# noway/nzcb-circom

Measured on AMD Instinct MI355X. Metric: PLONK proofs/sec for nzcp_live (~2^21 constraints) at 1/2/4/8 MI355X, higher is better.
Workload: dtype u32 limbs: BN254 Fr/Fq Montgomery, 8x32-bit and 9x29-bit (MSM, NTT twiddles, quotient); 1 GPU; nzcp_live fullProve: NZCPPubIdentity(1,351,0,4,2,4) witness on the GPU (600560 signals) + PLONK proof, n=2^21, nPublic=3, 2970 inputs; domain_size=2097152, n_public=3, n_constraints=1785813, n_vars=1782570, n_additions=1182010, proofs_per_gpu=140, total_proofs=140, parallelism=batch-shard x1 (no collective), proofs_in_flight_per_gpu=5

## Files before the change

include/nzcb_internal.h:

```cpp
#ifndef NZCB_INTERNAL_H
#define NZCB_INTERNAL_H

#include "nzcb.h"

#ifdef __cplusplus
extern "C" {
#endif

int nzcb_ctx_kernel_stats(nzcb_ctx* ctx, int enable, double out[4]);

int nzcb_debug_guard_check(int device, size_t* checked, int* damaged, nzcb_err* err);
int nzcb_debug_guard_selftest(int device, nzcb_err* err);

#define NZCB_FAULT_QUOTIENT 1
#define NZCB_DEBUG_GENERIC_K 2
#define NZCB_FAULT_LANE_ALLOC 3
int nzcb_debug_inject_fault(nzcb_ctx* ctx, int kind);

int nzcb_debug_f29(int device, int op, const uint32_t* in, size_t count, uint32_t* out, nzcb_err* err);

int nzcb_synth_setup(int power, int n_public, int n_inputs, uint64_t seed, uint32_t n_constraints,
                     const uint8_t* tau, int device, uint8_t** zkey_out, size_t* zkey_len, uint8_t** wtns_out,
                     size_t* wtns_len, nzcb_err* err);
#define NZCB_SYNTH_FREE_PUBLIC 1u
int nzcb_synth_setup_ex(int power, int n_public, int n_inputs, uint64_t seed, uint32_t n_constraints, uint32_t flags,
                        const uint8_t* tau, int device, uint8_t** zkey_out, size_t* zkey_len, uint8_t** wtns_out,
                        size_t* wtns_len, nzcb_err* err);
typedef struct nzcb_engine nzcb_engine;
nzcb_engine* nzcb_engine_create(int device, int max_log_ntt, size_t max_msm_points, nzcb_err* err);
void nzcb_engine_destroy(nzcb_engine* e);
int nzcb_engine_ntt(nzcb_engine* e, const uint8_t* in_lem, uint8_t* out_lem, int log_n, int inverse, nzcb_err* err);
int nzcb_engine_msm(nzcb_engine* e, const uint8_t* bases_lem, const uint8_t* scalars, size_t n, int scalars_mont,
                    uint8_t* out_affine, nzcb_err* err);
int nzcb_debug_ntt_coset(nzcb_engine* e, const uint8_t* in_lem, uint8_t* out_lem, int log_n, const uint8_t* c_lem,
                         int fold_len, nzcb_err* err);
int nzcb_engine_ntt_dev(nzcb_engine* e, const void* in, void* out, int log_n, int inverse, nzcb_err* err);
int nzcb_engine_msm_dev(nzcb_engine* e, const void* bases, const void* scalars, size_t n, int scalars_mont,
                        uint8_t* out_affine, nzcb_err* err);
int nzcb_engine_time_ntt(nzcb_engine* e, const void* in, void* out, int log_n, int inverse, int reps, double* ms,
                         nzcb_err* err);
int nzcb_engine_random_fr(nzcb_engine* e, void* dev_out, size_t n, uint64_t seed, nzcb_err* err);
int nzcb_engine_fixed_base(nzcb_engine* e, const void* dev_scalars_mont, size_t n, void* dev_out, nzcb_err* err);
int nzcb_engine_lagrange_basis(nzcb_engine* e, const void* dev_ptau, size_t ptau_n, int log_n, void* dev_out,
                               nzcb_err* err);
int nzcb_engine_time_msm(nzcb_engine* e, const void* bases, const void* scalars, size_t n, int scalars_mont, int reps,
                         double* ms, double* acc_ms, nzcb_err* err);
int nzcb_engine_msm_fixed_dev(nzcb_engine* e, const void* bases, size_t n_table, const void* scalars, size_t n,
                              int scalars_mont, uint8_t* out_affine, nzcb_err* err);
int nzcb_engine_msm_table_dev(nzcb_engine* e, const void* bases, size_t n_table, const void* scalars, size_t n,
                              int scalars_mont, int window, int sparse, int fold, uint8_t* out_affine,
                              nzcb_err* err);
int nzcb_debug_msm_plan(nzcb_engine* e, const void* bases, size_t n_table, const void* scalars, size_t n,
                        int scalars_mont, int window, int fold, uint32_t* info, uint32_t* offsets, size_t offsets_cap,
                        uint32_t* seg, size_t seg_cap, uint8_t* out_affine, nzcb_err* err);
int nzcb_engine_msm_sets_dev(nzcb_engine* e, const void* bases, size_t n_table, const void* const* scalars, int sets,
                             size_t n, int scalars_mont, int sparse, uint8_t* out_affine, nzcb_err* err);
int nzcb_engine_time_msm2(nzcb_engine* e, const void* bases, const void* scalars, size_t n, int scalars_mont,
                          int fixed_base, int reps, double* out, nzcb_err* err);
int nzcb_engine_fr_mul(nzcb_engine* e, const uint8_t* a_lem, const uint8_t* b_lem, uint8_t* out_lem, size_t n,
                       int field_q, nzcb_err* err);

int nzcb_engine_g1_lincomb(int device, const uint8_t* points, const uint8_t* scalars, const uint32_t* group_end,
                           size_t groups, uint8_t* out, nzcb_err* err);
int nzcb_engine_verify_batch(const uint8_t* vk, const uint8_t* proofs, const uint8_t* pubs, size_t pub_stride,
                             int n_public, int count, int transcript_public, int device, const uint8_t* seed,
                             int* valid_out, uint8_t* points_out, int* pairing_checks, nzcb_err* err);
int nzcb_debug_verify_batch_timings(double* ms, int cap);

nzcb_r1cs* nzcb_engine_r1cs_create(const uint8_t* r1cs, size_t len, int device, uint32_t long_row_threshold,
                                   int witness_tile, nzcb_err* err);
int nzcb_debug_r1cs_check_timings(double* ms, int cap);

nzcb_p256_key* nzcb_engine_p256_key_create(const uint8_t pub_xy[64], int device, int window, nzcb_err* err);
#define NZCB_P256_OP_ADD 0
#define NZCB_P256_OP_SUB 1
#define NZCB_P256_OP_MUL 2
#define NZCB_P256_OP_SQR 3
#define NZCB_P256_OP_INV 4
int nzcb_debug_p256_field(int device, int op, int field, const uint8_t* a, const uint8_t* b, size_t count,
                          uint8_t* out, nzcb_err* err);
int nzcb_debug_p256_mul2(nzcb_p256_key* k, const uint8_t* u1, const uint8_t* u2, size_t count, uint8_t* out_xy,
                         nzcb_err* err);
int nzcb_debug_p256_timings(double* ms, int cap);

int nzcb_debug_nzcp_decode_timings(double* ms, int cap);

int nzcb_engine_srs_check(int device, const uint8_t* points, uint64_t m, const uint8_t* g2, const uint8_t* seed,
                          uint32_t chunk_points, nzcb_key_finding* finding, uint8_t* lr_out ,
                          nzcb_err* err);
int nzcb_debug_key_check_timings(double* ms, int cap);

int nzcb_debug_ptau_timings(double* ms, int cap);
int nzcb_debug_ptau_batch_top(int level);

int nzcb_engine_groth16_rows(int device, int g2, const void* points, uint64_t n_points, const uint64_t* row_off,
                             uint64_t n_rows, const uint32_t* idx, const uint8_t* coefs, uint8_t* out,
                             nzcb_err* err);
int nzcb_debug_groth16_schedule(int chunk, int fan_in, int* prev_chunk, int* prev_fan_in);
int nzcb_debug_groth16_timings(double* out, int cap);

// ... 5 lines not shown
```

nzcb-circom_amd/csrc/capi_prover.cpp:

```cpp
#include <algorithm>
#include <atomic>
#include <condition_variable>
#include <cstring>
#include <mutex>
#include <shared_mutex>
#include <string>
#include <thread>
#include <vector>

#include "../../include/nzcb_internal.h"
#include "prover.h"

namespace nzcb {

std::string dec_le32(const uint8_t* le32) {
  uint32_t v[8];
  std::memcpy(v, le32, 32);
  std::string s;
  bool nz = true;
  while (nz) {
    uint64_t rem = 0;
    nz = false;
    for (int i = 7; i >= 0; i--) {
      uint64_t cur = (rem << 32) | v[i];
      v[i] = (uint32_t)(cur / 10);
      rem = cur % 10;
      if (v[i]) nz = true;
    }
    s.push_back((char)('0' + rem));
  }
  return std::string(s.rbegin(), s.rend());
}

}
using namespace nzcb;

struct nzcb_ctx {
  std::unique_ptr<Prover> p;
  std::vector<std::unique_ptr<Prover>> extra;
  std::vector<std::unique_ptr<Prover>> dev_p;
  std::vector<std::vector<std::unique_ptr<Prover>>> dev_extra;
  nzcb_log_fn log_fn = nullptr;
  void* log_user = nullptr;
  std::shared_mutex cfg;
  std::mutex pool_mu;
  std::condition_variable pool_cv;
  std::vector<Prover*> idle;
  double last_tm[11] = {0};
  std::atomic<int> pending_fault{0};
  std::atomic<int> lane_alloc_fault{0};
  Prover* lane(size_t i) { return i == 0 ? p.get() : extra[i - 1].get(); }
  size_t lanes() const { return 1 + extra.size(); }
  std::vector<Prover*> all() {
    std::vector<Prover*> v;
    for (size_t l = 0; l < lanes(); l++) {
      v.push_back(lane(l));
      for (size_t d = 0; d < dev_p.size(); d++) v.push_back(l == 0 ? dev_p[d].get() : dev_extra[d][l - 1].get());
    }
    return v;
  }
  std::vector<Prover*> usable() {
    if (p->split_send || !p->shards.empty()) return {p.get()};
    return all();
  }
  void reset_pool() {
    std::lock_guard<std::mutex> lk(pool_mu);
    idle = usable();
    std::reverse(idle.begin(), idle.end());
  }
  Prover* acquire(nzcb_log_fn fn, void* user) {
    Prover* q;
    {
      std::unique_lock<std::mutex> lk(pool_mu);
      pool_cv.wait(lk, [&] { return !idle.empty(); });
      q = idle.back();
      idle.pop_back();
    }
    if (!fn) {
      fn = log_fn;
      user = log_user;
    }
    if (fn)
      q->log = [fn, user](const std::string& m) { fn(user, m.c_str()); };
    else
      q->log = nullptr;
    q->fault = pending_fault.exchange(0);
    return q;
  }
  void release(Prover* q) {
    {
      std::lock_guard<std::mutex> lk(pool_mu);
      std::memcpy(last_tm, q->tm, sizeof(last_tm));
      idle.push_back(q);
    }
// ... 263 lines not shown
      throw;
    }
    pr->log = nullptr;
    ctx->release(pr);
    NZ_HIP(hipSetDevice(caller_dev));
  });
}
}

int nzcb_prove_witness(nzcb_ctx* ctx, const uint8_t* witness, size_t n_witness, const uint8_t* blinding,
                       uint8_t* proof_out, uint8_t* pub_out, size_t pub_cap, nzcb_err* err) {
  return prove_one(ctx, witness, n_witness, NZCB_WITNESS_HOST, blinding, proof_out, pub_out, pub_cap, nullptr, nullptr,
                   err);
}

int nzcb_prove_device(nzcb_ctx* ctx, const void* dev_witness, size_t n_witness, const uint8_t* blinding,
                      uint8_t* proof_out, uint8_t* pub_out, size_t pub_cap, nzcb_err* err) {
  return prove_one(ctx, dev_witness, n_witness, NZCB_WITNESS_DEVICE, blinding, proof_out, pub_out, pub_cap, nullptr,
                   nullptr, err);
}

int nzcb_prove(nzcb_ctx* ctx, const uint8_t* wtns, size_t wtns_len, const uint8_t* blinding, uint8_t* proof_out,
               uint8_t* pub_out, size_t pub_cap, nzcb_err* err) {
  return prove_one(ctx, wtns, wtns_len, NZCB_WITNESS_WTNS, blinding, proof_out, pub_out, pub_cap, nullptr, nullptr,
                   err);
}

int nzcb_prove_logged(nzcb_ctx* ctx, const void* witness, size_t n, int kind, const uint8_t* blinding,
                      uint8_t* proof_out, uint8_t* pub_out, size_t pub_cap, nzcb_log_fn log, void* log_user,
                      nzcb_err* err) {
  return prove_one(ctx, witness, n, kind, blinding, proof_out, pub_out, pub_cap, log, log_user, err);
}

int nzcb_ctx_last_timings(const nzcb_ctx* ctx, double* ms, int cap) {
  if (!ctx || !ms) return 0;
  int k = cap < 11 ? cap : 11;
  std::lock_guard<std::mutex> lk(const_cast<nzcb_ctx*>(ctx)->pool_mu);
  for (int i = 0; i < k; i++) ms[i] = ctx->last_tm[i];
  return k;
}

int nzcb_ctx_kernel_stats(nzcb_ctx* ctx, int enable, double out[4]) {
  if (!ctx) return NZCB_ERR_ARG;
  std::unique_lock<std::shared_mutex> ex(ctx->cfg, std::defer_lock);
  std::shared_lock<std::shared_mutex> sh(ctx->cfg, std::defer_lock);
  if (enable >= 0) ex.lock(); else sh.lock();
  if (out) {
    for (int i = 0; i < 4; i++) out[i] = 0;
    for (Prover* q : ctx->all())
      for (auto& m : q->msc) {
        out[0] += m->prof_ms;
        out[1] += (double)m->prof_launches;
        out[2] += (double)m->prof_points;
        out[3] += (double)m->prof_entries;
      }
  }
  if (enable >= 0) {
    for (Prover* q : ctx->all()) {
      q->prof_gpu = enable != 0;
      for (auto& m : q->msc) {
        m->prof = enable != 0;
        m->prof_ms = 0;
        m->prof_launches = m->prof_points = m->prof_entries = 0;
      }
    }
  }
  return 0;
}

int nzcb_debug_inject_fault(nzcb_ctx* ctx, int kind) {
  if (!ctx || (kind != 0 && kind != NZCB_FAULT_QUOTIENT && kind != NZCB_DEBUG_GENERIC_K &&
               kind != NZCB_FAULT_LANE_ALLOC))
    return NZCB_ERR_ARG;
  std::unique_lock<std::shared_mutex> lk(ctx->cfg);
  if (kind == NZCB_FAULT_LANE_ALLOC) {
    ctx->lane_alloc_fault = 1;
    return 0;
  }
  ctx->pending_fault = kind;
  if (kind == 0) ctx->lane_alloc_fault = 0;
  return 0;
}

int nzcb_proof_to_json(const uint8_t* proof, char* out, size_t cap) {
  if (!proof) return -1;
  static const char* pts[7] = {"A", "B", "C", "Z", "T1", "T2", "T3"};
  static const char* evs[7] = {"eval_a", "eval_b", "eval_c", "eval_s1", "eval_s2", "eval_zw", "eval_r"};
  std::string s = "{";
  for (int i = 0; i < 7; i++) s += std::string("\"") + pts[i] + "\":" + g1_json(proof + 64 * i) + ",";
  for (int i = 0; i < 7; i++) s += std::string("\"") + evs[i] + "\":\"" + dec_le32(proof + 9 * 64 + 32 * i) + "\",";
  s += "\"Wxi\":" + g1_json(proof + 7 * 64) + ",";
  s += "\"Wxiw\":" + g1_json(proof + 8 * 64) + ",";
  s += "\"protocol\":\"plonk\",\"curve\":\"bn128\"}";
  return copy_out(s, out, cap);
}

int nzcb_public_to_json(const uint8_t* pub, int n_public, char* out, size_t cap) {
  std::string s = "[";
  for (int i = 0; i < n_public; i++) {
    if (i) s += ",";
    s += "\"" + dec_le32(pub + 32 * i) + "\"";
  }
  s += "]";
  return copy_out(s, out, cap);
}

}
```

nzcb-circom_amd/csrc/groth16.h:

```cpp
#pragma once
#include <chrono>

#include "ptau_ops.h"
#include "r1cs_reader.h"

namespace nzcb {

struct G16Term {
  uint32_t idx, k;
};
constexpr uint32_t kG16Neg = 1u << 31, kG16Big = 1u << 30, kG16Low = kG16Big - 1;
struct G16Chunk {
  uint32_t t0, slot;
  uint16_t len, bits;
};
struct G16Fold {
  uint32_t begin, count;
};
constexpr uint32_t kG16NoSlot = ~0u;
constexpr uint32_t kG16DefaultChunk = 32, kG16DefaultFanIn = 8, kG16MaxKnob = 1024;

NZ_HD bool g16_bit(uint32_t k, const Fr* big, int b) {
  if (k & kG16Big) return (big[k & kG16Low].v[b >> 5] >> (b & 31)) & 1u;
  return b < 30 && ((k >> b) & 1u);
// ... 74 lines not shown
    if (!small) {
      if (big.size() >= kG16Low) throw Error(NZCB_ERR_ARG, "groth16: too many long coefficients");
      code = kG16Big | (uint32_t)big.size();
      big.push_back(k);
    }
    if (raw.size() >= kG16NoSlot - 1) throw Error(NZCB_ERR_ARG, "groth16: too many terms");
    raw.push_back({(uint32_t)row, (uint32_t)idx, code | (negative ? kG16Neg : 0u)});
  }
  G16Rows finish() {
    G16Rows r;
    r.n_rows = n_rows;
    r.n_points = n_points;
    r.row_off.assign((size_t)n_rows + 1, 0);
    for (const Raw& t : raw) r.row_off[t.row + 1]++;
    for (uint64_t i = 0; i < n_rows; i++) r.row_off[i + 1] += r.row_off[i];
    r.terms.resize(raw.size());
    std::vector<uint32_t> at(r.row_off.begin(), r.row_off.end() - 1);
    for (const Raw& t : raw) r.terms[at[t.row]++] = G16Term{t.idx, t.k};
    r.big = std::move(big);
    raw.clear();
    raw.shrink_to_fit();
    return r;
  }
};

struct G16Plan {
  std::vector<G16Chunk> chunks;
  std::vector<std::vector<G16Fold>> levels;
  std::vector<uint32_t> final_slot;
};
inline G16Plan g16_plan(G16Rows& r, uint32_t chunk, uint32_t fan_in) {
  if (chunk < 1 || chunk > kG16MaxKnob || fan_in < 2 || fan_in > kG16MaxKnob)
    throw Error(NZCB_ERR_ARG, "groth16: chunk length in 1..1024 and fan-in in 2..1024");
  G16Plan p;
  std::vector<uint32_t> off((size_t)r.n_rows), cnt((size_t)r.n_rows);
  std::vector<G16Chunk> cs;
  std::vector<uint32_t> hist((size_t)255 * (chunk + 1) + 1, 0);
  auto key = [&](const G16Chunk& c) { return (size_t)(254 - c.bits) * (chunk + 1) + (chunk - c.len); };
  uint32_t max_cnt = 0;
  for (uint64_t row = 0; row < r.n_rows; row++) {
    off[row] = (uint32_t)cs.size();
    if (r.row_off[row + 1] - r.row_off[row] > 1)
      std::stable_sort(r.terms.begin() + r.row_off[row], r.terms.begin() + r.row_off[row + 1],
                       [&](const G16Term& x, const G16Term& y) {
                         return g16_k_bits(x.k, r.big.data()) > g16_k_bits(y.k, r.big.data());
                       });
    for (uint32_t t0 = r.row_off[row], len; t0 < r.row_off[row + 1]; t0 += len) {
      uint32_t work = 0;
      for (len = 0; len < chunk && t0 + len < r.row_off[row + 1]; len++) {
        const uint32_t adds = std::max(1, g16_k_bits(r.terms[t0 + len].k, r.big.data()) / 2);
        if (len && work + adds > 4 * chunk) break;
        work += adds;
      }
      G16Chunk c;
      c.t0 = t0;
      c.slot = (uint32_t)cs.size();
      c.len = (uint16_t)len;
      c.bits = (uint16_t)g16_k_bits(r.terms[t0].k, r.big.data());
      hist[key(c) + 1]++;
      cs.push_back(c);
    }
    cnt[row] = (uint32_t)cs.size() - off[row];
    max_cnt = std::max(max_cnt, cnt[row]);
  }
  for (size_t i = 1; i < hist.size(); i++) hist[i] += hist[i - 1];
  p.chunks.resize(cs.size());
  for (const G16Chunk& c : cs) p.chunks[hist[key(c)]++] = c;
  while (max_cnt > 1) {
    std::vector<G16Fold> lv;
    max_cnt = 0;
    for (uint64_t row = 0; row < r.n_rows; row++) {
      const uint32_t begin = off[row], have = cnt[row];
      off[row] = (uint32_t)lv.size();
      for (uint32_t g = 0; g < have; g += fan_in) lv.push_back({begin + g, std::min(fan_in, have - g)});
      cnt[row] = (uint32_t)lv.size() - off[row];
      max_cnt = std::max(max_cnt, cnt[row]);
    }
    p.levels.push_back(std::move(lv));
  }
  p.final_slot.resize((size_t)r.n_rows);
  for (uint64_t row = 0; row < r.n_rows; row++) p.final_slot[row] = cnt[row] ? off[row] : kG16NoSlot;
  return p;
}

struct G16Schedule {
  uint32_t chunk = kG16DefaultChunk, fan_in = kG16DefaultFanIn;
};
inline G16Schedule& g16_schedule() {
  static G16Schedule s;
  return s;
}
enum {
  kG16MsKernels,
  kG16MsCall,
  kG16MsRowsG1,
  kG16MsRowsG2,
  kG16MsTests,
  kG16MsScale,
  kG16MsPlan,
  kG16TermsA,
  kG16TermsB1,
  kG16TermsB2,
  kG16TermsK,
  kG16ChunksG1,
  kG16ChunksG2,
  kG16StatCount
};
inline double* g16_stats() {
  thread_local double s[kG16StatCount] = {0};
  return s;
}
using G16Clock = std::chrono::steady_clock;
inline double g16_ms_since(G16Clock::time_point t0) {
  return std::chrono::duration<double, std::milli>(G16Clock::now() - t0).count();
}
struct G16CallClock {
  G16Clock::time_point t0 = G16Clock::now();
  G16CallClock() {
    for (int i = 0; i < kG16StatCount; i++) g16_stats()[i] = 0;
  }
  ~G16CallClock() { g16_stats()[kG16MsCall] = g16_ms_since(t0); }
};

struct G16Span {
  const uint8_t* p;
  uint64_t count;
};

struct G16HostBackend {
  Fq2 b2 = g2_twist_b();

  template <class F>
  Tally test(const uint8_t* pts, uint64_t n, bool zero_ok) {
    Tally t;
    for (uint64_t i = 0; i < n; i++) {
      PtAffine<F> p;
      std::memcpy((void*)&p, pts + sizeof p * i, sizeof p);
      const int st = g16_pt_status<F>(&p, b2, zero_ok);
      if (st == NZCB_KEY_OK) continue;
      t.n_bad++;
      t.key = std::min(t.key, srs_bad_key(i, st));
    }
    return t;
  }
  template <class F>
  void rows(const std::vector<G16Span>& spans, const G16Rows& r, const G16Plan& plan, uint8_t* out) {
    std::vector<PtAffine<F>> pts((size_t)r.n_points);
    size_t at = 0;
    for (const G16Span& s : spans) {
      if (s.count) std::memcpy((void*)(pts.data() + at), s.p, sizeof(PtAffine<F>) * (size_t)s.count);
      at += (size_t)s.count;
    }
    std::vector<PtXyzz<F>> a(plan.chunks.size()), b;
    parallel_for(plan.chunks.size(), [&](uint64_t i) {
      const G16Chunk& c = plan.chunks[i];
      a[c.slot] = g16_chunk_sum<F>(pts.data(), r.terms.data(), r.big.data(), c);
    });
    for (const auto& lv : plan.levels) {
      b.resize(lv.size());
      parallel_for(lv.size(), [&](uint64_t i) { b[i] = g16_fold_sum<F>(a.data(), lv[i]); });
      a.swap(b);
    }
    parallel_for(r.n_rows, [&](uint64_t row) {
      const uint32_t s = plan.final_slot[row];
      const PtAffine<F> v = s == kG16NoSlot ? PtAffine<F>{F::zero(), F::zero()} : pt_to_affine(a[s]);
      std::memcpy(out + sizeof v * row, &v, sizeof v);
// ... 334 lines not shown
```

nzcb-circom_amd/csrc/groth16.hip:

```cpp
#include "devcall.h"
#include "groth16.h"

namespace nzcb {

namespace {

constexpr unsigned kGB = 64;

template <class F>
__global__ __launch_bounds__(kGB) void k_g16_test(const PtAffine<F>* __restrict__ pts, uint64_t n, Fq2 b2,
                                                  int zero_ok, unsigned long long* res) {
  const uint64_t i = (uint64_t)blockIdx.x * kGB + threadIdx.x;
  if (i >= n) return;
  const PtAffine<F> p = pts[i];
  const int st = g16_pt_status<F>(&p, b2, zero_ok != 0);
  if (st != NZCB_KEY_OK) {
    atomicAdd(&res[0], 1ull);
    atomicMin(&res[1], (unsigned long long)srs_bad_key(i, st));
  }
}

template <class F>
__global__ __launch_bounds__(kGB) void k_g16_chunks(const PtAffine<F>* __restrict__ pts,
                                                    const G16Term* __restrict__ terms, const Fr* __restrict__ big,
// ... 109 lines not shown
    }
    k_g16_store<F><<<grid_for(r.n_rows, kGB, 1u << 30), kGB, 0, cs.st>>>(in, d_final.p, (uint32_t)r.n_rows, d_out.p);
    NZ_HIP(hipGetLastError());
    cs.record(1);
    NZ_HIP(hipMemcpyAsync(out, d_out.p, sizeof(PtAffine<F>) * (size_t)r.n_rows, hipMemcpyDeviceToHost, cs.st));
    NZ_HIP(hipStreamSynchronize(cs.st));
    took(std::is_same<F, Fq>::value ? kG16MsRowsG1 : kG16MsRowsG2);
  }
  template <class F>
  void rows(const std::vector<G16Span>& spans, const G16Rows& r, const G16Plan& plan, uint8_t* out) {
    DevBuf<PtAffine<F>> d_pts(std::max<size_t>(1, (size_t)r.n_points));
    size_t at = 0;
    for (const G16Span& s : spans) {
      if (s.count)
        NZ_HIP(hipMemcpyAsync(d_pts.p + at, s.p, sizeof(PtAffine<F>) * (size_t)s.count, hipMemcpyHostToDevice, cs.st));
      at += (size_t)s.count;
    }
    if (at != r.n_points) throw Error(NZCB_ERR_INTERNAL, "groth16: point count mismatch");
    rows_on<F>(d_pts.p, r, plan, out);
  }
  template <class F>
  void scale(const uint8_t* src, uint64_t n, const Fr& k, uint8_t* dst) {
    if (!n) return;
    DevBuf<uint8_t> d(sizeof(PtAffine<F>) * n);
    NZ_HIP(hipMemcpyAsync(d_k, &k, sizeof k, hipMemcpyHostToDevice, cs.st));
    NZ_HIP(hipMemcpyAsync(d.p, src, d.n, hipMemcpyHostToDevice, cs.st));
    cs.record(0);
    k_g16_scale<F><<<grid_for(n, kGB, 1u << 30), kGB, 0, cs.st>>>(reinterpret_cast<PtAffine<F>*>(d.p), n, d_k);
    NZ_HIP(hipGetLastError());
    cs.record(1);
    NZ_HIP(hipMemsetAsync(d_k, 0, sizeof(Fr), cs.st));
    NZ_HIP(hipMemcpyAsync(dst, d.p, d.n, hipMemcpyDeviceToHost, cs.st));
    NZ_HIP(hipStreamSynchronize(cs.st));
    took(kG16MsScale);
  }
};

void setup_on(int device, const uint8_t* r1cs, size_t r1cs_len, const uint8_t* ptau, size_t ptau_len,
              const char* out_path, PtauOut& o) {
  G16CallClock clock;
  if (device == NZCB_GROTH16_HOST) {
    G16HostBackend be;
    g16_setup(be, r1cs, r1cs_len, ptau, ptau_len, out_path, o);
  } else {
    G16DeviceBackend be(device);
    g16_setup(be, r1cs, r1cs_len, ptau, ptau_len, out_path, o);
  }
}

struct Secret {
  Fr d;
  ~Secret() { wipe(&d, sizeof d); }
};

void contribute_on(int device, const uint8_t* zkey, size_t len, const uint8_t* secret, const uint8_t* entropy,
                   size_t entropy_len, const char* out_path, PtauOut& o) {
  if (!zkey) throw Error(NZCB_ERR_ARG, "null argument");
  G16CallClock clock;
  (void)g16_zkey_open(zkey, len);
  Secret sec;
  make_secrets(secret, entropy, entropy_len, &sec.d, 1, "zkey");
  if (device == NZCB_GROTH16_HOST) {
    G16HostBackend be;
    g16_contribute(be, zkey, len, sec.d, out_path, o);
  } else {
    G16DeviceBackend be(device);
    g16_contribute(be, zkey, len, sec.d, out_path, o);
  }
}

void require_distinct(const char* in_path, const char* out_path, const char* what) {
  struct stat a, b;
  if (stat(in_path, &a) == 0 && stat(out_path, &b) == 0 && a.st_dev == b.st_dev && a.st_ino == b.st_ino)
    throw Error(NZCB_ERR_ARG, std::string(what) + ": the output path is an input file");
}

void give(PtauOut& o, uint8_t** out, size_t* out_len) {
  *out_len = (size_t)o.len;
  *out = o.release();
}

}

}

using namespace nzcb;

extern "C" {

int nzcb_groth16_setup(const uint8_t* r1cs, size_t r1cs_len, const uint8_t* ptau, size_t ptau_len, int device,
                       uint8_t** zkey_out, size_t* zkey_len, nzcb_err* err) {
  return guarded(err, [&] {
    if (!zkey_out || !zkey_len) throw Error(NZCB_ERR_ARG, "null argument");
    PtauOut o;
    setup_on(device, r1cs, r1cs_len, ptau, ptau_len, nullptr, o);
    give(o, zkey_out, zkey_len);
  });
}

int nzcb_groth16_setup_file(const char* r1cs_path, const char* ptau_path, const char* zkey_path, int device,
                            nzcb_err* err) {
  return guarded(err, [&] {
    if (!r1cs_path || !ptau_path || !zkey_path) throw Error(NZCB_ERR_ARG, "null argument");
    require_distinct(r1cs_path, zkey_path, "groth16");
    require_distinct(ptau_path, zkey_path, "groth16");
    MappedFile rf(r1cs_path, "the r1cs", "r1cs: invalid file format");
    MappedFile pf(ptau_path, "the ptau", "ptau: invalid file format");
    PtauOut o;
    setup_on(device, rf.data, rf.size, pf.data, pf.size, zkey_path, o);
  });
}

int nzcb_groth16_contribute(const uint8_t* zkey, size_t len, const uint8_t* secret, const uint8_t* entropy,
                            size_t entropy_len, int device, uint8_t** zkey_out, size_t* zkey_len, nzcb_err* err) {
  return guarded(err, [&] {
    if (!zkey_out || !zkey_len) throw Error(NZCB_ERR_ARG, "null argument");
    PtauOut o;
    contribute_on(device, zkey, len, secret, entropy, entropy_len, nullptr, o);
    give(o, zkey_out, zkey_len);
  });
}

int nzcb_groth16_contribute_file(const char* in_path, const char* out_path, const uint8_t* secret,
                                 const uint8_t* entropy, size_t entropy_len, int device, nzcb_err* err) {
  return guarded(err, [&] {
    if (!in_path || !out_path) throw Error(NZCB_ERR_ARG, "null argument");
    require_distinct(in_path, out_path, "zkey");
    MappedFile mf(in_path, "the zkey", "zkey: invalid file format");
    PtauOut o;
    contribute_on(device, mf.data, mf.size, secret, entropy, entropy_len, out_path, o);
  });
}

int nzcb_groth16_vk_to_json(const uint8_t* zkey, size_t len, char* out, size_t cap) {
  nzcb_err err;
  std::string s;
  const int rc = guarded(&err, [&] { s = g16_vk_json(zkey, len); });
  if (rc != 0) {
    if (out && cap) std::snprintf(out, cap, "%s", err.msg);
    return rc;
  }
  if (!out || cap < s.size() + 1) return -(int)(s.size() + 1);
  std::memcpy(out, s.c_str(), s.size() + 1);
  return 0;
}

int nzcb_groth16_vk_to_json_file(const char* zkey_path, char* out, size_t cap) {
  nzcb_err err;
  std::string s;
  const int rc = guarded(&err, [&] {
    if (!zkey_path) throw Error(NZCB_ERR_ARG, "null argument");
    MappedFile mf(zkey_path, "the zkey", "zkey: invalid file format");
    s = g16_vk_json(mf.data, mf.size);
  });
  if (rc != 0) {
    if (out && cap) std::snprintf(out, cap, "%s", err.msg);
    return rc;
  }
  if (!out || cap < s.size() + 1) return -(int)(s.size() + 1);
  std::memcpy(out, s.c_str(), s.size() + 1);
  return 0;
}

int nzcb_engine_groth16_rows(int device, int g2, const void* points, uint64_t n_points, const uint64_t* row_off,
                             uint64_t n_rows, const uint32_t* idx, const uint8_t* coefs, uint8_t* out,
                             nzcb_err* err) {
// ... 42 lines not shown
```

nzcb-circom_amd/csrc/msm.h:

```cpp
#pragma once
#include <vector>

#include "common.h"
#include "ec.h"
#include "f29.h"
#include "msm_seg.h"

namespace nzcb {

struct MsmBaseTable {
  DevBuf<G1Affine> q;
  size_t n = 0, stride = 0;
  int c = 0, nw = 0;
  bool mont_folded = false;
  bool sparse = false;
  void build(const G1Affine* bases, size_t n, int c, hipStream_t st, bool fold_mont = false);
};

int fixed_base_window();
int lagrange_window();
bool lagrange_sparse();
bool acc_segments();

struct MsmScratch {
  size_t max_points = 0;
  int max_lsets = 1;
  DevBuf<uint32_t> offsets;
  DevBuf<uint32_t> sorted;
  DevBuf<uint32_t> keys_in, keys_out, vals_in;
  DevBuf<uint8_t> sort_tmp;
  size_t sort_tmp_bytes = 0;
  DevBuf<uint32_t> bin_counts, vals_mid;
  DevBuf<uint32_t> lo_seg;
  DevBuf<G1xyzz> buckets;
  DevBuf<G1xyzz> carry_own;
  DevBuf<G1xyzz> carry_cont;
  DevBuf<Xyzz29> buckets29, carry_own29, carry_cont29;
  DevBuf<uint32_t> large;
  DevBuf<uint32_t> large_off;
  DevBuf<Xyzz29> large_part;
  DevBuf<uint32_t> seg_start, seg_len, seg_bucket, seg_dst, seg_cnt, seg_meta, seg_mk, seg_mfs, seg_mnp;
  DevBuf<Xyzz29> rowp29, colp29, lines29;
  DevBuf<G1xyzz> seg_tot;
  DevBuf<G1xyzz> seg_run;
  DevBuf<G1xyzz> parts;
  DevBuf<G1xyzz> win;
  G1xyzz* host_win = nullptr;
  uint32_t* host_total = nullptr;
  size_t host_win_cap = 0;
  int cur_c = 0, cur_nsets = 0, cur_nbits = 0, cur_seglen = 0;
  bool cur_fixed = false, cur_sparse = false;
  bool cur_seg = false;
  int cur_a = 0, cur_hb = 0;
  int cur_msets = 1;
  size_t cur_n = 0;
  uint32_t cur_nkeys = 0;
  bool prof = false, prof_phases = false;
  double prof_ms = 0;
  double phase_ms[7] = {0, 0, 0, 0, 0, 0, 0};
  double host_ms = 0;
  double enqueue_ms = 0;
  double sort_host_ms = 0;
  uint64_t prof_launches = 0, prof_points = 0, prof_entries = 0;
  hipEvent_t ev[8] = {nullptr, nullptr, nullptr, nullptr, nullptr, nullptr, nullptr, nullptr};
  hipEvent_t done = nullptr;
  void init(size_t max_points, bool fixed_base = false, int lagrange_sets = 1, bool generic = true);
  ~MsmScratch();
};

int msm_window_bits(size_t n);

void msm_enqueue(MsmScratch& sc, const G1Affine* bases, const Fr* scalars, size_t n, bool scalars_mont,
                 hipStream_t st, const MsmBaseTable* table = nullptr);
G1xyzz msm_finish(MsmScratch& sc, hipStream_t st);
void msm_enqueue_sets(MsmScratch& sc, const Fr* const* scalars, int sets, size_t n, bool scalars_mont,
                      hipStream_t st, const MsmBaseTable* table);
void msm_finish_sets(MsmScratch& sc, hipStream_t st, G1xyzz* out);

inline G1xyzz msm(MsmScratch& sc, const G1Affine* bases, const Fr* scalars, size_t n, bool mont, hipStream_t st,
                  const MsmBaseTable* table = nullptr) {
  msm_enqueue(sc, bases, scalars, n, mont, st, table);
  return msm_finish(sc, st);
}

bool msm_debug_plan(MsmScratch& sc, hipStream_t st, std::vector<uint32_t>& offsets, std::vector<uint32_t>& start,
                    std::vector<uint32_t>& len, std::vector<uint32_t>& bucket);

G1Affine xyzz_to_affine(const G1xyzz& p);

}
```

nzcb-circom_amd/csrc/msm.hip:

```cpp
#include "msm.h"

#include "f29.h"

#include <chrono>
#include <cstdlib>
#include <type_traits>
#include <rocprim/rocprim.hpp>
#include <rocprofiler-sdk-roctx/roctx.h>

namespace nzcb {

static constexpr int kMsmThreads = 256;

#ifndef NZ_TAIL_PRIO
#define NZ_TAIL_PRIO 0
#endif
__device__ __forceinline__ void tail_prio() {
  if constexpr (NZ_TAIL_PRIO > 0) __builtin_amdgcn_s_setprio(NZ_TAIL_PRIO);
}

using SortConfig = rocprim::radix_sort_config<
    rocprim::default_config, rocprim::default_config,
    rocprim::radix_sort_onesweep_config<rocprim::kernel_config<1024, 16>, rocprim::kernel_config<1024, 16>, 10,
                                        rocprim::block_radix_rank_algorithm::match>>;
// ... 97 lines not shown
      if (d) f(w, d - 1u, 0u);
      carry = 0;
    }
  }
}

#ifdef NZCB_MSM_STATS
template <class F>
static void for_each_digit_host(const Fr& s, int C, F&& f) {
  const int NW = (255 + C - 1) / C;
  const uint32_t MASK = (1u << C) - 1u, HALF = 1u << (C - 1);
  uint32_t carry = 0;
  for (int w = 0; w < NW; w++) {
    const int bit = w * C, limb = bit >> 5, sh = bit & 31;
    uint64_t x = s.v[limb];
    if (limb + 1 < 8) x |= (uint64_t)s.v[limb + 1] << 32;
    uint32_t d = ((uint32_t)(x >> sh) & MASK) + carry;
    if (d > HALF) {
      uint32_t mag = (MASK + 1u) - d;
      if (mag) f(w, mag - 1u, 1u);
      carry = 1;
    } else {
      if (d) f(w, d - 1u, 0u);
      carry = 0;
    }
  }
}
#endif

template <int C>
__global__ void __launch_bounds__(kMsmThreads)
msm_keys_kernel(const Fr* __restrict__ scalars, size_t n, int mont, uint32_t* __restrict__ keys,
                uint32_t* __restrict__ vals) {
  constexpr int NW = (255 + C - 1) / C;
  constexpr uint32_t NB = 1u << (C - 1);
  constexpr uint32_t SENTINEL = NW * NB;
  for (size_t i = (size_t)blockIdx.x * blockDim.x + threadIdx.x; i < n; i += (size_t)gridDim.x * blockDim.x) {
    Fr s = scalars[i];
    if (mont) s = from_mont_fr29(s);
    uint32_t k[NW];
#pragma unroll
    for (int w = 0; w < NW; w++) k[w] = SENTINEL;
    uint32_t sg[NW];
#pragma unroll
    for (int w = 0; w < NW; w++) sg[w] = 0;
    for_each_digit<C>(s, [&](int w, uint32_t b, uint32_t sign) {
      k[w] = (uint32_t)w * NB + b;
      sg[w] = sign << 31;
    });
#pragma unroll
    for (int w = 0; w < NW; w++) {
      keys[(size_t)w * n + i] = k[w];
      vals[(size_t)w * n + i] = (uint32_t)i | sg[w];
    }
  }
}

static constexpr int kBinThreads = 256;
static constexpr int kBinPer = 2;
static constexpr uint32_t kTileScalars = kBinThreads * kBinPer;
static constexpr int kLoThreads = 512;

static constexpr int kDigMont = 1;
static constexpr int kDigMinForm = 2;

__device__ __forceinline__ uint32_t scalar_min_form(Fr& s) {
  constexpr uint32_t H[8] = {0xf8000000u, 0xa1f0fac9u, 0x3cdcb848u, 0x9419f424u,
                             0x40c0ac2eu, 0xdc2822dbu, 0x7098d014u, 0x18322739u};
  bool gt = false, eq = true, lt_r = false, eq_r = true;
#pragma unroll
  for (int l = 7; l >= 0; l--) {
    gt = gt || (eq && s.v[l] > H[l]);
    eq = eq && s.v[l] == H[l];
    lt_r = lt_r || (eq_r && s.v[l] < FrParams::P[l]);
    eq_r = eq_r && s.v[l] == FrParams::P[l];
  }
  if (!(gt && lt_r)) return 0u;
  s = neg(s);
  return 1u;
}

template <int C, int NW>
__device__ __forceinline__ uint32_t bin_entries(const Fr* __restrict__ scalars, size_t i, int mont, size_t stride,
                                                uint32_t (&kk)[NW], uint32_t (&vv)[NW]) {
  Fr s = scalars[i];
  if (mont & kDigMont) s = from_mont_fr29(s);
  const uint32_t flip = (mont & kDigMinForm) ? scalar_min_form(s) : 0u;
  uint32_t live = 0;
#pragma unroll
  for (int w = 0; w < NW; w++) {
    kk[w] = 0;
    vv[w] = 0;
  }
  for_each_digit<C>(s, [&](int w, uint32_t b, uint32_t sign) {
    kk[w] = b;
    vv[w] = (uint32_t)((size_t)w * stride + i) | ((sign ^ flip) << 31);
    live |= 1u << w;
  });
  return live;
}

template <int KB> struct BinKeys {
  static constexpr int LO = KB - 8 > 8 ? KB - 8 : 8;
  using Lo = typename std::conditional<LO <= 8, uint8_t, uint16_t>::type;
  using Full = typename std::conditional<KB <= 16, uint16_t, uint32_t>::type;
};

static constexpr int kMaxSets = 3;
struct BinSets {
  const Fr* p[kMaxSets];
  uint32_t tps;
  uint32_t nb;
};

template <int C, int KB>
__global__ void __launch_bounds__(kBinThreads)
msm_bin_hist_kernel(BinSets sets, size_t n, int mont, uint32_t* __restrict__ counts, uint32_t ntiles) {
  constexpr int NW = (255 + C - 1) / C;
  constexpr int LO = BinKeys<KB>::LO;
  __shared__ uint32_t h[256];
  h[threadIdx.x] = 0;
  __syncthreads();
  const uint32_t set = blockIdx.x / sets.tps, lt = blockIdx.x - set * sets.tps;
  const Fr* __restrict__ scalars = sets.p[set];
  const uint32_t kbase = set * sets.nb;
#pragma unroll
  for (int j = 0; j < kBinPer; j++) {
    const size_t i = (size_t)lt * kTileScalars + (size_t)j * kBinThreads + threadIdx.x;
    if (i < n) {
      uint32_t kk[NW], vv[NW];
      const uint32_t live = bin_entries<C, NW>(scalars, i, mont, 0, kk, vv);
#pragma unroll
      for (int w = 0; w < NW; w++)
        if ((live >> w) & 1u) atomicAdd(&h[(kk[w] + kbase) >> LO], 1u);
    }
  }
  __syncthreads();
  counts[(size_t)threadIdx.x * ntiles + blockIdx.x] = h[threadIdx.x];
}

__device__ __forceinline__ uint32_t wave_incl_scan(uint32_t v) {
  const int lane = threadIdx.x & 63;
#pragma unroll
  for (int off = 1; off < 64; off <<= 1) {
    const uint32_t u = __shfl_up(v, off, 64);
    if (lane >= off) v += u;
  }
  return v;
}

__device__ __forceinline__ uint32_t scan256_excl(uint32_t v, uint32_t* wsum4, uint32_t& total) {
  const uint32_t inc = wave_incl_scan(threadIdx.x < 256 ? v : 0u);
  if (threadIdx.x < 256 && (threadIdx.x & 63) == 63) wsum4[threadIdx.x >> 6] = inc;
  __syncthreads();
  uint32_t off = 0;
  for (int w = 0; w < (int)(threadIdx.x >> 6) && w < 4; w++) off += wsum4[w];
  total = wsum4[0] + wsum4[1] + wsum4[2] + wsum4[3];
  __syncthreads();
  return threadIdx.x < 256 ? off + inc - v : 0u;
}

__global__ void __launch_bounds__(256)
msm_bin_rowscan_kernel(uint32_t* __restrict__ counts, uint32_t ntiles, uint32_t* __restrict__ tail) {
  __shared__ uint32_t wsum[4];
  uint32_t* row = counts + (size_t)blockIdx.x * ntiles;
  uint32_t carry = 0;
  for (uint32_t c0 = 0; c0 < ntiles; c0 += 256) {
    const uint32_t t = c0 + threadIdx.x;
    const uint32_t v = t < ntiles ? row[t] : 0u;
    uint32_t tot;
    const uint32_t ex = scan256_excl(v, wsum, tot);
    if (t < ntiles) row[t] = carry + ex;
    carry += tot;
  }
  if (threadIdx.x == 0) tail[blockIdx.x] = carry;
}

template <int C, int KB>
__global__ void __launch_bounds__(kBinThreads)
msm_bin_scatter_kernel(BinSets sets, size_t n, int mont, size_t stride, const uint32_t* __restrict__ counts,
                       uint32_t ntiles, typename BinKeys<KB>::Lo* __restrict__ lo2, uint32_t* __restrict__ vals2) {
  constexpr int NW = (255 + C - 1) / C;
  constexpr int TE = kTileScalars * NW;
  constexpr int LO = BinKeys<KB>::LO;
  __shared__ uint32_t lcount[256], lstart[256], gbase[256];
  __shared__ uint32_t lval[TE];
  __shared__ typename BinKeys<KB>::Full lkey[TE];
  const uint32_t set = blockIdx.x / sets.tps, lt = blockIdx.x - set * sets.tps;
  const Fr* __restrict__ scalars = sets.p[set];
  const uint32_t kbase = set * sets.nb;
  __shared__ uint32_t wsum[4];
  const uint32_t* tail = counts + (size_t)256 * ntiles;
  {
    uint32_t tot;
    const uint32_t st = scan256_excl(tail[threadIdx.x], wsum, tot);
    gbase[threadIdx.x] = st + counts[(size_t)threadIdx.x * ntiles + blockIdx.x];
    lcount[threadIdx.x] = 0;
  }
  __syncthreads();
  uint32_t kk[kBinPer][NW], vv[kBinPer][NW], rk[kBinPer][NW], live[kBinPer];
#pragma unroll
  for (int j = 0; j < kBinPer; j++) {
    const size_t i = (size_t)lt * kTileScalars + (size_t)j * kBinThreads + threadIdx.x;
    live[j] = 0;
    if (i < n) {
      live[j] = bin_entries<C, NW>(scalars, i, mont, stride, kk[j], vv[j]);
#pragma unroll
      for (int w = 0; w < NW; w++) {
        kk[j][w] += kbase;
        if ((live[j] >> w) & 1u) rk[j][w] = atomicAdd(&lcount[kk[j][w] >> LO], 1u);
      }
    }
  }
  __syncthreads();
  uint32_t total;
  {
    lstart[threadIdx.x] = scan256_excl(lcount[threadIdx.x], wsum, total);
  }
  __syncthreads();
#pragma unroll
  for (int j = 0; j < kBinPer; j++) {
#pragma unroll
    for (int w = 0; w < NW; w++) {
      if ((live[j] >> w) & 1u) {
        const uint32_t q = lstart[kk[j][w] >> LO] + rk[j][w];
        lkey[q] = (typename BinKeys<KB>::Full)kk[j][w];
        lval[q] = vv[j][w];
      }
    }
  }
  __syncthreads();
  for (uint32_t q = threadIdx.x; q < total; q += kBinThreads) {
    const uint32_t key = lkey[q], hb = key >> LO;
    const uint32_t pos = gbase[hb] + (q - lstart[hb]);
    lo2[pos] = (typename BinKeys<KB>::Lo)(key & ((1u << LO) - 1u));
    vals2[pos] = lval[q];
  }
}

template <int NT>
__device__ __forceinline__ uint32_t block_scan_excl(uint32_t* a, uint32_t count, uint32_t* wsum) {
  const uint32_t per = (count + NT - 1) / NT;
  const uint32_t b = threadIdx.x * per;
  uint32_t loc = 0;
  for (uint32_t i = 0; i < per; i++)
    if (b + i < count) loc += a[b + i];
  const uint32_t inc = wave_incl_scan(loc);
  if ((threadIdx.x & 63) == 63) wsum[threadIdx.x >> 6] = inc;
  __syncthreads();
  uint32_t off = 0, tot = 0;
#pragma unroll
  for (int w = 0; w < NT / 64; w++) {
    if (w < (int)(threadIdx.x >> 6)) off += wsum[w];
    tot += wsum[w];
  }
  uint32_t run = off + inc - loc;
  for (uint32_t i = 0; i < per; i++)
    if (b + i < count) {
      const uint32_t v = a[b + i];
      a[b + i] = run;
      run += v;
    }
  __syncthreads();
  return tot;
}

static constexpr uint32_t kLoSeg = 32768;
static constexpr uint32_t kLoU = 8;

__device__ __forceinline__ void lo_regions(const uint32_t* __restrict__ tail, uint32_t* wsum, uint32_t* rs,
                                           uint32_t* rf) {
  const uint32_t t = threadIdx.x;
  const uint32_t cnt = t < 256 ? tail[t] : 0u;
  uint32_t tot, nitems;
  const uint32_t st = scan256_excl(cnt, wsum, tot);
  const uint32_t f = scan256_excl((cnt + kLoSeg - 1) / kLoSeg, wsum, nitems);
  if (t < 256) {
    rs[t] = st;
    rf[t] = f;
  }
  if (t == 0) rf[256] = nitems;
  __syncthreads();
}

__device__ __forceinline__ uint32_t lo_region_of(const uint32_t* rf, uint32_t item) {
  uint32_t lo = 0, hi = 256;
  while (hi - lo > 1) {
    const uint32_t mid = (lo + hi) >> 1;
    if (rf[mid] <= item) lo = mid; else hi = mid;
// ... 206 lines not shown
    inf = false;
  } else {
    F29 U2, S2, PP, RR;
    mul29x2<Fq29>(x, acc.ZZ, y, acc.ZZZ, U2, S2);
    const F29 Pd = sub29(U2, acc.X, Fq29::K8);
    const F29 R = sub29(S2, acc.Y, Fq29::K4);
    sqr29x2(Pd, R, PP, RR);
    if (is0p29_fast(PP)) {
      if (is0p29(RR)) {
        norm29(y);
        mdbl29_rare(x, y, &acc);
      } else {
        inf = true;
      }
    } else {
      F29 PPP, Q, ZZ3, ZZZ3;
      mul29x2<Fq29>(Pd, PP, acc.X, PP, PPP, Q);
      const F29 X3 = sub2x29(RR, PPP, Q);
      mul29x2<Fq29>(acc.ZZ, PP, acc.ZZZ, PPP, ZZ3, ZZZ3);
      acc.Y = mul2sum29(R, sub29_nn(Q, X3, Fq29W::K10), neg4p29_nn(acc.Y), PPP);
      acc.ZZ = ZZ3;
      acc.ZZZ = ZZZ3;
      acc.X = X3;
    }
  }
}

static constexpr uint32_t kLdsStride = kMsmThreads + 1;
template <bool kLdsIdx>
__global__ void __launch_bounds__(kMsmThreads) __attribute__((amdgpu_waves_per_eu(3, 8)))
msm_accumulate29_kernel(uint32_t chunk, const G1Affine* __restrict__ bases, const uint32_t* __restrict__ sorted,
                        const uint32_t* __restrict__ offsets, uint32_t nkeys, size_t nthreads,
                        Xyzz29* __restrict__ buckets, Xyzz29* __restrict__ carry_own,
                        Xyzz29* __restrict__ carry_cont) {
  __shared__ uint32_t sidx[kLdsIdx ? kChunk * kLdsStride : 1];
  const uint32_t t = blockIdx.x * blockDim.x + threadIdx.x;
  const uint32_t M = offsets[nkeys];
  if (!chunk) {
    chunk = dyn_chunk(M);
    tail_prio();
  }
  if (kLdsIdx) {
    const uint32_t wg0 = (uint32_t)blockIdx.x * kMsmThreads * chunk;
    if (wg0 >= M) return;
    const uint32_t inv = (uint32_t)((0x100000000ull + chunk - 1) / chunk);
    for (uint32_t j = threadIdx.x; j < kMsmThreads * chunk; j += kMsmThreads) {
      const uint32_t thr = __umulhi(j, inv), slot = j - thr * chunk;
      sidx[slot * kLdsStride + thr] = wg0 + j < M ? sorted[wg0 + j] : 0u;
    }
    __syncthreads();
  }
  if (t >= nthreads) return;
  const uint32_t s = (uint32_t)t * chunk;
  if (s >= M) return;
  const uint32_t e = (s + chunk < M) ? s + chunk : M;
  auto index_at = [&](uint32_t q) -> uint32_t {
    return kLdsIdx ? sidx[(q - s) * kLdsStride + threadIdx.x] : sorted[q];
  };
  uint32_t k = find_key(offsets, nkeys, s);
  uint32_t kstart = offsets[k], kend = offsets[k + 1];
  Xyzz29 acc;
  bool inf = true;
  uint32_t ent = index_at(s);
  G1Affine P = bases[ent & 0x7fffffffu];
  uint32_t ent_n = s + 1 < e ? index_at(s + 1) : 0u;
  for (uint32_t pos = s; pos < e;) {
    G1Affine Pn;
    uint32_t ent_nn = 0;
    if (pos + 1 < e) Pn = bases[ent_n & 0x7fffffffu];
    if (pos + 2 < e) ent_nn = index_at(pos + 2);
    acc_entry29(acc, inf, P, ent);
    pos++;
    if (pos == kend || pos == e) {
      const bool starts = kstart >= s;
      const bool ends = kend <= e;
      Xyzz29 out = acc;
      if (inf)
#pragma unroll
        for (int i = 0; i < 9; i++) out.ZZ.v[i] = 0;
      if (starts && ends) buckets[k] = out;
      else if (!starts) carry_cont[t] = out;
      else carry_own[t] = out;
      inf = true;
      while (pos < e && kend <= pos) {
        k++;
        kstart = kend;
        kend = offsets[k + 1];
      }
    }
    ent = ent_n;
    ent_n = ent_nn;
    P = Pn;
  }
}

struct SegPlan {
  uint32_t *start, *len, *bucket, *dst;
  uint32_t *mk, *mfs, *mnp;
  uint32_t* meta;
};

static constexpr int kSegThreads = 256;
static constexpr uint32_t kSegWaves = kSegThreads / 64;

__global__ void __launch_bounds__(kSegThreads)
msm_seg_hist_kernel(const uint32_t* __restrict__ offsets, uint32_t nkeys, uint32_t ntiles,
                    uint32_t* __restrict__ cnt, uint32_t* __restrict__ meta) {
  __shared__ uint32_t h[kSegWaves][kSegMax + 1];
  const uint32_t wave = threadIdx.x >> 6, lane = threadIdx.x & 63;
  const uint32_t tile = blockIdx.x * kSegWaves + wave;
  for (uint32_t i = threadIdx.x; i < kSegWaves * (kSegMax + 1); i += kSegThreads) (&h[0][0])[i] = 0;
  if (blockIdx.x == 0 && threadIdx.x == 0) meta[1] = 0;
  __syncthreads();
  if (tile < ntiles) {
    for (uint32_t it = 0; it < kSegTile / 64; it++) {
      const uint32_t k = tile * kSegTile + it * 64 + lane;
      if (k >= nkeys) break;
      const uint32_t len = offsets[k + 1] - offsets[k];
      const uint32_t whole = len / kSegMax, rest = len % kSegMax;
      if (whole) atomicAdd(&h[wave][kSegMax], whole);
      if (rest) atomicAdd(&h[wave][rest], 1u);
    }
  }
  __syncthreads();
  if (tile < ntiles)
    for (uint32_t L = 1 + lane; L <= kSegMax; L += 64) cnt[(size_t)(kSegMax - L) * ntiles + tile] = h[wave][L];
}

__global__ void __launch_bounds__(kSegThreads)
msm_seg_scatter_kernel(const uint32_t* __restrict__ offsets, uint32_t nkeys, uint32_t ntiles,
                       const uint32_t* __restrict__ cnt, SegPlan pl) {
  __shared__ uint32_t cb[256], wsum[4];
  __shared__ uint32_t base_s[kSegWaves][kSegMax + 1];
  const uint32_t wave = threadIdx.x >> 6, lane = threadIdx.x & 63;
  const uint32_t tile = blockIdx.x * kSegWaves + wave;
  uint32_t total;
  const uint32_t* tail = cnt + (size_t)kSegMax * ntiles;
  cb[threadIdx.x] = scan256_excl(threadIdx.x < kSegMax ? tail[threadIdx.x] : 0u, wsum, total);
  if (blockIdx.x == 0 && threadIdx.x == 0) pl.meta[0] = total;
  __syncthreads();
  volatile uint32_t* base = base_s[wave];
  if (tile < ntiles)
    for (uint32_t L = 1 + lane; L <= kSegMax; L += 64)
      base[L] = cb[kSegMax - L] + cnt[(size_t)(kSegMax - L) * ntiles + tile];
  __syncthreads();
  if (tile >= ntiles) return;
  for (uint32_t it = 0; it < kSegTile / 64; it++) {
    const uint32_t k0 = tile * kSegTile + it * 64;
    if (k0 >= nkeys) break;
    const uint32_t k = k0 + lane;
    const uint32_t s = k < nkeys ? offsets[k] : 0u;
    const uint32_t len = k < nkeys ? offsets[k + 1] - s : 0u;
    const uint32_t whole = len / kSegMax, rest = len % kSegMax;
    const bool cut = whole + (rest ? 1u : 0u) > 1;
    const uint32_t incl = wave_incl_scan(whole);
    const uint32_t wtot = __shfl(incl, 63, 64);
    const uint32_t fs = base[kSegMax] + incl - whole;
    if (lane == 0 && wtot) base[kSegMax] = fs + wtot;
    const uint32_t dst = cut ? 0x80000000u | fs : k;
    for (uint32_t j = 0; j < whole; j++) {
      pl.start[fs + j] = s + j * kSegMax;
      pl.len[fs + j] = kSegMax;
      pl.bucket[fs + j] = k;
      pl.dst[fs + j] = dst;
    }
    uint64_t same = __ballot(rest != 0);
#pragma unroll
// ... 733 lines not shown
  };
  switch (c) {
#define NZ_CASE(K) case K: launch(std::integral_constant<int, K>()); break;
    NZ_CASE(4) NZ_CASE(5) NZ_CASE(6) NZ_CASE(7) NZ_CASE(8) NZ_CASE(9) NZ_CASE(10) NZ_CASE(11) NZ_CASE(12)
    NZ_CASE(13) NZ_CASE(14) NZ_CASE(15) NZ_CASE(16)
#undef NZ_CASE
    default: throw Error(NZCB_ERR_INTERNAL, "bad msm window");
  }
  NZ_HIP(hipGetLastError());
}

G1Affine xyzz_to_affine(const G1xyzz& p) {
  G1Affine r;
  if (p.is_inf()) {
    r.x = Fq::zero();
    r.y = Fq::zero();
    return r;
  }
  r.x = p.X * inverse(p.ZZ);
  r.y = p.Y * inverse(p.ZZZ);
  return r;
}

template <class Mark>
static void fixed_bucketing(MsmScratch& sc, const MsmPlan& p, const BinSets& sets, size_t n, int mdig,
                            const MsmBaseTable* table, hipStream_t st, const Mark& mark) {
  const uint32_t tps = (uint32_t)((n + kTileScalars - 1) / kTileScalars);
  const uint32_t ntiles = tps * (uint32_t)p.msets;
  BinSets bs = sets;
  bs.tps = tps;
  bs.nb = p.nb;
  uint32_t* tail = sc.bin_counts.p + (size_t)256 * ntiles;
  auto run_bins = [&](auto cc, auto kb) {
    constexpr int C = decltype(cc)::value;
    constexpr int KB = decltype(kb)::value;
    using Lo = typename BinKeys<KB>::Lo;
    constexpr int LO = BinKeys<KB>::LO;
    Lo* lo2 = (Lo*)sc.keys_out.p;
    hipLaunchKernelGGL((msm_bin_hist_kernel<C, KB>), dim3(ntiles), dim3(kBinThreads), 0, st, bs, n, mdig,
                       sc.bin_counts.p, ntiles);
    NZ_HIP(hipGetLastError());
    lmark("mark: L hist");
    mark(1);
    hipLaunchKernelGGL(msm_bin_rowscan_kernel, dim3(256), dim3(256), 0, st, sc.bin_counts.p, ntiles, tail);
    lmark("mark: L rowscan");
    hipLaunchKernelGGL((msm_bin_scatter_kernel<C, KB>), dim3(ntiles), dim3(kBinThreads), 0, st, bs, n, mdig,
                       table->stride, sc.bin_counts.p, ntiles, lo2, sc.vals_mid.p);
    NZ_HIP(hipGetLastError());
    lmark("mark: L scatter");
    mark(2);
    const dim3 igrid((unsigned)lo_items_bound(p.entries));
    hipLaunchKernelGGL(msm_lo_count_kernel<LO>, igrid, dim3(kLoThreads), 0, st, (const Lo*)lo2, sc.bin_counts.p,
                       ntiles, sc.lo_seg.p);
    NZ_HIP(hipGetLastError());
    lmark("mark: L lo_count");
    hipLaunchKernelGGL(msm_lo_scan_kernel<LO>, dim3(256), dim3(kLoThreads), 0, st, sc.bin_counts.p, ntiles,
                       sc.lo_seg.p, p.nkeys, sc.offsets.p, sc.large.p);
    NZ_HIP(hipGetLastError());
    lmark("mark: L lo_scan");
    constexpr int sNT = LO > 8 ? 1024 : kLoThreads;
    constexpr uint32_t sU = LO > 8 ? 16 : kLoU;
    hipLaunchKernelGGL((msm_lo_scatter_kernel<LO, sNT, sU>), igrid, dim3(sNT), 0, st, (const Lo*)lo2, sc.vals_mid.p,
                       sc.bin_counts.p, ntiles, (const uint32_t*)sc.lo_seg.p, sc.sorted.p);
    NZ_HIP(hipGetLastError());
    lmark("mark: L lo_scatter");
  };
  using std::integral_constant;
  if (p.msets > 1) {
    if (p.c != 17) throw Error(NZCB_ERR_INTERNAL, "msm sets: the Lagrange window (17) only");
    run_bins(integral_constant<int, 17>(), integral_constant<int, 18>());
    return;
  }
  switch (p.c) {
    case 16: run_bins(integral_constant<int, 16>(), integral_constant<int, 15>()); break;
    case 17: run_bins(integral_constant<int, 17>(), integral_constant<int, 16>()); break;
    case 18: run_bins(integral_constant<int, 18>(), integral_constant<int, 17>()); break;
    case 19: run_bins(integral_constant<int, 19>(), integral_constant<int, 18>()); break;
    case 20: run_bins(integral_constant<int, 20>(), integral_constant<int, 19>()); break;
    default: throw Error(NZCB_ERR_INTERNAL, "bad fixed-base msm window");
  }
}

static void msm_enqueue_impl(MsmScratch& sc, const G1Affine* bases, const Fr* const* scalars, int msets, size_t n,
                             bool mont, hipStream_t st, const MsmBaseTable* table) {
  const auto t_enq = std::chrono::steady_clock::now();
  struct EnqueueClock {
    MsmScratch& sc;
    std::chrono::steady_clock::time_point t0;
    ~EnqueueClock() {
      if (sc.prof && sc.prof_phases)
        sc.enqueue_ms += std::chrono::duration<double, std::milli>(std::chrono::steady_clock::now() - t0).count();
    }
  } enqueue_clock{sc, t_enq};
  if (msets < 1 || msets > kMaxSets || (msets > 1 && (!table || msets > sc.max_lsets)))
    throw Error(NZCB_ERR_ARG, "msm sets: 1..3 over a table, within the scratch's sizing");
  sc.cur_n = n;
  sc.cur_msets = table ? msets : 1;
  if (n == 0) return;
  if (!sc.done) NZ_HIP(hipEventCreateWithFlags(&sc.done, hipEventDisableTiming));
  if (n > sc.max_points) throw Error(NZCB_ERR_ARG, "msm larger than scratch");
  if (table && n > table->n) throw Error(NZCB_ERR_ARG, "msm larger than its base table");
  if (table && table->mont_folded && !mont) throw Error(NZCB_ERR_ARG, "2^-256-folded table needs Montgomery scalars");
  if (table && (!sc.buckets29.p || !sc.bin_counts.p))
    throw Error(NZCB_ERR_ARG, "msm scratch was not sized for the fixed-base schedule");
  const int mdig = (mont && !(table && table->mont_folded)) ? 1 : 0;
  const MsmPlan p = make_plan(n, table, msets);
#ifdef NZCB_MSM_STATS
  if (table && !table->mont_folded) {
    NZ_HIP(hipStreamSynchronize(st));
    for (int k = 0; k < msets; k++) {
      std::vector<Fr> h(n);
      NZ_HIP(hipMemcpy(h.data(), scalars[k], n * sizeof(Fr), hipMemcpyDeviceToHost));
      size_t e_pos = 0, e_min = 0, nneg = 0, zero = 0, hist[17] = {0};
      for (size_t i = 0; i < n; i++) {
        Fr v = mdig ? from_mont(h[i]) : h[i];
        if (v.is_zero()) { zero++; continue; }
        const Fr w = neg(v);
        auto digits = [&](const Fr& x) {
          size_t d = 0;
          for_each_digit_host(x, p.c, [&](int, uint32_t, uint32_t) { d++; });
          return d;
        };
        const size_t dp = digits(v), dn = digits(w);
        e_pos += dp;
        e_min += dp <= dn ? dp : dn;
        if (dn < dp) nneg++;
        const size_t dm = dp <= dn ? dp : dn;
        hist[dm < 16 ? dm : 16]++;
      }
      fprintf(stderr, "MSMSCALARS set=%d n=%zu c=%d zero=%zu entries=%zu entries_minform=%zu flipped=%zu hist_minform=",
              k, n, p.c, zero, e_pos, e_min, nneg);
      for (int b = 0; b < 17; b++) fprintf(stderr, "%zu%c", hist[b], b == 16 ? '\n' : ',');
    }
  }
#endif
  if (p.entries + 4 > sc.sorted.n || p.nkeys + 1 > sc.offsets.n)
    throw Error(NZCB_ERR_ARG, "msm scratch was not sized for this schedule");
  const bool seg = table && !table->sparse && msets == 1 && acc_segments();
  if (seg && (seg_bound(p.entries, p.nkeys) > sc.seg_start.n || seg_counters(p.nkeys) > sc.seg_cnt.n ||
              seg_multi_bound(p.entries, p.nkeys) + 1 > sc.seg_mk.n ||
              seg_whole_bound(p.entries) + 1 > sc.carry_cont29.n ||
              seg_carry_bound(p.entries, p.nkeys) / kPieceCarries + seg_multi_bound(p.entries, p.nkeys) + 1 >
                  sc.large_part.n))
    throw Error(NZCB_ERR_ARG, "msm scratch was not sized for the segment plan");
  if (table && ((size_t)p.nb / kTileSide * msets > sc.rowp29.n ||
                (((size_t)1 << p.hb) + ((size_t)1 << p.a)) * msets > sc.lines29.n ||
                (size_t)(p.lb + 1) * msets > sc.host_win_cap || (msets > 1 && p.c >= kStripMinC)))
    throw Error(NZCB_ERR_ARG, "msm scratch was not sized for this window");
  sc.cur_c = p.c;
  sc.cur_nsets = p.nsets;
  sc.cur_nbits = p.nbits;
  sc.cur_seglen = p.seglen;
  sc.cur_nkeys = p.nkeys;
  sc.cur_fixed = table != nullptr;
  sc.cur_seg = seg;
  sc.cur_a = p.a;
  sc.cur_hb = p.hb;
  sc.cur_msets = p.msets;
  const bool phases = sc.prof && sc.prof_phases;
  if (sc.prof && !sc.ev[0])
    for (auto& e : sc.ev) NZ_HIP(hipEventCreate(&e));
  auto mark = [&](int i) {
    if (phases) NZ_HIP(hipEventRecord(sc.ev[i], st));
  };
  mark(0);
  if (table) {
    BinSets bs{};
    for (int k = 0; k < msets; k++) bs.p[k] = scalars[k];
    fixed_bucketing(sc, p, bs, n, mdig | (table->mont_folded ? 0 : kDigMinForm), table, st, mark);
  } else {
    keys_dispatch(p.c, scalars[0], n, mdig, sc, st);
    mark(1);
    size_t tmp = sc.sort_tmp_bytes;
    int end_bit = 1;
    while ((1u << end_bit) <= p.nkeys) end_bit++;
    const auto t_sort = std::chrono::steady_clock::now();
    radix_sort(sc.sort_tmp.p, tmp, sc.keys_in.p, sc.keys_out.p, sc.vals_in.p, sc.sorted.p, p.entries, end_bit, st);
    if (phases)
      sc.sort_host_ms += std::chrono::duration<double, std::milli>(std::chrono::steady_clock::now() - t_sort).count();
    mark(2);
    hipLaunchKernelGGL(msm_offsets_kernel, dim3(grid_for((size_t)p.nkeys + 1, kMsmThreads, 1u << 30)),
                       dim3(kMsmThreads), 0, st, sc.keys_out.p, p.entries, p.nkeys, sc.offsets.p);
    NZ_HIP(hipGetLastError());
  }
  const SegPlan pl{sc.seg_start.p, sc.seg_len.p, sc.seg_bucket.p, sc.seg_dst.p,
                   sc.seg_mk.p,    sc.seg_mfs.p, sc.seg_mnp.p,   sc.seg_meta.p};
  if (seg) {
    const uint32_t ntiles = (uint32_t)seg_tiles(p.nkeys);
    const dim3 tgrid((ntiles + kSegWaves - 1) / kSegWaves);
    hipLaunchKernelGGL(msm_seg_hist_kernel, tgrid, dim3(kSegThreads), 0, st, (const uint32_t*)sc.offsets.p, p.nkeys,
                       ntiles, sc.seg_cnt.p, sc.seg_meta.p);
    NZ_HIP(hipGetLastError());
    hipLaunchKernelGGL(msm_bin_rowscan_kernel, dim3(kSegMax), dim3(256), 0, st, sc.seg_cnt.p, ntiles,
                       sc.seg_cnt.p + (size_t)kSegMax * ntiles);
    NZ_HIP(hipGetLastError());
    hipLaunchKernelGGL(msm_seg_scatter_kernel, tgrid, dim3(kSegThreads), 0, st, (const uint32_t*)sc.offsets.p, p.nkeys,
                       ntiles, (const uint32_t*)sc.seg_cnt.p, pl);
    NZ_HIP(hipGetLastError());
    lmark("mark: L seg_plan");
  }
  if (sc.prof) NZ_HIP(hipEventRecord(sc.ev[3], st));
  const bool sparse = table && table->sparse;
  sc.cur_sparse = sparse;
  const uint32_t chunk = sparse ? 0u : chunk_for(p.entries);
  const size_t nthreads = sparse ? dyn_threads_bound(p.entries) : (p.entries + chunk - 1) / chunk;
  const dim3 agrid(grid_for(nthreads, kMsmThreads, 1u << 30));
  const G1Affine* gather = table ? table->q.p : bases;
  if (seg) {
    const dim3 sgrid(grid_for(seg_bound(p.entries, p.nkeys), kMsmThreads, 1u << 30));
    hipLaunchKernelGGL(msm_accumulate29_seg_kernel, sgrid, dim3(kMsmThreads), 0, st, gather, (const uint32_t*)sc.sorted.p,
                       (const uint32_t*)pl.start, (const uint32_t*)pl.len, (const uint32_t*)pl.dst,
                       (const uint32_t*)pl.meta, sc.buckets29.p, sc.carry_own29.p, sc.carry_cont29.p);
  } else if (table) {
    if (chunk == kChunk || sparse)
      hipLaunchKernelGGL(msm_accumulate29_kernel<true>, agrid, dim3(kMsmThreads), 0, st, chunk, gather, sc.sorted.p,
                         sc.offsets.p, p.nkeys, nthreads, sc.buckets29.p, sc.carry_own29.p, sc.carry_cont29.p);
    else
      hipLaunchKernelGGL(msm_accumulate29_kernel<false>, agrid, dim3(kMsmThreads), 0, st, chunk, gather, sc.sorted.p,
                         sc.offsets.p, p.nkeys, nthreads, sc.buckets29.p, sc.carry_own29.p, sc.carry_cont29.p);
  } else {
    hipLaunchKernelGGL(msm_accumulate_kernel, agrid, dim3(kMsmThreads), 0, st, chunk, gather, sc.sorted.p, sc.offsets.p,
                       p.nkeys, nthreads, sc.buckets.p, sc.carry_own.p, sc.carry_cont.p);
  }
  NZ_HIP(hipGetLastError());
  lmark("mark: L accumulate");
  if (sc.prof) NZ_HIP(hipEventRecord(sc.ev[4], st));
  const dim3 fgrid(grid_for(p.nkeys, kMsmThreads, 1u << 30));
  if (table) {
    auto finalize = [&](auto kseg) {
      constexpr bool kSeg = decltype(kseg)::value;
      const dim3 grid = kSeg ? dim3(grid_for(seg_multi_bound(p.entries, p.nkeys) + 1, kMsmThreads, 1u << 30)) : fgrid;
      hipLaunchKernelGGL(msm_finalize29_kernel<kSeg>, grid, dim3(kMsmThreads), 0, st, chunk, sc.offsets.p, p.nkeys,
                         sparse ? kSeqSpanSparse : kSeqSpan29, (const Xyzz29*)sc.carry_own29.p,
                         (const Xyzz29*)sc.carry_cont29.p, sc.large.p, sc.buckets29.p, pl);
      NZ_HIP(hipGetLastError());
      lmark("mark: L finalize");
      hipLaunchKernelGGL(msm_large_scan_kernel<kSeg>, dim3(1), dim3(1024), 0, st, chunk, sc.offsets.p, p.nkeys,
                         sc.large.p, sc.large_off.p, pl);
      NZ_HIP(hipGetLastError());
      lmark("mark: L large_scan");
      hipLaunchKernelGGL(msm_large_piece29_kernel<kSeg>, dim3(sparse ? kSparsePieceBlocks : kLargePieceBlocks),
                         dim3(kSumThreads), 0, st, chunk, sc.offsets.p, p.nkeys, sc.large.p, sc.large_off.p,
                         (const Xyzz29*)sc.carry_own29.p, (const Xyzz29*)sc.carry_cont29.p, sc.large_part.p, pl);
      NZ_HIP(hipGetLastError());
      lmark("mark: L piece");
      if (sparse)
        hipLaunchKernelGGL((msm_large_final29_kernel<kSumThreads, kSeg>), dim3(kSparseFinalBlocks), dim3(kSumThreads),
                           0, st, sc.large.p, sc.large_off.p, sc.large_part.p, sc.buckets29.p,
                           (const uint32_t*)pl.mk);
      else
        hipLaunchKernelGGL((msm_large_final29_kernel<64, kSeg>), dim3(kLargeFinalBlocks), dim3(64), 0, st, sc.large.p,
// ... 5 lines not shown
    mark(5);
    int lparts = p.ltiles, hparts = p.htiles;
    if (p.c >= kStripMinC) {
      lparts = (1 << p.a) / kStrip;
      hparts = (1 << p.hb) / kStrip;
      const size_t nthr = ((size_t)lparts << p.hb) + ((size_t)hparts << p.a);
      hipLaunchKernelGGL(msm_strips29_kernel, dim3(grid_for(nthr, 256, 1u << 30)), dim3(256), 0, st,
                         (const Xyzz29*)sc.buckets29.p, sc.offsets.p, p.a, p.hb, sc.rowp29.p, sc.colp29.p);
    } else {
      hipLaunchKernelGGL(msm_tile29_kernel, dim3((unsigned)(p.ltiles * p.htiles), (unsigned)p.msets), dim3(256), 0, st,
                         (const Xyzz29*)sc.buckets29.p, sc.offsets.p, p.a, p.ltiles, p.htiles, sc.rowp29.p, sc.colp29.p);
    }
    NZ_HIP(hipGetLastError());
    mark(6);
    const int nrows = 1 << p.hb, ncols = 1 << p.a;
    hipLaunchKernelGGL(msm_lines29_kernel, dim3(grid_for((size_t)(nrows + ncols) * kLineThreads, 256), (unsigned)p.msets),
                       dim3(256), 0,
                       st, (const Xyzz29*)sc.rowp29.p, lparts, (const Xyzz29*)sc.colp29.p, hparts, nrows, ncols,
                       sc.lines29.p);
    NZ_HIP(hipGetLastError());
    lmark("mark: L lines");
    hipLaunchKernelGGL(msm_slots29_kernel, dim3(p.hb + p.a + 1, (unsigned)p.msets), dim3(kSumThreads), 0, st,
                       (const Xyzz29*)sc.lines29.p, p.hb, p.a, sc.host_win, (const uint32_t*)sc.offsets.p + p.nkeys,
                       sc.prof ? sc.host_total : nullptr);
    NZ_HIP(hipGetLastError());
    lmark("mark: L slots");
    mark(7);
    NZ_HIP(hipEventRecord(sc.done, st));
    return;
  }
  NZ_HIP(hipMemsetAsync(sc.large.p, 0, sizeof(uint32_t), st));
  hipLaunchKernelGGL(msm_bucket_finalize_kernel, fgrid, dim3(kMsmThreads), 0, st, chunk, sc.offsets.p, p.nkeys,
                     kSeqSpan, (const G1xyzz*)sc.carry_own.p, (const G1xyzz*)sc.carry_cont.p, sc.buckets.p, sc.large.p);
  NZ_HIP(hipGetLastError());
  hipLaunchKernelGGL(msm_bucket_large_kernel, dim3(kLargeBlocks), dim3(kSumThreads), 0, st, chunk, sc.offsets.p,
                     sc.large.p, (const G1xyzz*)sc.carry_own.p, (const G1xyzz*)sc.carry_cont.p, sc.buckets.p);
  NZ_HIP(hipGetLastError());
  mark(5);
  hipLaunchKernelGGL(msm_bucket_reduce_kernel, dim3(grid_for((size_t)p.nsets * p.nseg, kMsmThreads, 1u << 30)),
                     dim3(kMsmThreads), 0, st, sc.buckets.p, sc.offsets.p, (int)p.nb, p.seglen, p.nseg, p.nsets,
                     sc.seg_tot.p, sc.seg_run.p);
  NZ_HIP(hipGetLastError());
  mark(6);
  hipLaunchKernelGGL(msm_sums_kernel, dim3(p.nsets * p.nslots * p.nparts), dim3(kSumThreads), 0, st, sc.seg_tot.p,
                     sc.seg_run.p, p.nseg, p.nslots, p.nparts, sc.parts.p);
  NZ_HIP(hipGetLastError());
  hipLaunchKernelGGL(msm_parts_kernel, dim3(p.nsets * p.nslots), dim3(kPartThreads), 0, st, sc.parts.p, p.nparts,
                     sc.win.p);
  NZ_HIP(hipGetLastError());
  mark(7);
  if (sc.prof) NZ_HIP(hipMemcpyAsync(sc.host_total, sc.offsets.p + p.nkeys, 4, hipMemcpyDeviceToHost, st));
  NZ_HIP(hipMemcpyAsync(sc.host_win, sc.win.p, (size_t)p.nsets * p.nslots * sizeof(G1xyzz), hipMemcpyDeviceToHost,
                        st));
  NZ_HIP(hipEventRecord(sc.done, st));
}

bool msm_debug_plan(MsmScratch& sc, hipStream_t st, std::vector<uint32_t>& offsets, std::vector<uint32_t>& start,
                    std::vector<uint32_t>& len, std::vector<uint32_t>& bucket) {
  if (!sc.cur_fixed || !sc.cur_seg || sc.cur_n == 0) return false;
  NZ_HIP(hipStreamSynchronize(st));
  uint32_t meta[2] = {0, 0};
  NZ_HIP(hipMemcpy(meta, sc.seg_meta.p, sizeof(meta), hipMemcpyDeviceToHost));
  if (meta[0] > sc.seg_start.n) throw Error(NZCB_ERR_INTERNAL, "segment plan larger than its bound");
  offsets.resize((size_t)sc.cur_nkeys + 1);
  start.resize(meta[0]);
  len.resize(meta[0]);
  bucket.resize(meta[0]);
  NZ_HIP(hipMemcpy(offsets.data(), sc.offsets.p, offsets.size() * 4, hipMemcpyDeviceToHost));
  if (meta[0]) {
    NZ_HIP(hipMemcpy(start.data(), sc.seg_start.p, (size_t)meta[0] * 4, hipMemcpyDeviceToHost));
    NZ_HIP(hipMemcpy(len.data(), sc.seg_len.p, (size_t)meta[0] * 4, hipMemcpyDeviceToHost));
    NZ_HIP(hipMemcpy(bucket.data(), sc.seg_bucket.p, (size_t)meta[0] * 4, hipMemcpyDeviceToHost));
  }
  return true;
}

void msm_enqueue(MsmScratch& sc, const G1Affine* bases, const Fr* scalars, size_t n, bool mont, hipStream_t st,
                 const MsmBaseTable* table) {
  const Fr* one[1] = {scalars};
  msm_enqueue_impl(sc, bases, one, 1, n, mont, st, table);
}

void msm_enqueue_sets(MsmScratch& sc, const Fr* const* scalars, int sets, size_t n, bool mont, hipStream_t st,
                      const MsmBaseTable* table) {
  if (!table) throw Error(NZCB_ERR_ARG, "msm sets: a table schedule");
  msm_enqueue_impl(sc, nullptr, scalars, sets, n, mont, st, table);
}

static G1xyzz fixed_window_result(const G1xyzz* s, int hb, int a) {
  G1xyzz acc = G1xyzz::inf();
  for (int b = hb - 1; b >= 0; b--) acc = xyzz_add(xyzz_dbl(acc), s[b]);
  for (int i = 0; i < a; i++) acc = xyzz_dbl(acc);
  G1xyzz col = G1xyzz::inf();
  for (int b = a - 1; b >= 0; b--) col = xyzz_add(xyzz_dbl(col), s[hb + b]);
  return xyzz_add(xyzz_add(acc, col), s[hb + a]);
}

void msm_finish_sets(MsmScratch& sc, hipStream_t st, G1xyzz* out) {
  const int msets = sc.cur_msets;
  if (sc.cur_n == 0) {
    for (int k = 0; k < msets; k++) out[k] = G1xyzz::inf();
    return;
  }
  out[0] = msm_finish(sc, st);
  for (int k = 1; k < msets; k++) out[k] = fixed_window_result(sc.host_win + (size_t)k * (sc.cur_hb + sc.cur_a + 1),
                                                               sc.cur_hb, sc.cur_a);
}

G1xyzz msm_finish(MsmScratch& sc, hipStream_t st) {
  if (sc.cur_n == 0) return G1xyzz::inf();
  NZ_HIP(hipEventSynchronize(sc.done));
#ifdef NZCB_MSM_STATS
  if (sc.cur_fixed) {
    std::vector<uint32_t> off(sc.cur_nkeys + 1);
    NZ_HIP(hipMemcpy(off.data(), sc.offsets.p, off.size() * 4, hipMemcpyDeviceToHost));
    uint32_t cnt = 0;
    NZ_HIP(hipMemcpy(&cnt, sc.large.p, 4, hipMemcpyDeviceToHost));
    uint32_t pieces = 0;
    NZ_HIP(hipMemcpy(&pieces, sc.large_off.p + cnt, 4, hipMemcpyDeviceToHost));
    const uint32_t M = off.back();
    const uint32_t chunk = sc.cur_sparse ? dyn_chunk(M) : chunk_for(sc.cur_n * (size_t)num_windows(sc.cur_c));
    size_t h[12] = {0};
    uint32_t mx = 0;
    uint64_t carries_large = 0, carries_mid = 0;
    for (uint32_t k = 0; k < sc.cur_nkeys; k++) {
      if (off[k + 1] == off[k]) { h[0]++; continue; }
      const uint32_t sp = (off[k + 1] - 1) / chunk - off[k] / chunk + 1;
      mx = sp > mx ? sp : mx;
      int b = 1;
      while (b < 11 && sp > (1u << (b - 1))) b++;
      h[b]++;
      if (sp > (sc.cur_sparse ? kSeqSpanSparse : kSeqSpan29) + 1) carries_large += sp; else if (sp > 1) carries_mid += sp;
    }
    fprintf(stderr, "MSMSTATS n=%zu c=%d entries=%u chunk=%u large=%u pieces=%u maxspan=%u carries_mid=%llu "
            "carries_large=%llu spans[empty,1,2,<=4,<=8,..,<=512,>512]=", sc.cur_n, sc.cur_c, M, chunk, cnt, pieces, mx,
            (unsigned long long)carries_mid, (unsigned long long)carries_large);
    for (int b = 0; b < 12; b++) fprintf(stderr, "%zu%c", h[b], b == 11 ? '\n' : ',');
  }
#endif
  const int c = sc.cur_c, nsets = sc.cur_nsets, nslots = sc.cur_nbits + 1;
  if (sc.prof) {
    float t = 0;
    NZ_HIP(hipEventElapsedTime(&t, sc.ev[3], sc.ev[4]));
    const uint32_t total = *sc.host_total;
    sc.prof_ms += t;
    sc.prof_launches++;
    sc.prof_points += sc.cur_n;
    sc.prof_entries += total;
    if (sc.prof_phases) {
      for (int i = 0; i < 7; i++) {
        float ms = 0;
        NZ_HIP(hipEventElapsedTime(&ms, sc.ev[i], sc.ev[i + 1]));
        sc.phase_ms[i] += ms;
      }
    }
  }
  const auto t_host = std::chrono::steady_clock::now();
  struct HostClock {
    MsmScratch& sc;
    std::chrono::steady_clock::time_point t0;
    ~HostClock() {
      if (sc.prof && sc.prof_phases)
        sc.host_ms += std::chrono::duration<double, std::milli>(std::chrono::steady_clock::now() - t0).count();
    }
  } host_clock{sc, t_host};
  if (sc.cur_fixed) return fixed_window_result(sc.host_win, sc.cur_hb, sc.cur_a);
  int lg_seg = 0;
  while ((1 << lg_seg) < sc.cur_seglen) lg_seg++;
  G1xyzz res = G1xyzz::inf();
// ... 18 lines not shown
```

nzcb-circom_amd/csrc/prover.h:

```cpp
#pragma once
#include <chrono>
#include <functional>
#include <memory>
#include <string>
#include <vector>

#include "engine.h"
#include "zkey.h"

namespace nzcb {

struct AddRec {
  uint32_t ai, bi, dst, pad;
  Fr ac, bc;
};

struct MsmShard {
  static constexpr int kSlots = 3;
  int device = 0;
  size_t lo = 0, hi = 0;
  size_t llo = 0, lhi = 0;
  MsmBaseTable table, ltable;
  std::unique_ptr<MsmScratch> sc[kSlots];
  DevBuf<Fr> scal[kSlots];
  hipStream_t st[kSlots] = {nullptr, nullptr, nullptr};
  ~MsmShard();
};

struct Prover {
  uint32_t n = 0, n4 = 0, nVars = 0, nPublic = 0, nAdditions = 0, nConstraints = 0, nWit = 0;
  int power = 0;
  Fr k1, k2, wn, w2;
  std::vector<uint32_t> add_level_start;
  bool transcript_public = true;
  std::function<void(const std::string&)> log;

  std::unique_ptr<Engine> eng;
  static constexpr int kSlots = 3;
  std::unique_ptr<MsmScratch> msc[kSlots];
  hipStream_t aux[kSlots] = {nullptr, nullptr, nullptr};
  hipEvent_t ready[kSlots] = {nullptr, nullptr, nullptr};
  bool slot_split[kSlots] = {false, false, false};
  bool slot_lag[kSlots] = {false, false, false};
  hipEvent_t side_ready = nullptr, side_done = nullptr, pows_done = nullptr;
  ~Prover();
  DevBuf<G1Affine> ptau;
  MsmBaseTable ptab;
  DevBuf<G1Affine> ltau;
  MsmBaseTable ltab;
  bool lcommit = false;
  DevBuf<Fr> qm, ql, qr, qo, qc;
  DevBuf<Fr> sigma;
  DevBuf<Fr> sig_h;
  DevBuf<Fr> q_h;
  DevBuf<Fr> w_h;
  DevBuf<Fr> lagrange;
  DevBuf<uint32_t> amap, bmap, cmap;
  DevBuf<AddRec> adds;
  DevBuf<Fr> root_lo, root_hi;
  DevBuf<Fr> x_lo;
  DevBuf<Fr> g_lo, g_hi, gi_lo, gi_hi;
  DevBuf<F29> g29, gi29;
  Fr zh_inv[4];
  DevBuf<Fr> cq, cs, cl;
  bool quot3 = false;
  DevBuf<Fr> cq3, cs3, cl3;
  DevBuf<NttTables::Tw> ctw3;
  DevBuf<F29> itw3;
  Fr d3[3];
  Fr sig_top[3][4];
  DevBuf<Fr> wit;
  DevBuf<Fr> wtns_in;
  DevBuf<Fr> A, B, C, Z;
  DevBuf<Fr> pol_a, pol_b, pol_c, pol_z;
  DevBuf<Fr> A4, B4, C4, Z4, T, Tz, t;
  DevBuf<Fr> bx_lo;
  DevBuf<Fr> pol_r, pol_wxi, pol_wxiw;
  DevBuf<Fr> blind;
  DevBuf<Fr> scan_tmp;
  DevBuf<Fr> lin_tab;
  size_t lin_qn = 0;
  Fr* lin_tile_pows(int k);
  std::vector<Fr> lin_host;
  DevBuf<Fr> eval_part;
  DevBuf<F29> eval_pw;
  DevBuf<uint32_t> flags;
  std::vector<Fr> host_part;
  DevBuf<uint32_t> ntt_scr2;
  Fr* top_host = nullptr;
  static constexpr int kMbFlags = 24, kMbTotals = 25, kMbEvals = 27, kMbEvalMax = 8;
  size_t mb_apub = 0, mb_pubw = 0, mb_words = 0;

  int lane_id = 0;
  int fault = 0;
  double tm[11] = {0};
  bool prof_gpu = false;
  std::vector<std::pair<hipEvent_t, hipEvent_t>> span_ev;
  std::vector<int> span_kind;
  size_t spans_used = 0;
  size_t span_begin(int kind, hipStream_t s);
  void span_end(size_t i, hipStream_t s);
  void span_totals(double* msm_ms, double* ntt_ms);

  Prover(const uint8_t* zkey, size_t len, int device);
  Prover(const Prover& primary, int lane);
  void set_msm_devices(const std::vector<int>& devices);
  std::vector<std::unique_ptr<MsmShard>> shards;
  size_t own_hi = 0, own_lhi = 0;
  nzcb_msm_send_fn split_send = nullptr;
  nzcb_msm_gather_fn split_gather = nullptr;
  void* split_user = nullptr;
  int split_world = 1;
  size_t split_own = 0, split_own_l = 0;
  void set_msm_split(int world, size_t own_points, size_t own_lagrange, nzcb_msm_send_fn send,
                     nzcb_msm_gather_fn gather, void* user);
  void prove(const uint8_t* witness, size_t n_witness, const uint8_t* blinding, uint8_t* proof_out,
             uint8_t* pub_out, bool witness_on_device = false);

 private:
  hipStream_t st() const { return eng->stream; }
  void init_slots();
  void alloc_workspace();
  void to4t(const Fr* evals, Fr* coefs, Fr* evals4, const int* bidx, int nb, hipStream_t s = nullptr);
  void to4t_coefs(const Fr* evals, Fr* coefs, const int* bidx, int nb, hipStream_t s, uint32_t* scr = nullptr);
  void to4t_evals4(const Fr* coefs, Fr* evals4, int nb, hipStream_t s, uint32_t* scr = nullptr);
  void round3_quot3(const Fr& beta, const Fr& gamma, const Fr& alpha, hipStream_t s);
  void launch_gate_check(hipStream_t s);
  void copy_tops(hipStream_t s);
  void commit_start(int slot, const Fr* scalars, size_t len, const MsmBaseTable* tab = nullptr,
                    const G1Affine* bases = nullptr, bool on_main = false);
  G1Affine commit_finish(int slot);
  void commit_start_abc(size_t len);
  void commit_finish_abc(G1Affine& a, G1Affine& b, G1Affine& c);
  void eval_many(int np, const Fr* const* polys, const size_t* lens, const Fr* xs, Fr* out,
                 const std::function<void()>& overlap = nullptr);
  void div_pol1(const Fr* src, size_t m, int tab, const Fr& p0_adjust, Fr* dst, uint32_t flag_bit);
  void lin_tables(int k, const Fr& d, hipStream_t s);
  double ms_since(std::chrono::steady_clock::time_point t0);
  double msm_ms = 0, ntt_ms = 0;
};

}
```

nzcb-circom_amd/csrc/prover.hip:

```cpp
#include <rocprofiler-sdk-roctx/roctx.h>
#include "lagrange.h"
#include "prover.h"
#include "transcript.h"

#include <cstring>
#include <cerrno>
#include <string>
#include <sys/random.h>

#include "keccak.h"

namespace nzcb {

static constexpr int kT = 256;
static constexpr uint32_t kZeroRef = 0xffffffffu;

__global__ void k_wit_to_mont(const Fr* __restrict__ in, Fr* __restrict__ out, size_t n) {
  size_t i = (size_t)blockIdx.x * blockDim.x + threadIdx.x;
  if (i >= n) return;
  out[i] = (i == 0) ? Fr::zero() : to_mont(in[i]);
}

__global__ void k_additions(const AddRec* __restrict__ recs, uint32_t count, Fr* __restrict__ wit) {
  uint32_t i = blockIdx.x * blockDim.x + threadIdx.x;
  if (i >= count) return;
  const AddRec r = recs[i];
  Fr a = r.ai == kZeroRef ? Fr::zero() : wit[r.ai];
  Fr b = r.bi == kZeroRef ? Fr::zero() : wit[r.bi];
  wit[r.dst] = r.ac * a + r.bc * b;
}


__global__ void k_build_abc(const uint32_t* __restrict__ am, const uint32_t* __restrict__ bm,
                            const uint32_t* __restrict__ cm, uint32_t nc, uint32_t n, const Fr* __restrict__ wit,
                            uint32_t nvars, Fr* __restrict__ A, Fr* __restrict__ B, Fr* __restrict__ C,
                            uint32_t npub, Fr* __restrict__ mb_apub, Fr* __restrict__ mb_pubw) {
  uint32_t i = blockIdx.x * blockDim.x + threadIdx.x;
  if (i < npub) {
    host_put(mb_pubw + i, 1 + i < nvars ? wit[1 + i] : Fr::zero());
  }
  if (i >= n) {
    if (i < npub) host_put_done();
    return;
  }
  Fr a = Fr::zero(), b = Fr::zero(), c = Fr::zero();
  if (i < nc) {
    uint32_t ia = am[i], ib = bm[i], ic = cm[i];
    if (ia < nvars) a = wit[ia];
    if (ib < nvars) b = wit[ib];
    if (ic < nvars) c = wit[ic];
  }
  A[i] = a;
  B[i] = b;
  C[i] = c;
  if (i < npub) {
    host_put(mb_apub + i, a);
    host_put_done();
  }
}

__global__ void k_tops(const Fr* __restrict__ pa, const Fr* __restrict__ pb, const Fr* __restrict__ pc,
                       const Fr* __restrict__ pz, size_t n, const uint32_t* __restrict__ flags, Fr* __restrict__ mb) {
  const int t = threadIdx.x;
  if (t < 24) {
    const int k = t / 6, j = t % 6;
    const Fr* src = k == 0 ? pa + (n - 4) : k == 1 ? pb + (n - 4) : k == 2 ? pc + (n - 4) : pz + (n - 3);
    host_put(mb + t, src[j]);
  } else if (t == 24) {
    Fr f = Fr::zero();
    f.v[0] = *flags;
    host_put(mb + 24, f);
  }
  host_put_done();
}

struct BlindIdx {
  int idx[3];
  int count;
};

__global__ void k_blind(Fr* pol, size_t n, const Fr* __restrict__ bl, BlindIdx bi) {
  if (threadIdx.x != 0 || blockIdx.x != 0) return;
  for (int k = 0; k < bi.count; k++) {
    Fr b = bl[bi.idx[k]];
    pol[n + k] = b;
    pol[k] = pol[k] - b;
  }
}

__global__ void k_abc_tail(Fr* A, Fr* B, Fr* C, size_t n, const Fr* __restrict__ bl) {
  if (threadIdx.x != 0 || blockIdx.x != 0) return;
  A[n] = bl[2];
  A[n + 1] = bl[1];
  B[n] = bl[4];
  B[n + 1] = bl[3];
  C[n] = bl[6];
  C[n + 1] = bl[5];
}

static bool abc_sets_enabled() {
  static const bool v = [] {
    const char* e = std::getenv("NZCB_ABC_SETS");
    return !e || std::atoi(e) != 0;
  }();
  return v;
}

static bool lagrange_commit_enabled() {
  static const bool v = [] {
    const char* e = std::getenv("NZCB_LAGRANGE_COMMIT");
    return !e || std::atoi(e) != 0;
  }();
  return v;
}

__device__ __forceinline__ Fr root4(const Fr* __restrict__ lo, const Fr* __restrict__ hi, size_t i) {
  return lo[i & 4095] * hi[i >> 12];
}

struct PermArgs {
  F29 beta, beta_s;
  F29 k1beta, k1beta_s, k2beta, k2beta_s;
  F29 gamma256;
  int k23;
};
static void shoup_pair(const Fr& c, F29& w, F29& ws) {
  Fr m = c;
  for (int k = 0; k < 5; k++) m = m + m;
  w = split29(from_mont(c));
  ws = mul_lo261(split29(m), f29_const(Fr29::NINV));
}

static F29 fr29_operand(Fr c) {
  for (int k = 0; k < 5; k++) c = c + c;
  return split29(c);
}

#ifndef NZ_KPER
#define NZ_KPER 4
#endif
static constexpr int kPer = NZ_KPER;
static constexpr int kTileN = kT * kPer;
static constexpr int kStageWords = kTileN * 8 + kTileN / 4;

__device__ __forceinline__ int stage_word(int e) { return e * 8 + e / 4; }

template <class F, class U>
__device__ __forceinline__ void stage_use(F&& f, size_t base, size_t len, uint32_t* lds, U&& use) {
#pragma unroll
  for (int k = 0; k < kPer; k++) {
    const int e = k * kT + (int)threadIdx.x;
    const size_t g = base + (size_t)e;
    const Fr v = g < len ? f(g) : Fr::zero();
#pragma unroll
    for (int w = 0; w < 8; w++) lds[stage_word(e) + w] = v.v[w];
  }
  __syncthreads();
#pragma unroll
  for (int j = 0; j < kPer; j++) {
    const int e = kPer * (int)threadIdx.x + j;
    Fr x;
#pragma unroll
    for (int w = 0; w < 8; w++) x.v[w] = lds[stage_word(e) + w];
    use(j, x);
  }
  __syncthreads();
}
template <class F>
__device__ __forceinline__ void stage_in(F&& f, size_t base, size_t len, uint32_t* lds, Fr (&out)[kPer]) {
  stage_use(f, base, len, lds, [&](int j, const Fr& x) { out[j] = x; });
}

__device__ __forceinline__ void stage_out(const Fr (&v)[kPer], size_t base, size_t len, uint32_t* lds, Fr* dst) {
#pragma unroll
  for (int j = 0; j < kPer; j++) {
    const int e = kPer * (int)threadIdx.x + j;
#pragma unroll
    for (int w = 0; w < 8; w++) lds[stage_word(e) + w] = v[j].v[w];
  }
  __syncthreads();
// ... 768 lines not shown
  n4 = 4 * n;
  power = z.power;
  nVars = z.nVars;
  nPublic = z.nPublic;
  nAdditions = z.nAdditions;
  nConstraints = z.nConstraints;
  if (nAdditions > nVars) throw Error(NZCB_ERR_FORMAT, "nAdditions > nVars");
  nWit = nVars - nAdditions;
  k1 = z.k1;
  k2 = z.k2;
  wn = fr_root_of_unity(power);
  w2 = fr_root_of_unity(2);
  eng.reset(new Engine(device, power + 2, 0));
  init_slots();
  hipStream_t s = st();
  auto up = [&](auto& buf, const Section& sec) {
    using T = typename std::remove_reference<decltype(*buf.p)>::type;
    buf.alloc(sec.len / sizeof(T) ? sec.len / sizeof(T) : 1);
    if (sec.len) NZ_HIP(hipMemcpyAsync(buf.p, sec.p, sec.len, hipMemcpyHostToDevice, s));
  };
  up(ptau, z.ptau);
  ptab.build(ptau.p, ptau.n, fixed_base_window(), s, true);
  lcommit = lagrange_commit_enabled() && ptau.n >= (size_t)n + 2;
  if (lcommit) {
    ltau.alloc((size_t)n + 2);
    lagrange_basis(ptau.p, ptau.n, power, ltau.p, s);
    ltab.build(ltau.p, ltau.n, lagrange_window(), s);
    ltab.sparse = lagrange_sparse();
  }
  up(qm, z.qm);
  up(ql, z.ql);
  up(qr, z.qr);
  up(qo, z.qo);
  up(qc, z.qc);
  up(sigma, z.sigma);
  sig_h.alloc((size_t)3 * n);
  w_h.alloc(n);
  for (int k = 0; k < 3; k++)
    hipLaunchKernelGGL(k_stride4, dim3(grid_for(n, kT, 1u << 30)), dim3(kT), 0, s, sigma.p + (size_t)k * 5 * n + n,
                       (size_t)n, sig_h.p + (size_t)k * n);
  NZ_HIP(hipGetLastError());
  up(lagrange, z.lagrange);
  up(amap, z.amap);
  up(bmap, z.bmap);
  up(cmap, z.cmap);
  {
    std::vector<uint32_t> level(nAdditions, 0);
    std::vector<AddRec> recs(nAdditions);
    uint32_t maxlev = 0;
    for (uint32_t k = 0; k < nAdditions; k++) {
      const uint8_t* p = z.additions.p + (size_t)k * 72;
      AddRec r;
      std::memcpy(&r.ai, p, 4);
      std::memcpy(&r.bi, p + 4, 4);
      std::memcpy(r.ac.v, p + 8, 32);
      std::memcpy(r.bc.v, p + 40, 32);
      r.dst = nWit + k;
      r.pad = 0;
      uint32_t lv = 0;
      for (uint32_t* ref : {&r.ai, &r.bi}) {
        if (*ref >= nVars) *ref = kZeroRef;
        else if (*ref >= nWit) {
          uint32_t kk = *ref - nWit;
          if (kk >= k) *ref = kZeroRef;
          else lv = std::max(lv, level[kk] + 1);
        }
      }
      level[k] = lv;
      maxlev = std::max(maxlev, lv);
      recs[k] = r;
    }
    std::vector<uint32_t> cnt(maxlev + 2, 0);
    for (uint32_t k = 0; k < nAdditions; k++) cnt[level[k] + 1]++;
    for (uint32_t l = 1; l < cnt.size(); l++) cnt[l] += cnt[l - 1];
    add_level_start.assign(cnt.begin(), cnt.end());
    std::vector<AddRec> sorted(nAdditions);
    std::vector<uint32_t> cur(cnt.begin(), cnt.end());
    for (uint32_t k = 0; k < nAdditions; k++) sorted[cur[level[k]]++] = recs[k];
    adds.alloc(nAdditions ? nAdditions : 1);
    if (nAdditions)
      NZ_HIP(hipMemcpyAsync(adds.p, sorted.data(), nAdditions * sizeof(AddRec), hipMemcpyHostToDevice, s));
    NZ_HIP(hipStreamSynchronize(s));
  }
  Fr w4 = fr_root_of_unity(power + 2);
  size_t nlo = 4096, nhi = (n4 + 4095) / 4096;
  const Fr one = Fr::one();
  auto table = [&](DevBuf<Fr>& out, size_t cnt, const Fr& base, const Fr& scale) {
    out.alloc(cnt);
    hipLaunchKernelGGL(k_root_table, dim3(grid_for(cnt, kT)), dim3(kT), 0, s, out.p, base, scale, cnt);
    NZ_HIP(hipGetLastError());
  };
  table(root_lo, nlo, w4, one);
  table(root_hi, nhi, pow_u64(w4, 4096), one);
  hipLaunchKernelGGL(k_root_n, dim3(grid_for(n, kT, 1u << 30)), dim3(kT), 0, s, w_h.p, root_lo.p, root_hi.p,
                     (size_t)n);
  NZ_HIP(hipGetLastError());
  const Fr g = fr_small(5), gi = inverse(g);
  table(x_lo, nlo, w4, g);
  table(g_lo, nlo, g, one);
  table(g_hi, nhi, pow_u64(g, 4096), one);
  table(gi_lo, nlo, gi, one);
  table(gi_hi, nhi, pow_u64(gi, 4096), one);
  quot3 = quot3_enabled() && nPublic <= kQ29MaxPub && power >= 6;
  {
    const Fr two = one + one;
    g29.alloc((size_t)n + 8);
    hipLaunchKernelGGL(k_factor29_table, dim3(grid_for((size_t)n + 8, kT, 1u << 30)), dim3(kT), 0, s, g29.p, g_lo.p,
                       g_hi.p, one, (size_t)n + 8);
    if (!quot3) {
      gi29.alloc(n4);
      hipLaunchKernelGGL(k_factor29_table, dim3(grid_for(n4, kT, 1u << 30)), dim3(kT), 0, s, gi29.p, gi_lo.p,
                         gi_hi.p, inverse(pow_u64(two, (uint64_t)power + 2)), (size_t)n4);
    }
    NZ_HIP(hipGetLastError());
  }
  {
    Fr gn = pow_u64(g, n), w4n = pow_u64(w4, n), p = gn;
    for (int k = 0; k < 4; k++) {
      zh_inv[k] = inverse(p - one);
      p = p * w4n;
    }
  }
  alloc_workspace();
  if (quot3) {
    q_h.alloc((size_t)5 * n);
    const DevBuf<Fr>* qs[5] = {&qm, &ql, &qr, &qo, &qc};
    for (int k = 0; k < 5; k++)
      hipLaunchKernelGGL(k_stride4, dim3(grid_for(n, kT, 1u << 30)), dim3(kT), 0, s, qs[k]->p + n, (size_t)n,
                         q_h.p + (size_t)k * n);
    NZ_HIP(hipGetLastError());
  }
  if (quot3) {
    const size_t nhi3 = (n + 4095) / 4096;
    ctw3.alloc((size_t)3 * (n - 1));
    itw3.alloc((size_t)3 * n);
    const Fr inv4n = inverse(fr_small(n4));
    DevBuf<Fr> lo, hi;
    for (int j = 0; j < 3; j++) {
      const Fr cj = g * pow_u64(w4, (uint64_t)j), cji = inverse(cj);
      d3[j] = pow_u64(cj, n);
      ntt_coset_twiddles(eng->ntt_tables, cj, power, ctw3.p + (size_t)j * (n - 1), s);
      table(lo, nlo, cji, one);
      table(hi, nhi3, pow_u64(cji, 4096), one);
      hipLaunchKernelGGL(k_factor29_table, dim3(grid_for(n, kT, 1u << 30)), dim3(kT), 0, s, itw3.p + (size_t)j * n,
                         lo.p, hi.p, inv4n * zh_inv[j], (size_t)n);
      NZ_HIP(hipGetLastError());
      NZ_HIP(hipStreamSynchronize(s));
    }
    for (int k = 0; k < 3; k++)
      NZ_HIP(hipMemcpy(sig_top[k], sigma.p + (size_t)k * 5 * n + (n - 4), 4 * sizeof(Fr), hipMemcpyDeviceToHost));
  }
  if (quot3) {
    const uint32_t nl = nPublic > 0 ? nPublic : 1;
    const size_t n3 = (size_t)3 * n;
    cq3.alloc(5 * n3);
    cs3.alloc(3 * n3);
    cl3.alloc(nl * n3);
    auto coset3 = [&](const Fr* coefs, Fr* out) {
      for (int j = 0; j < 3; j++) {
        NttIo io;
        io.in_len = n;
        io.tw = ctw3.p + (size_t)j * (n - 1);
        ntt(eng->ntt_tables, coefs, out + (size_t)j * n, power, false, s, nullptr, &io);
      }
    };
    const DevBuf<Fr>* qs[5] = {&qm, &ql, &qr, &qo, &qc};
    for (int k = 0; k < 5; k++) coset3(qs[k]->p, cq3.p + (size_t)k * n3);
    for (int k = 0; k < 3; k++) coset3(sigma.p + (size_t)k * 5 * n, cs3.p + (size_t)k * n3);
    for (uint32_t j = 0; j < nl; j++) coset3(lagrange.p + (size_t)j * 5 * n, cl3.p + (size_t)j * n3);
    NZ_HIP(hipGetLastError());
    auto scale = [&](Fr* p, size_t m, int e) {
      hipLaunchKernelGGL(k_dbl_pow, dim3(grid_for(m, kT, 1u << 30)), dim3(kT), 0, s, p, m, e);
    };
    scale(cq3.p, n3, 10);
    scale(cq3.p + n3, 3 * n3, 5);
    scale(cl3.p, (size_t)nl * n3, 5);
    scale(x_lo.p, nlo, 5);
    NZ_HIP(hipGetLastError());
  } else {
    const uint32_t nl = nPublic > 0 ? nPublic : 1;
    cq.alloc((size_t)5 * n4);
    cs.alloc((size_t)3 * n4);
    cl.alloc((size_t)nl * n4);
    auto coset_eval = [&](const Fr* coefs, Fr* out) {
      NttIo io;
      io.in_len = n;
      io.in_f = g29.p;
      ntt(eng->ntt_tables, coefs, out, power + 2, false, s, nullptr, &io);
    };
    const DevBuf<Fr>* qs[5] = {&qm, &ql, &qr, &qo, &qc};
    for (int k = 0; k < 5; k++) coset_eval(qs[k]->p, cq.p + (size_t)k * n4);
    for (int k = 0; k < 3; k++) coset_eval(sigma.p + (size_t)k * 5 * n, cs.p + (size_t)k * n4);
    for (uint32_t j = 0; j < nl; j++) coset_eval(lagrange.p + (size_t)j * 5 * n, cl.p + (size_t)j * n4);
    NZ_HIP(hipGetLastError());
    if (nPublic <= kQ29MaxPub) {
      auto scale = [&](Fr* p, size_t m, int e) {
        hipLaunchKernelGGL(k_dbl_pow, dim3(grid_for(m, kT, 1u << 30)), dim3(kT), 0, s, p, m, e);
      };
      scale(cq.p, n4, 10);
      scale(cq.p + n4, 3 * n4, 5);
      scale(cl.p, (size_t)nl * n4, 5);
      scale(x_lo.p, nlo, 5);
      NZ_HIP(hipGetLastError());
    }
  }
  NZ_HIP(hipStreamSynchronize(s));
}

void Prover::init_slots() {
  for (int i = 0; i < kSlots; i++) {
    msc[i].reset(new MsmScratch());
#ifdef NZCB_AB_GENERIC
    msc[i]->init((size_t)n + 6, true, i == 0 ? 3 : 1, true);
#else
    msc[i]->init((size_t)n + 6, true, i == 0 ? 3 : 1, false);
#endif
    NZ_HIP(hipStreamCreateWithFlags(&aux[i], hipStreamNonBlocking));
    NZ_HIP(hipEventCreateWithFlags(&ready[i], hipEventDisableTiming));
  }
  NZ_HIP(hipEventCreateWithFlags(&side_ready, hipEventDisableTiming));
  NZ_HIP(hipEventCreateWithFlags(&side_done, hipEventDisableTiming));
  NZ_HIP(hipEventCreateWithFlags(&pows_done, hipEventDisableTiming));
  mb_apub = kMbEvals + kMbEvalMax;
  mb_pubw = mb_apub + nPublic;
  mb_words = mb_pubw + nPublic;
  NZ_HIP(hipHostMalloc((void**)&top_host, mb_words * sizeof(Fr), hipHostMallocCoherent));
  std::memset((void*)top_host, 0, mb_words * sizeof(Fr));
}

void Prover::alloc_workspace() {
  wit.alloc(nVars ? nVars : 1);
  wtns_in.alloc(nWit ? nWit : 1);
  A.alloc(n + 2); B.alloc(n + 2); C.alloc(n + 2); Z.alloc(n);
  pol_a.alloc(n + 2); pol_b.alloc(n + 2); pol_c.alloc(n + 2); pol_z.alloc(n + 3);
  const size_t ne = quot3 ? (size_t)3 * n : n4;
  A4.alloc(ne); B4.alloc(ne); C4.alloc(ne); Z4.alloc(ne);
  T.alloc(ne); Tz.alloc(ne); t.alloc(quot3 ? ne + 6 : n4);
  if (quot3) bx_lo.alloc(4096);
  pol_r.alloc(n + 3); pol_wxi.alloc(n + 6); pol_wxiw.alloc(n + 3);
  blind.alloc(13);
  scan_tmp.alloc(3 * ((size_t)n / kTileN + 2) + 64);
  lin_qn = (size_t)n / kTileN + 3;
  lin_tab.alloc(2 * sizeof(LinTab) / sizeof(Fr) + 4 * lin_qn);
  lin_host.resize(2 * sizeof(LinTab) / sizeof(Fr));
  size_t nblocks = ((size_t)3 * n + 6 + (size_t)kT * kEvalChunk2 - 1) / ((size_t)kT * kEvalChunk2) + 1;
  eval_part.alloc((size_t)kEvalMax * nblocks + kEvalMax);
  eval_pw.alloc((size_t)kEvalMax * kT + (kEvalMax * kEvalBits * sizeof(Fr) + sizeof(F29) - 1) / sizeof(F29));
  host_part.resize(std::max<size_t>(nblocks, kEvalMax));
  flags.p = (uint32_t*)(blind.p + 12);
  flags.n = 1;
  flags.owned = false;
  const int zlog = quot3 ? power : power + 2;
  if (zlog > 8) ntt_scr2.alloc((size_t)9 << zlog);
}

Prover::Prover(const Prover& pk, int lane) {
  GuardScope guards;
  lane_id = lane;
  n = pk.n; n4 = pk.n4; nVars = pk.nVars; nPublic = pk.nPublic; nAdditions = pk.nAdditions;
  nConstraints = pk.nConstraints; nWit = pk.nWit; power = pk.power;
  k1 = pk.k1; k2 = pk.k2; wn = pk.wn; w2 = pk.w2;
  add_level_start = pk.add_level_start;
  transcript_public = pk.transcript_public;
  for (int k = 0; k < 4; k++) zh_inv[k] = pk.zh_inv[k];
  NZ_HIP(hipSetDevice(pk.eng->device));
  eng.reset(new Engine(pk.eng->device, power + 2, 0));
  init_slots();
  ptau.alias(pk.ptau);
  ptab.q.alias(pk.ptab.q);
  ptab.n = pk.ptab.n; ptab.stride = pk.ptab.stride; ptab.c = pk.ptab.c; ptab.nw = pk.ptab.nw;
  ptab.mont_folded = pk.ptab.mont_folded;
  lcommit = pk.lcommit;
  ltau.alias(pk.ltau);
  ltab.q.alias(pk.ltab.q);
  ltab.n = pk.ltab.n; ltab.stride = pk.ltab.stride; ltab.c = pk.ltab.c; ltab.nw = pk.ltab.nw;
  ltab.sparse = pk.ltab.sparse;
  qm.alias(pk.qm); ql.alias(pk.ql); qr.alias(pk.qr); qo.alias(pk.qo); qc.alias(pk.qc);
  sigma.alias(pk.sigma); sig_h.alias(pk.sig_h); q_h.alias(pk.q_h); w_h.alias(pk.w_h); lagrange.alias(pk.lagrange);
  amap.alias(pk.amap); bmap.alias(pk.bmap); cmap.alias(pk.cmap); adds.alias(pk.adds);
  root_lo.alias(pk.root_lo); root_hi.alias(pk.root_hi); x_lo.alias(pk.x_lo);
  g_lo.alias(pk.g_lo); g_hi.alias(pk.g_hi); gi_lo.alias(pk.gi_lo); gi_hi.alias(pk.gi_hi);
  g29.alias(pk.g29); gi29.alias(pk.gi29);
  cq.alias(pk.cq); cs.alias(pk.cs); cl.alias(pk.cl);
  quot3 = pk.quot3;
  cq3.alias(pk.cq3); cs3.alias(pk.cs3); cl3.alias(pk.cl3);
  ctw3.alias(pk.ctw3); itw3.alias(pk.itw3);
  for (int j = 0; j < 3; j++) d3[j] = pk.d3[j];
  std::memcpy(sig_top, pk.sig_top, sizeof(sig_top));
  alloc_workspace();
}

void Prover::launch_gate_check(hipStream_t s) {
  hipLaunchKernelGGL(k_gate_h, dim3(grid_for(n, kT, 1u << 30)), dim3(kT), 0, s, A.p, B.p, C.p, q_h.p, (size_t)n,
                     nPublic, flags.p);
  NZ_HIP(hipGetLastError());
}

void Prover::copy_tops(hipStream_t s) {
  hipLaunchKernelGGL(k_tops, dim3(1), dim3(32), 0, s, pol_a.p, pol_b.p, pol_c.p, pol_z.p, (size_t)n,
                     (const uint32_t*)flags.p, top_host);
  NZ_HIP(hipGetLastError());
  NZ_HIP(hipStreamSynchronize(s));
  if (top_host[kMbFlags].v[0] & 1u) throw Error(NZCB_ERR_T_DIV, "T Polynomial is not divisible");
}

void Prover::round3_quot3(const Fr& beta, const Fr& gamma, const Fr& alpha, hipStream_t s) {
  const size_t n3 = (size_t)3 * n;
  const bool side = lcommit;
  if (side) copy_tops(s);
  QArgs29 q29;
  q29.beta = f29_exp(beta, 5);
  q29.k23 = k1 == fr_small(2) && k2 == fr_small(3) ? 1 : 0;
  q29.bk1 = f29_exp(beta * k1, 5);
  q29.bk2 = f29_exp(beta * k2, 5);
  q29.alpha2 = f29_exp(alpha * alpha, 5);
  for (int k = 0; k < 4; k++) q29.zhinv[k] = f29_exp(zh_inv[k], 5);
  q29.gamma = f29_exp(gamma, 0);
  q29.negone = f29_exp(neg(Fr::one()), 0);
  q29.alpha = f29_exp(alpha, 20);
  if (q29.k23)
    hipLaunchKernelGGL(k_beta_xlo, dim3(grid_for(4096, kT)), dim3(kT), 0, s, x_lo.p, q29.beta, (size_t)4096, bx_lo.p);
  hipLaunchKernelGGL((k_quotient_coset29<true>), dim3(grid_for(n3, kT, 1u << 30)), dim3(kT), 0, s, A4.p, B4.p, C4.p,
                     Z4.p, cq3.p, cs3.p, cl3.p, nPublic, A.p, (size_t)n, x_lo.p, root_hi.p, bx_lo.p, q29, T.p);
  if (!side) launch_gate_check(s);
  for (int j = 0; j < 3; j++) {
    NttIo io;
    io.out_f = itw3.p + (size_t)j * n;
    io.out_f_has_scale = true;
    {
      const size_t sp = prof_gpu ? span_begin(1, s) : 0;
      ntt(eng->ntt_tables, T.p + (size_t)j * n, Tz.p + (size_t)j * n, power, true, s, nullptr, &io);
      if (prof_gpu) span_end(sp, s);
    }
  }
  NZ_HIP(hipGetLastError());
  if (!side) copy_tops(s);
  Fr top[4][6];
  std::memcpy(top, top_host, sizeof(top));
  Fr p1[4][6], p2[4][6];
  const Fr w = wn, wi = inverse(wn);
  const Fr wpow[6] = {w * w, w, Fr::one(), wi, wi * wi, wi * wi * wi};
  for (int u = 0; u < 6; u++) {
    for (int f3 = 0; f3 < 3; f3++) {
      p1[f3][u] = top[f3][5 - u];
      p2[f3][u] = top[f3][5 - u];
      if (u >= 2) p2[f3][u] = p2[f3][u] + beta * sig_top[f3][5 - u];
    }
    p1[3][u] = top[3][5 - u];
    p2[3][u] = top[3][5 - u] * wpow[u];
  }
  auto conv = [](const Fr (&x)[6], const Fr (&y)[6], Fr (&out)[6]) {
    for (int s2 = 0; s2 < 6; s2++) {
      Fr acc = Fr::zero();
      for (int u = 0; u <= s2; u++) acc = acc + x[u] * y[s2 - u];
      out[s2] = acc;
    }
  };
  Fr e1[6], e2[6], e3[6], h1[6], h2[6], h3[6];
  conv(p1[0], p1[1], e1);
// ... 84 lines not shown
  slot_split[slot] = false;
  if (!shards.empty() && (!lag || own_lhi)) {
    for (auto& sh : shards) {
      const size_t lo = lag ? sh->llo : sh->lo, hi = lag ? sh->lhi : sh->hi;
      const size_t cnt = len > lo ? std::min(len, hi) - lo : 0;
      NZ_HIP(hipSetDevice(sh->device));
      if (cnt) {
        NZ_HIP(hipStreamWaitEvent(sh->st[slot], ready[slot], 0));
        NZ_HIP(hipMemcpyPeerAsync(sh->scal[slot].p, sh->device, coefs + lo, eng->device, cnt * sizeof(Fr),
                                  sh->st[slot]));
      }
      msm_enqueue(*sh->sc[slot], nullptr, sh->scal[slot].p, cnt, true, sh->st[slot],
                  lag ? &sh->ltable : &sh->table);
    }
    NZ_HIP(hipSetDevice(eng->device));
    len = std::min(len, lag ? own_lhi : own_hi);
    slot_split[slot] = true;
  }
  if (split_send && (!lag || split_own_l)) {
    NZ_HIP(hipEventSynchronize(ready[slot]));
    if (split_send(split_user, slot | (lag ? NZCB_MSM_LAGRANGE : 0), coefs, len) != 0)
      throw Error(NZCB_ERR_INTERNAL, "msm split: sending the scalars to the other ranks failed");
    len = std::min(len, lag ? split_own_l : split_own);
    slot_split[slot] = true;
  }
  const size_t sp = prof_gpu ? span_begin(0, ms) : 0;
  msm_enqueue(*msc[slot], bases ? bases : ptau.p, coefs, len, true, ms, tab ? tab : &ptab);
  if (prof_gpu) span_end(sp, ms);
  static const bool serial = std::getenv("NZCB_SERIAL") != nullptr;
  if (serial) NZ_HIP(hipStreamSynchronize(ms));
  static const char* const kDone[kSlots] = {"mark: commit enqueued slot 0", "mark: commit enqueued slot 1",
                                            "mark: commit enqueued slot 2"};
  roctxMarkA(kDone[slot]);
}

namespace {
void affine_to_le(const G1Affine& a, uint8_t* out) {
  const Fq x = a.is_inf() ? Fq::zero() : from_mont(a.x);
  const Fq y = a.is_inf() ? Fq::zero() : from_mont(a.y);
  std::memcpy(out, x.v, 32);
  std::memcpy(out + 32, y.v, 32);
}

G1xyzz xyzz_from_le(const uint8_t* in) {
  G1Affine a;
  Fq x, y;
  std::memcpy(x.v, in, 32);
  std::memcpy(y.v, in + 32, 32);
  if (x.is_zero() && y.is_zero()) return G1xyzz::inf();
  if (reduce_once(x) != x || reduce_once(y) != y) throw Error(NZCB_ERR_ARG, "msm split: partial not reduced");
  a.x = to_mont(x);
  a.y = to_mont(y);
  return xyzz_from_affine(a);
}
}

G1Affine Prover::commit_finish(int slot) {
  auto t0 = std::chrono::steady_clock::now();
  G1xyzz r = msm_finish(*msc[slot], aux[slot]);
  static const char* const kRes[kSlots] = {"mark: commit result slot 0", "mark: commit result slot 1",
                                           "mark: commit result slot 2"};
  roctxMarkA(kRes[slot]);
  const bool split = slot_split[slot];
  for (auto& sh : shards) {
    if (!split) break;
    NZ_HIP(hipSetDevice(sh->device));
    r = xyzz_add(r, msm_finish(*sh->sc[slot], sh->st[slot]));
  }
  if (!shards.empty()) NZ_HIP(hipSetDevice(eng->device));
  if (split && split_gather) {
    const G1Affine own = xyzz_to_affine(r);
    uint8_t own_le[64];
    affine_to_le(own, own_le);
    std::vector<uint8_t> parts((size_t)split_world * 64);
    if (split_gather(split_user, slot | (slot_lag[slot] ? NZCB_MSM_LAGRANGE : 0), own_le, parts.data()) != 0)
      throw Error(NZCB_ERR_INTERNAL, "msm split: gathering the partial sums failed");
    r = G1xyzz::inf();
    for (int k = 0; k < split_world; k++) r = xyzz_add(r, xyzz_from_le(parts.data() + 64 * (size_t)k));
  }
  msm_ms += ms_since(t0);
  return xyzz_to_affine(r);
}

void Prover::commit_start_abc(size_t len) {
  roctxMarkA("mark: commit enqueue A, B, C");
  const Fr* sc[3] = {A.p, B.p, C.p};
  const size_t sp = prof_gpu ? span_begin(0, st()) : 0;
  msm_enqueue_sets(*msc[0], sc, 3, len, true, st(), &ltab);
  if (prof_gpu) span_end(sp, st());
  roctxMarkA("mark: commit enqueued A, B, C");
}

void Prover::commit_finish_abc(G1Affine& a, G1Affine& b, G1Affine& c) {
  auto t0 = std::chrono::steady_clock::now();
  G1xyzz r[3];
  msm_finish_sets(*msc[0], st(), r);
  roctxMarkA("mark: commit result A, B, C");
  a = xyzz_to_affine(r[0]);
  b = xyzz_to_affine(r[1]);
  c = xyzz_to_affine(r[2]);
  msm_ms += ms_since(t0);
}

void Prover::set_msm_split(int world, size_t own_points, size_t own_lagrange, nzcb_msm_send_fn send,
                           nzcb_msm_gather_fn gather, void* user) {
  if (world <= 1 || !send || !gather) {
    split_send = nullptr;
    split_gather = nullptr;
    split_world = 1;
    split_own = split_own_l = 0;
    return;
  }
  if (!shards.empty()) throw Error(NZCB_ERR_ARG, "msm split: a context splits over devices or over ranks, not both");
  if (own_points == 0 || own_points > ptau.n) throw Error(NZCB_ERR_ARG, "msm split: bad own point count");
  if (own_lagrange > (lcommit ? ltau.n : 0))
    throw Error(NZCB_ERR_ARG, "msm split: bad own Lagrange point count (A, B, C are committed from coefficients "
                              "when the context has no Lagrange basis)");
  split_send = send;
  split_gather = gather;
  split_user = user;
  split_world = world;
  split_own = own_points;
  split_own_l = own_lagrange;
}

void Prover::eval_many(int np, const Fr* const* polys, const size_t* lens, const Fr* xs, Fr* out,
                       const std::function<void()>& overlap) {
  if (np < 1 || np > kEvalMax) throw Error(NZCB_ERR_INTERNAL, "eval_many: bad count");
  hipStream_t s = st();
  EvalSet es{};
  size_t maxlen = 0;
  for (int j = 0; j < np; j++) {
    es.p[j] = polys[j];
    es.len[j] = lens[j];
    es.x[j] = xs[j];
    es.x29[j] = fr29_operand(xs[j]);
    es.y29[j] = fr29_operand(pow_u64(xs[j], kT));
    es.x4096[j] = pow_u64(xs[j], (uint64_t)kT * kEvalChunk2);
    maxlen = std::max(maxlen, lens[j]);
  }
  es.np = np;
  const size_t nblocks = (maxlen + (size_t)kT * kEvalChunk2 - 1) / ((size_t)kT * kEvalChunk2);
  if (nblocks > ((size_t)1 << kEvalBits)) throw Error(NZCB_ERR_INTERNAL, "eval_many: polynomial too long");
  es.nbits = 1;
  while (((size_t)1 << es.nbits) < nblocks) es.nbits++;
  if ((size_t)np * nblocks + kEvalMax > eval_part.n) throw Error(NZCB_ERR_INTERNAL, "eval partial buffer too small");
  Fr* res = eval_part.p + (size_t)np * nblocks;
  F29* pw = eval_pw.p;
  Fr* pw2 = (Fr*)(eval_pw.p + (size_t)kEvalMax * kT);
  hipLaunchKernelGGL(k_eval_pows, dim3((unsigned)np), dim3(kT), 0, s, es, pw, pw2);
  if (np == 7)
    hipLaunchKernelGGL(k_eval_multi<7>, dim3((unsigned)nblocks), dim3(kT), 0, s, es, (const F29*)pw, (const Fr*)pw2,
                       eval_part.p, (int)nblocks);
  else if (np == 1)
    hipLaunchKernelGGL(k_eval_multi<1>, dim3((unsigned)nblocks), dim3(kT), 0, s, es, (const F29*)pw, (const Fr*)pw2,
                       eval_part.p, (int)nblocks);
  else
    throw Error(NZCB_ERR_INTERNAL, "eval_many: 1 or 7 evaluations");
  NZ_HIP(hipGetLastError());
  (void)res;
  hipLaunchKernelGGL(k_eval_sum, dim3(np), dim3(kT), 0, s, (const Fr*)eval_part.p, (int)nblocks,
                     top_host + kMbEvals);
  NZ_HIP(hipGetLastError());
  if (overlap) overlap();
  NZ_HIP(hipStreamSynchronize(s));
  for (int j = 0; j < np; j++) out[j] = top_host[kMbEvals + j];
}

void Prover::lin_tables(int k, const Fr& d, hipStream_t s) {
  LinTab& t = ((LinTab*)lin_host.data())[k];
  t.dp[0] = Fr::one();
  for (int j = 1; j <= kPer; j++) t.dp[j] = t.dp[j - 1] * d;
  const Fr dk = t.dp[kPer], dki = inverse(dk);
  t.P[0] = t.Pinv[0] = Fr::one();
  for (int i = 1; i <= kT; i++) {
    t.P[i] = t.P[i - 1] * dk;
    t.Pinv[i] = t.Pinv[i - 1] * dki;
  }
  NZ_HIP(hipMemcpyAsync((LinTab*)lin_tab.p + k, &t, sizeof(LinTab), hipMemcpyHostToDevice, s));
  Fr* q = lin_tile_pows(k);
  const int qn = (int)lin_qn;
  hipLaunchKernelGGL(k_pow_tiles, dim3((qn + 255) / 256), dim3(256), 0, s, t.P[kT], t.Pinv[kT], qn, q, q + qn);
  NZ_HIP(hipGetLastError());
}

Fr* Prover::lin_tile_pows(int k) { return lin_tab.p + 2 * sizeof(LinTab) / sizeof(Fr) + (size_t)k * 2 * lin_qn; }

void Prover::div_pol1(const Fr* src, size_t m, int tab, const Fr& p0_adjust, Fr* dst, uint32_t flag_bit) {
  hipStream_t s = st();
  const size_t ntiles = (m + kTileN - 1) / kTileN;
  const LinTab* lt = (const LinTab*)lin_tab.p + tab;
  const LinTab& ht = ((const LinTab*)lin_host.data())[tab];
  if (ntiles + 1 > lin_qn) throw Error(NZCB_ERR_INTERNAL, "divPol1: more tiles than its power tables");
  Fr* heads = scan_tmp.p;
  hipLaunchKernelGGL(k_lin_tile<false>, dim3((unsigned)ntiles), dim3(kT), 0, s, src, m, lt, (const Fr*)nullptr, heads);
  const Fr* q = lin_tile_pows(tab);
  hipLaunchKernelGGL(k_tile_heads, dim3(1), dim3(1024), 0, s, heads, (int)ntiles, q, q + lin_qn);
  NZ_HIP(hipGetLastError());
  hipLaunchKernelGGL(k_lin_tile<true>, dim3((unsigned)ntiles), dim3(kT), 0, s, src, m, lt, (const Fr*)heads, dst);
  hipLaunchKernelGGL(k_div_check, dim3(1), dim3(64), 0, s, src, p0_adjust, dst, ht.dp[1], flags.p, flag_bit,
                     (uint32_t*)(top_host + kMbFlags));
  NZ_HIP(hipGetLastError());
}

namespace {
struct RoctxPhases {
  bool open = false;
  explicit RoctxPhases(const char* proof) { roctxRangePush(proof); }
  void next(const char* phase) {
    if (open) roctxRangePop();
    roctxRangePush(phase);
    open = true;
  }
  ~RoctxPhases() {
    if (open) roctxRangePop();
    roctxRangePop();
  }
};
}

namespace {
Fr random_fr() {
  for (;;) {
    uint8_t b[32];
    size_t got = 0;
    while (got < sizeof(b)) {
      ssize_t k = getrandom(b + got, sizeof(b) - got, 0);
      if (k < 0) {
        if (errno == EINTR || errno == EAGAIN) continue;
        throw Error(NZCB_ERR_INTERNAL, std::string("getrandom failed: ") + std::strerror(errno) +
                                           " (no entropy for the blinding scalars)");
      }
      got += (size_t)k;
    }
    b[31] &= 0x3f;
    Fr x;
    std::memcpy(x.v, b, 32);
    if (reduce_once(x) == x) return to_mont(x);
  }
}
}

void Prover::prove(const uint8_t* witness, size_t n_witness, const uint8_t* blinding, uint8_t* proof_out,
                   uint8_t* pub_out, bool witness_on_device) {
  if (n_witness != nWit) {
    throw Error(NZCB_ERR_WITNESS_LEN, "Invalid witness length. Circuit: " + std::to_string(nVars) +
                                          ", witness: " + std::to_string(n_witness) + ", " +
                                          std::to_string(nAdditions));
  }
  NZ_HIP(hipSetDevice(eng->device));
  hipStream_t s = st();
  msm_ms = ntt_ms = 0;
  spans_used = 0;
  if (side_done) NZ_HIP(hipEventSynchronize(side_done));
  static const char* kLaneMark[17] = {"lane 0", "lane 1", "lane 2", "lane 3", "lane 4", "lane 5", "lane 6", "lane 7",
                                      "lane 8", "lane 9", "lane 10", "lane 11", "lane 12", "lane 13", "lane 14",
                                      "lane 15", "lane 16"};
  roctxMarkA(kLaneMark[lane_id < 16 ? lane_id : 16]);
  RoctxPhases ranges("plonk_prove");
  ranges.next("witness: calculateAdditions + buildABC");
  auto T0 = std::chrono::steady_clock::now();
  auto lg = [&](const std::string& m) { if (log) log(m); };
  Fr bl[13];
  bl[0] = Fr::zero();
  bl[12] = Fr::zero();
  for (int i = 1; i <= 11; i++) bl[i] = blinding ? fr_from_le_normal(blinding + 32 * (i - 1)) : random_fr();
  NZ_HIP(hipMemcpyAsync(blind.p, bl, sizeof(bl), hipMemcpyHostToDevice, s));

  lg("Reading Wtns");
  const Fr* wsrc = (const Fr*)witness;
  if (!witness_on_device) {
    NZ_HIP(hipMemcpyAsync(wtns_in.p, witness, (size_t)nWit * 32, hipMemcpyHostToDevice, s));
    wsrc = wtns_in.p;
  } else {
    hipPointerAttribute_t at;
    if (hipPointerGetAttributes(&at, witness) == hipSuccess && at.device != eng->device) {
      NZ_HIP(hipMemcpyPeerAsync(wtns_in.p, eng->device, witness, at.device, (size_t)nWit * 32, s));
      wsrc = wtns_in.p;
    }
  }
  hipLaunchKernelGGL(k_wit_to_mont, dim3(grid_for(nWit, kT, 1u << 30)), dim3(kT), 0, s, wsrc, wit.p,
                     (size_t)nWit);
  for (size_t l = 0; l + 1 < add_level_start.size(); l++) {
    uint32_t a0 = add_level_start[l], a1 = add_level_start[l + 1];
    if (a1 > a0)
      hipLaunchKernelGGL(k_additions, dim3(grid_for(a1 - a0, kT, 1u << 30)), dim3(kT), 0, s, adds.p + a0, a1 - a0,
                         wit.p);
  }
  hipLaunchKernelGGL(k_build_abc, dim3(grid_for(std::max<size_t>(n, nPublic), kT, 1u << 30)), dim3(kT), 0, s,
                     amap.p, bmap.p, cmap.p, nConstraints, n, wit.p, nVars, A.p, B.p, C.p, nPublic,
                     top_host + mb_apub, top_host + mb_pubw);
  NZ_HIP(hipGetLastError());
  NZ_HIP(hipStreamSynchronize(s));
  tm[1] = ms_since(T0);

  ranges.next("round1: to4T + commit A, B, C");
  auto t1 = std::chrono::steady_clock::now();
  G1Affine pA, pB, pC, pZ, pT1, pT2, pT3, pWxi, pWxiw;
  {
    const int ba[2] = {2, 1}, bb[2] = {4, 3}, bc[2] = {6, 5};
    const bool abc_sets = lcommit && shards.empty() && !split_send && msc[0]->max_lsets >= 3 && abc_sets_enabled();
    if (lcommit) {
      hipLaunchKernelGGL(k_abc_tail, dim3(1), dim3(64), 0, s, A.p, B.p, C.p, (size_t)n, blind.p);
      NZ_HIP(hipGetLastError());
      NZ_HIP(hipEventRecord(side_ready, s));
      if (abc_sets) {
        lg("multiexp A");
        lg("multiexp B");
        lg("multiexp C");
        commit_start_abc(n + 2);
      } else {
      lg("multiexp A");
      commit_start(0, A.p, n + 2, &ltab, ltau.p);
      lg("multiexp B");
      commit_start(1, B.p, n + 2, &ltab, ltau.p);
      lg("multiexp C");
      }
      hipStream_t ss = aux[2];
      if (!abc_sets) commit_start(2, C.p, n + 2, &ltab, ltau.p, true);
      NZ_HIP(hipStreamWaitEvent(ss, side_ready, 0));
      to4t(A.p, pol_a.p, A4.p, ba, 2, ss);
      to4t(B.p, pol_b.p, B4.p, bb, 2, ss);
      to4t(C.p, pol_c.p, C4.p, bc, 2, ss);
      if (quot3) launch_gate_check(ss);
      NZ_HIP(hipEventRecord(side_done, ss));
    } else {
      to4t(A.p, pol_a.p, A4.p, ba, 2);
      lg("multiexp A");
      commit_start(0, pol_a.p, n + 2);
      to4t(B.p, pol_b.p, B4.p, bb, 2);
      lg("multiexp B");
      commit_start(1, pol_b.p, n + 2);
      to4t(C.p, pol_c.p, C4.p, bc, 2);
      lg("multiexp C");
      commit_start(2, pol_c.p, n + 2);
    }
    if (lcommit && abc_sets) {
      commit_finish_abc(pA, pB, pC);
    } else {
      pA = commit_finish(0);
      pB = commit_finish(1);
      pC = commit_finish(2);
    }
  }
  tm[2] = ms_since(t1);

  ranges.next("round2: grand product Z + commit");
  auto t2 = std::chrono::steady_clock::now();
  Fr beta, gamma;
  const Fr* Apub = top_host + mb_apub;
  {
    std::vector<uint8_t> tr;
    if (transcript_public) {
      for (uint32_t i = 0; i < nPublic; i++) {
        uint8_t be[32];
        fr_to_be(Apub[i], be);
        tr.insert(tr.end(), be, be + 32);
      }
    }
    for (const G1Affine* p : {&pA, &pB, &pC}) {
      uint8_t u[64];
      g1_uncompressed(*p, u);
      tr.insert(tr.end(), u, u + 64);
    }
    beta = hash_to_fr(tr);
    lg("beta: " + fr_dec(beta));
    std::vector<uint8_t> tr2(32);
    fr_to_be(beta, tr2.data());
    gamma = hash_to_fr(tr2);
    lg("gamma: " + fr_dec(gamma));
  }
  {
    PermArgs pa;
    shoup_pair(beta, pa.beta, pa.beta_s);
    shoup_pair(k1 * beta, pa.k1beta, pa.k1beta_s);
    shoup_pair(k2 * beta, pa.k2beta, pa.k2beta_s);
    pa.gamma256 = f29_exp(gamma, 0);
    pa.k23 = k1 == fr_small(2) && k2 == fr_small(3) ? 1 : 0;
    if (fault == NZCB_DEBUG_GENERIC_K) {
      fault = 0;
      pa.k23 = 0;
    }
    const size_t ntiles = (n + kTileN - 1) / kTileN;
    if (ntiles > 1024 * 64) throw Error(NZCB_ERR_INTERNAL, "round 2: domain too large for the tile factors");
    Fr* ntot = scan_tmp.p;
    Fr* dtot = ntot + ntiles;
    Fr* fac = dtot + ntiles;
    Fr* totals = fac + ntiles;
    hipLaunchKernelGGL(k_perm_tile, dim3((unsigned)ntiles), dim3(kT), 0, s, A.p, B.p, C.p, sig_h.p, (size_t)n,
                       w_h.p, pa, Z.p, ntot, dtot);
    hipLaunchKernelGGL(k_perm_factors, dim3(1), dim3(1024), 0, s, (const Fr*)ntot, (const Fr*)dtot, (int)ntiles,
                       fac, top_host + kMbTotals);
    NZ_HIP(hipGetLastError());
// ... 209 lines not shown
```

nzcb-circom_amd/nzcb/__init__.py:

```python
from __future__ import annotations

import ctypes
import json
import os
from ctypes import POINTER, c_char, c_double, c_int, c_size_t, c_uint8, c_uint32, c_uint64, c_void_p

_HERE = os.path.dirname(os.path.abspath(__file__))
LIB_PATH = os.environ.get("NZCB_LIB", os.path.join(os.path.dirname(_HERE), "lib", "libnzcb.so"))

PROOF_BYTES = 9 * 64 + 7 * 32
BLINDING_BYTES = 11 * 32
VK_BYTES = 8 + 2 * 32 + 8 * 64 + 4 * 32 + 32
PROOF_POINTS = ("A", "B", "C", "Z", "T1", "T2", "T3", "Wxi", "Wxiw")
PROOF_EVALS = ("eval_a", "eval_b", "eval_c", "eval_s1", "eval_s2", "eval_zw", "eval_r")
VK_POINTS = ("Qm", "Ql", "Qr", "Qo", "Qc", "S1", "S2", "S3")

ERROR_NAMES = {
    0: "OK", 1: "ARG", 2: "FORMAT", 3: "NOT_PLONK", 4: "CURVE", 5: "WITNESS_LEN", 6: "COPY",
    7: "T_DIV", 8: "TZ", 9: "DIVPOL", 10: "HIP", 11: "INTERNAL",
}

EXPORTED_SYMBOLS = [
    "nzcb_version", "nzcb_device_count", "nzcb_ctx_create", "nzcb_ctx_destroy", "nzcb_ctx_set_logger",
    "nzcb_ctx_set_transcript_public", "nzcb_ctx_info", "nzcb_prove", "nzcb_prove_witness", "nzcb_prove_device",
    "nzcb_ctx_kernel_stats",
    "nzcb_ctx_last_timings", "nzcb_proof_to_json", "nzcb_public_to_json", "nzcb_synth_setup", "nzcb_free",
    "nzcb_engine_create", "nzcb_engine_destroy", "nzcb_engine_ntt", "nzcb_engine_msm", "nzcb_dev_alloc",
    "nzcb_dev_free", "nzcb_memcpy_h2d", "nzcb_memcpy_d2h", "nzcb_engine_ntt_dev", "nzcb_engine_msm_dev",
    "nzcb_engine_time_ntt", "nzcb_engine_fr_mul", "nzcb_engine_random_fr", "nzcb_engine_fixed_base",
    "nzcb_engine_time_msm", "nzcb_engine_msm_fixed_dev", "nzcb_engine_msm_table_dev", "nzcb_engine_msm_sets_dev", "nzcb_engine_time_msm2", "nzcb_ctx_set_lanes",
    "nzcb_ctx_lanes", "nzcb_prove_batch", "nzcb_vk_from_zkey", "nzcb_vk_from_zkey_file", "nzcb_vk_to_json", "nzcb_verify",
    "nzcb_proof_to_calldata", "nzcb_vk_to_solidity", "nzcb_engine_lagrange_basis", "nzcb_ctx_set_msm_devices", "nzcb_nzcp_input_signals", "nzcb_nzcp_witness",
    "nzcb_nzcp_witness_dev", "nzcb_synth_setup_ex", "nzcb_memcpy_d2d",
    "nzcb_plonk_setup", "nzcb_prove_batch_status", "nzcb_wprog_remap", "nzcb_prove_logged", "nzcb_memcpy_d2d_async",
    "nzcb_debug_guard_check", "nzcb_debug_guard_selftest", "nzcb_debug_inject_fault", "nzcb_debug_f29",
    "nzcb_debug_ntt_coset", "nzcb_debug_msm_plan",
    "nzcb_msm_table_create_lagrange",
    "nzcb_verify_batch", "nzcb_engine_g1_lincomb", "nzcb_engine_verify_batch", "nzcb_debug_verify_batch_timings",
    "nzcb_r1cs_create", "nzcb_r1cs_create_file", "nzcb_r1cs_info", "nzcb_r1cs_check", "nzcb_r1cs_destroy",
    "nzcb_engine_r1cs_create", "nzcb_debug_r1cs_check_timings",
    "nzcb_p256_key_create", "nzcb_p256_verify", "nzcb_p256_key_destroy", "nzcb_engine_p256_key_create",
    "nzcb_debug_p256_field", "nzcb_debug_p256_mul2", "nzcb_debug_p256_timings",
    "nzcb_nzcp_pass_layout", "nzcb_nzcp_decode", "nzcb_nzcp_decode_dev", "nzcb_debug_nzcp_decode_timings",
    "nzcb_ptau_check", "nzcb_ptau_check_file", "nzcb_zkey_check", "nzcb_zkey_check_file", "nzcb_engine_srs_check",
    "nzcb_debug_key_check_timings",
    "nzcb_ptau_new", "nzcb_ptau_new_file", "nzcb_ptau_contribute", "nzcb_ptau_contribute_file",
    "nzcb_ptau_prepare_phase2", "nzcb_ptau_prepare_phase2_file", "nzcb_debug_ptau_timings",
    "nzcb_debug_ptau_batch_top",
    "nzcb_groth16_setup", "nzcb_groth16_setup_file", "nzcb_groth16_contribute", "nzcb_groth16_contribute_file",
    "nzcb_groth16_vk_to_json", "nzcb_groth16_vk_to_json_file", "nzcb_engine_groth16_rows",
    "nzcb_debug_groth16_schedule", "nzcb_debug_groth16_timings",
]

NZCB_FAULT_QUOTIENT = 1
NZCB_DEBUG_GENERIC_K = 2
NZCB_FAULT_LANE_ALLOC = 3
VERIFY_HOST = -1
R1CS_HOST = -1
WITNESS_WTNS, WITNESS_HOST, WITNESS_DEVICE = 0, 1, 2
P256_HOST = -1
SIG_OK, SIG_INVALID, SIG_RANGE = 0, 1, 2
NZCP_HOST = -1
PASS_MAX_URI = 2048
PASS_STATUS_NAMES = ("OK", "LENGTH", "PREFIX", "BASE32", "TRUNCATED", "CBOR", "NOT_COSE", "HEADER",
                     "CLAIMS")
PASS_HAS_ALG, PASS_HAS_KID, PASS_HAS_ISS, PASS_HAS_NBF, PASS_HAS_EXP, PASS_HAS_CTI, PASS_HAS_SIG = (
    1, 2, 4, 8, 16, 32, 64)
KEY_HOST = -1
PTAU_HOST = -1
GROTH16_HOST = -1
KEY_STATUS_NAMES = ("OK", "G2", "RANGE", "CURVE", "GENERATOR", "SEQUENCE", "COSETS", "NONCANONICAL", "LAGRANGE",
                    "EVALS", "COMMIT")
KEY_PARTS = ("Qm", "Ql", "Qr", "Qo", "Qc", "S1", "S2", "S3")
P256_OPS = {"add": 0, "sub": 1, "mul": 2, "sqr": 3, "inv": 4}


def lagrange_commit_enabled() -> bool:
    import re
    e = os.environ.get("NZCB_LAGRANGE_COMMIT")
    if e is None:
        return True
    m = re.match(r"\s*[+-]?\d+", e)
    return bool(m) and int(m.group()) != 0


def guard_check(device: int = -1) -> int:
    err, checked, bad = _Err(), c_size_t(0), c_int(0)
    _check(load().nzcb_debug_guard_check(device, ctypes.byref(checked), ctypes.byref(bad), ctypes.byref(err)), err)
    return checked.value


F29_WORDS = {1: (27, 9), 2: (54, 18), 3: (18, 9), 4: (36, 18), 5: (18, 18), 6: (36, 9), 7: (10, 9)}


def f29_check(op: int, words, device: int = 0):
    win, wout = F29_WORDS[op]
    count = len(words) // win
    assert count * win == len(words)
    arr = (c_uint32 * max(1, len(words)))(*words)
    out = (c_uint32 * max(1, count * wout))()
    err = _Err()
    _check(load().nzcb_debug_f29(device, op, arr, count, out, ctypes.byref(err)), err)
    return list(out)[:count * wout]


def guard_selftest(device: int = 0) -> None:
    err = _Err()
    _check(load().nzcb_debug_guard_selftest(device, ctypes.byref(err)), err)


class NzcbError(RuntimeError):
    def __init__(self, code: int, msg: str):
        super().__init__(msg)
        self.code = code
        self.name = ERROR_NAMES.get(code, str(code))


class _Err(ctypes.Structure):
    _fields_ = [("code", c_int), ("msg", c_char * 256)]


class NzcpParams(ctypes.Structure):
    _fields_ = [("is_live", ctypes.c_int32), ("max_tbs_bytes", ctypes.c_int32),
                ("max_array_len_vc", ctypes.c_int32), ("max_map_len_vc", ctypes.c_int32)]


class NzcpRecord(ctypes.Structure):
    _fields_ = [("status", ctypes.c_int32), ("detail", ctypes.c_int32), ("exp", ctypes.c_uint32),
                ("vc_pos", ctypes.c_int32), ("given_len", ctypes.c_int32), ("family_len", ctypes.c_int32),
                ("dob_len", ctypes.c_int32), ("nullifier_len", ctypes.c_int32),
                ("tbs_sha256", c_uint8 * 32), ("nullifier_sha512", c_uint8 * 64), ("nullifier", c_uint8 * 64),
                ("pub", (c_uint8 * 32) * 3)]


class NzcpPass(ctypes.Structure):
    _fields_ = [("status", ctypes.c_int32), ("detail", c_uint32), ("version", c_uint32), ("present", c_uint32),
                ("alg", ctypes.c_int32), ("kid_len", c_uint32), ("iss_len", c_uint32), ("cti_len", c_uint32),
                ("sig_len", c_uint32), ("cose_len", c_uint32), ("protected_off", c_uint32),
                ("protected_len", c_uint32), ("payload_off", c_uint32), ("payload_len", c_uint32),
                ("tbs_len", c_uint32), ("fits", c_uint32), ("nbf", c_uint64), ("exp", c_uint64),
                ("kid", c_uint8 * 32), ("cti", c_uint8 * 32), ("iss", c_uint8 * 64), ("sig", c_uint8 * 64),
                ("tbs_sha256", c_uint8 * 32)]


NZCP_LIVE = dict(is_live=1, max_tbs_bytes=351, max_array_len_vc=0, max_map_len_vc=4)
NZCP_EXAMPLE = dict(is_live=0, max_tbs_bytes=314, max_array_len_vc=0, max_map_len_vc=4)

LOG_FN = ctypes.CFUNCTYPE(None, c_void_p, ctypes.c_char_p)
MSM_SEND_FN = ctypes.CFUNCTYPE(c_int, c_void_p, c_int, c_void_p, c_size_t)
MSM_GATHER_FN = ctypes.CFUNCTYPE(c_int, c_void_p, c_int, POINTER(c_uint8), POINTER(c_uint8))
MSM_LAGRANGE = 0x100

class KeyFinding(ctypes.Structure):
    _fields_ = [("status", ctypes.c_int32), ("pairing_checks", c_uint32), ("index", ctypes.c_uint64),
                ("n_bad", ctypes.c_uint64), ("checked", ctypes.c_uint64)]


_lib = None


def load(path: str | None = None):
    global _lib
    if _lib is not None and path is None:
        return _lib
    if os.environ.get("GPU_MAX_HW_QUEUES", "4") == "4":
        os.environ["GPU_MAX_HW_QUEUES"] = "24"
# ... 81 lines not shown
                                           c_void_p, POINTER(_Err)]),
        "nzcb_msm_table_create": (c_void_p, [c_int, c_void_p, c_size_t, POINTER(_Err)]),
        "nzcb_msm_table_create_lagrange": (c_void_p, [c_int, c_void_p, c_size_t, c_int, c_size_t, c_size_t,
                                                      POINTER(_Err)]),
        "nzcb_msm_table_run": (c_int, [c_void_p, c_void_p, c_size_t, c_int, u8p, POINTER(_Err)]),
        "nzcb_msm_table_destroy": (None, [c_void_p]),
        "nzcb_ptau_synth": (c_int, [c_int, u8p, c_int, POINTER(POINTER(c_uint8)), POINTER(c_size_t), POINTER(_Err)]),
        "nzcb_wprog_create": (c_void_p, [ctypes.c_char_p, c_size_t, c_int, POINTER(_Err)]),
        "nzcb_wprog_destroy": (None, [c_void_p]),
        "nzcb_wprog_info": (c_int, [c_void_p, POINTER(c_uint32)]),
        "nzcb_wprog_run_dev": (c_int, [c_void_p, c_void_p, c_int, c_void_p, c_size_t, POINTER(ctypes.c_int32),
                                       c_void_p, POINTER(_Err)]),
        "nzcb_wprog_run": (c_int, [c_void_p, ctypes.c_char_p, c_int, u8p, POINTER(ctypes.c_int32), POINTER(_Err)]),
        "nzcb_wprog_remap": (c_int, [ctypes.c_char_p, c_size_t, ctypes.c_char_p, c_size_t, ctypes.c_char_p, c_size_t,
                                     POINTER(POINTER(c_uint8)), POINTER(c_size_t), POINTER(c_uint32), POINTER(_Err)]),
        "nzcb_debug_guard_check": (c_int, [c_int, POINTER(c_size_t), POINTER(c_int), POINTER(_Err)]),
        "nzcb_debug_guard_selftest": (c_int, [c_int, POINTER(_Err)]),
        "nzcb_debug_inject_fault": (c_int, [c_void_p, c_int]),
        "nzcb_debug_f29": (c_int, [c_int, c_int, POINTER(c_uint32), c_size_t, POINTER(c_uint32), POINTER(_Err)]),
        "nzcb_verify_batch": (c_int, [u8p, u8p, u8p, c_size_t, c_int, c_int, c_int, c_int, u8p, POINTER(c_int),
                                      POINTER(_Err)]),
        "nzcb_engine_g1_lincomb": (c_int, [c_int, u8p, u8p, POINTER(c_uint32), c_size_t, u8p, POINTER(_Err)]),
        "nzcb_engine_verify_batch": (c_int, [u8p, u8p, u8p, c_size_t, c_int, c_int, c_int, c_int, u8p, POINTER(c_int),
                                             u8p, POINTER(c_int), POINTER(_Err)]),
        "nzcb_debug_verify_batch_timings": (c_int, [POINTER(c_double), c_int]),
        "nzcb_r1cs_create": (c_void_p, [ctypes.c_char_p, c_size_t, c_int, POINTER(_Err)]),
        "nzcb_r1cs_create_file": (c_void_p, [ctypes.c_char_p, c_int, POINTER(_Err)]),
        "nzcb_engine_r1cs_create": (c_void_p, [ctypes.c_char_p, c_size_t, c_int, c_uint32, c_int, POINTER(_Err)]),
        "nzcb_r1cs_info": (c_int, [c_void_p, POINTER(c_uint32)]),
        "nzcb_r1cs_check": (c_int, [c_void_p, c_void_p, c_size_t, c_int, c_int, c_size_t, POINTER(c_uint32),
                                    POINTER(c_uint32), c_uint32, c_void_p, POINTER(_Err)]),
        "nzcb_r1cs_destroy": (None, [c_void_p]),
        "nzcb_debug_r1cs_check_timings": (c_int, [POINTER(c_double), c_int]),
        "nzcb_p256_key_create": (c_void_p, [ctypes.c_char_p, c_int, POINTER(_Err)]),
        "nzcb_engine_p256_key_create": (c_void_p, [ctypes.c_char_p, c_int, c_int, POINTER(_Err)]),
        "nzcb_p256_verify": (c_int, [c_void_p, c_void_p, c_size_t, c_void_p, c_size_t, c_int, c_int,
                                     POINTER(ctypes.c_int32), c_void_p, POINTER(_Err)]),
        "nzcb_p256_key_destroy": (None, [c_void_p]),
        "nzcb_debug_p256_field": (c_int, [c_int, c_int, c_int, ctypes.c_char_p, ctypes.c_char_p, c_size_t, u8p,
                                          POINTER(_Err)]),
        "nzcb_debug_p256_mul2": (c_int, [c_void_p, ctypes.c_char_p, ctypes.c_char_p, c_size_t, u8p, POINTER(_Err)]),
        "nzcb_debug_p256_timings": (c_int, [POINTER(c_double), c_int]),
        "nzcb_nzcp_pass_layout": (None, [POINTER(c_uint32)]),
        "nzcb_nzcp_decode": (c_int, [c_int, ctypes.c_char_p, POINTER(c_uint32), c_int, POINTER(NzcpParams),
                                     ctypes.c_char_p, POINTER(NzcpPass), u8p, u8p, c_size_t, POINTER(_Err)]),
        "nzcb_nzcp_decode_dev": (c_int, [c_int, c_void_p, c_void_p, c_int, POINTER(NzcpParams), c_void_p, c_void_p,
                                         c_void_p, c_void_p, c_size_t, c_void_p, POINTER(_Err)]),
        "nzcb_debug_nzcp_decode_timings": (c_int, [POINTER(c_double), c_int]),
        "nzcb_ptau_check": (c_int, [c_void_p, c_size_t, ctypes.c_uint64, c_int, u8p, POINTER(KeyFinding),
                                    POINTER(_Err)]),
        "nzcb_ptau_check_file": (c_int, [ctypes.c_char_p, ctypes.c_uint64, c_int, u8p, POINTER(KeyFinding),
                                         POINTER(_Err)]),
        "nzcb_zkey_check": (c_int, [c_void_p, c_size_t, c_int, u8p, POINTER(c_int), POINTER(KeyFinding),
                                    POINTER(KeyFinding), c_uint32, POINTER(c_uint32), POINTER(_Err)]),
        "nzcb_zkey_check_file": (c_int, [ctypes.c_char_p, c_int, u8p, POINTER(c_int), POINTER(KeyFinding),
                                         POINTER(KeyFinding), c_uint32, POINTER(c_uint32), POINTER(_Err)]),
        "nzcb_engine_srs_check": (c_int, [c_int, c_void_p, ctypes.c_uint64, u8p, u8p, c_uint32, POINTER(KeyFinding),
                                          u8p, POINTER(_Err)]),
        "nzcb_debug_key_check_timings": (c_int, [POINTER(c_double), c_int]),
        "nzcb_ptau_new": (c_int, [c_int, POINTER(POINTER(c_uint8)), POINTER(c_size_t), POINTER(_Err)]),
        "nzcb_ptau_new_file": (c_int, [c_int, ctypes.c_char_p, POINTER(_Err)]),
        "nzcb_ptau_contribute": (c_int, [c_void_p, c_size_t, u8p, ctypes.c_char_p, c_size_t, c_int,
                                         POINTER(POINTER(c_uint8)), POINTER(c_size_t), POINTER(_Err)]),
        "nzcb_ptau_contribute_file": (c_int, [ctypes.c_char_p, ctypes.c_char_p, u8p, ctypes.c_char_p, c_size_t,
                                              c_int, POINTER(_Err)]),
        "nzcb_ptau_prepare_phase2": (c_int, [c_void_p, c_size_t, c_int, POINTER(POINTER(c_uint8)),
                                             POINTER(c_size_t), POINTER(_Err)]),
        "nzcb_ptau_prepare_phase2_file": (c_int, [ctypes.c_char_p, ctypes.c_char_p, c_int, POINTER(_Err)]),
        "nzcb_debug_ptau_timings": (c_int, [POINTER(c_double), c_int]),
        "nzcb_debug_ptau_batch_top": (c_int, [c_int]),
        "nzcb_groth16_setup": (c_int, [c_void_p, c_size_t, c_void_p, c_size_t, c_int, POINTER(POINTER(c_uint8)),
                                       POINTER(c_size_t), POINTER(_Err)]),
        "nzcb_groth16_setup_file": (c_int, [ctypes.c_char_p, ctypes.c_char_p, ctypes.c_char_p, c_int, POINTER(_Err)]),
        "nzcb_groth16_contribute": (c_int, [c_void_p, c_size_t, u8p, ctypes.c_char_p, c_size_t, c_int,
                                            POINTER(POINTER(c_uint8)), POINTER(c_size_t), POINTER(_Err)]),
        "nzcb_groth16_contribute_file": (c_int, [ctypes.c_char_p, ctypes.c_char_p, u8p, ctypes.c_char_p, c_size_t,
                                                 c_int, POINTER(_Err)]),
        "nzcb_groth16_vk_to_json": (c_int, [c_void_p, c_size_t, ctypes.c_char_p, c_size_t]),
        "nzcb_groth16_vk_to_json_file": (c_int, [ctypes.c_char_p, ctypes.c_char_p, c_size_t]),
        "nzcb_engine_groth16_rows": (c_int, [c_int, c_int, c_void_p, ctypes.c_uint64, POINTER(ctypes.c_uint64),
                                             ctypes.c_uint64, POINTER(c_uint32), u8p, u8p, POINTER(_Err)]),
        "nzcb_debug_groth16_schedule": (c_int, [c_int, c_int, POINTER(c_int), POINTER(c_int)]),
        "nzcb_debug_groth16_timings": (c_int, [POINTER(c_double), c_int]),
    }
    lib.missing_symbols = []
    for name, (res, args) in sigs.items():
        try:
            fn = getattr(lib, name)
        except AttributeError:
            lib.missing_symbols.append(name)
            continue
        fn.restype = res
        fn.argtypes = args
    if "nzcb_nzcp_pass_layout" not in lib.missing_symbols:
        lay = (c_uint32 * 3)()
        lib.nzcb_nzcp_pass_layout(lay)
        if list(lay) != [ctypes.sizeof(NzcpPass), NzcpPass.sig.offset, NzcpPass.tbs_sha256.offset]:
            raise OSError(f"NzcpPass does not mirror nzcb_nzcp_pass: the library reports {list(lay)}")
    _lib = lib
    return lib


def _buf(data: bytes):
    return (c_uint8 * len(data)).from_buffer_copy(data) if data else (c_uint8 * 1)()


def _out(n: int):
    return (c_uint8 * max(n, 1))()


def _check(rc: int, err: _Err):
    if rc != 0:
        raise NzcbError(rc, err.msg.decode(errors="replace"))


def version() -> str:
    return load().nzcb_version().decode()


def device_count() -> int:
    return load().nzcb_device_count()


def nzcp_input_signals(params: dict) -> int:
    return load().nzcb_nzcp_input_signals(ctypes.byref(NzcpParams(**params)))


def _record_dict(r: NzcpRecord) -> dict:
    return {
        "status": r.status, "detail": r.detail, "exp": r.exp, "vc_pos": r.vc_pos, "given_len": r.given_len,
        "family_len": r.family_len, "dob_len": r.dob_len, "nullifier_len": r.nullifier_len,
        "tbs_sha256": bytes(r.tbs_sha256), "nullifier_sha512": bytes(r.nullifier_sha512),
        "nullifier": bytes(r.nullifier), "out": [int.from_bytes(bytes(r.pub[k]), "little") for k in range(3)],
    }


def nzcp_witness(inputs: bytes, count: int, params: dict = NZCP_LIVE, device: int = 0) -> list:
    lib = load()
    prm = NzcpParams(**params)
    need = lib.nzcb_nzcp_input_signals(ctypes.byref(prm)) * 32 * count
    if len(inputs) != need:
        raise ValueError(f"nzcp inputs are {len(inputs)} bytes, expected {need}")
    recs = (NzcpRecord * max(count, 1))()
    err = _Err()
    _check(lib.nzcb_nzcp_witness(device, ctypes.byref(prm), _buf(inputs), count, recs, ctypes.byref(err)), err)
    return [_record_dict(recs[i]) for i in range(count)]


def nzcp_witness_dev(dev_inputs: int, count: int, params: dict = NZCP_LIVE, device: int = 0,
                     dev_records: int | None = None, dev_witness: int | None = None, witness_stride: int = 0,
                     stream: int | None = None):
    lib = load()
    err = _Err()
    _check(lib.nzcb_nzcp_witness_dev(device, ctypes.byref(NzcpParams(**params)), dev_inputs, count, dev_records,
                                     dev_witness, witness_stride, stream, ctypes.byref(err)), err)


def nzcp_records_from_bytes(raw: bytes, count: int) -> list:
    size = ctypes.sizeof(NzcpRecord)
    return [_record_dict(NzcpRecord.from_buffer_copy(raw[i * size:(i + 1) * size])) for i in range(count)]


def _pass_dict(r: NzcpPass) -> dict:
    has = lambda bit: bool(r.present & bit)
    return {
        "status": r.status, "status_name": PASS_STATUS_NAMES[r.status], "detail": r.detail, "version": r.version,
# ... 401 lines not shown
        err = _Err()
        _check(self.lib.nzcb_ctx_set_lanes(self.h, lanes, ctypes.byref(err)), err)

    def set_msm_devices(self, devices):
        arr = (c_int * len(devices))(*devices)
        err = _Err()
        _check(self.lib.nzcb_ctx_set_msm_devices(self.h, arr, len(devices), ctypes.byref(err)), err)

    def set_msm_split(self, world: int, own_points: int, send, gather, own_lagrange: int = 0):
        if world <= 1:
            self._split_cbs = None
            _check(self.lib.nzcb_ctx_set_msm_split(self.h, 1, 0, 0, MSM_SEND_FN(), MSM_GATHER_FN(), None,
                                                   ctypes.byref(_Err())), _Err())
            return

        def _send(_u, slot, ptr, count):
            try:
                send(slot, ptr, count)
                return 0
            except Exception:
                import traceback
                traceback.print_exc()
                return 1

        def _gather(_u, slot, own, out):
            try:
                parts = gather(slot, ctypes.string_at(own, 64))
                if len(parts) != 64 * world:
                    return 1
                ctypes.memmove(out, parts, len(parts))
                return 0
            except Exception:
                import traceback
                traceback.print_exc()
                return 1

        self._split_cbs = (MSM_SEND_FN(_send), MSM_GATHER_FN(_gather))
        err = _Err()
        _check(self.lib.nzcb_ctx_set_msm_split(self.h, world, own_points, own_lagrange, self._split_cbs[0],
                                               self._split_cbs[1], None, ctypes.byref(err)), err)

    @property
    def lanes(self) -> int:
        return self.lib.nzcb_ctx_lanes(self.h)

    def prove_batch_raw(self, witnesses, n_witness: int | None = None, blindings=None, on_device: bool = False,
                        statuses: list | None = None):
        count = len(witnesses)
        keep = []
        ptrs = (c_void_p * max(count, 1))()
        for i, w in enumerate(witnesses):
            if on_device:
                ptrs[i] = w
            else:
                b = _buf(w)
                keep.append(b)
                ptrs[i] = ctypes.cast(b, c_void_p).value
                if n_witness is None:
                    n_witness = len(w) // 32
        bl = None
        if blindings is not None:
            bl = _buf(b"".join(x if x is not None else random_blinding() for x in blindings))
        proofs = _out(PROOF_BYTES * count)
        stride = 32 * max(self.n_public, 1)
        pubs = _out(stride * count)
        err = _Err()
        if statuses is None:
            _check(self.lib.nzcb_prove_batch(self.h, ptrs, n_witness or 0, count, int(on_device), bl, proofs, pubs,
                                             stride, ctypes.byref(err)), err)
        else:
            st = (c_int * max(count, 1))()
            rc = self.lib.nzcb_prove_batch_status(self.h, ptrs, n_witness or 0, count, int(on_device), bl, proofs,
                                                  pubs, stride, st, ctypes.byref(err))
            if rc and not any(st[i] for i in range(count)):
                _check(rc, err)
            statuses[:] = [st[i] for i in range(count)]
        P, Q = bytes(proofs), bytes(pubs)
        return [(P[i * PROOF_BYTES:(i + 1) * PROOF_BYTES], Q[i * stride:i * stride + 32 * self.n_public])
                for i in range(count)]

    def inject_fault(self, kind: int = NZCB_FAULT_QUOTIENT) -> None:
        if self.lib.nzcb_debug_inject_fault(self.h, kind) != 0:
            raise ValueError(f"bad fault kind {kind}")

    def kernel_stats(self, enable: int = -1):
        out = (c_double * 4)()
        self.lib.nzcb_ctx_kernel_stats(self.h, enable, out)
        return tuple(out)

    def prove(self, wtns, blinding: bytes | None = None):
        proof, pub = self.prove_raw(wtns, blinding)
        return {"proof": proof_to_json(proof), "publicSignals": public_to_json(pub, self.n_public)}

    def last_timings(self):
        ms = (c_double * 11)()
        k = self.lib.nzcb_ctx_last_timings(self.h, ms, 11)
        names = ["total", "witness", "round1", "round2", "round3", "round4", "round5", "msm_host_wait",
                 "ntt_host_enqueue", "msm_gpu", "ntt_gpu"]
        out = dict(zip(names[:k], list(ms)[:k]))
        return {key: v for key, v in out.items() if v >= 0}


class MsmTable:

    def __init__(self, dev_bases: int, n: int, device: int = 0, _handle=None):
        self.lib = load()
        err = _Err()
        self.n = n
        self.h = _handle or self.lib.nzcb_msm_table_create(device, dev_bases, n, ctypes.byref(err))
        if not self.h:
            raise NzcbError(err.code, err.msg.decode(errors="replace"))

    @classmethod
    def lagrange(cls, dev_ptau: int, ptau_n: int, log_n: int, lo: int, hi: int, device: int = 0):
        lib = load()
        err = _Err()
        h = lib.nzcb_msm_table_create_lagrange(device, dev_ptau, ptau_n, log_n, lo, hi, ctypes.byref(err))
        if not h:
            raise NzcbError(err.code, err.msg.decode(errors="replace"))
        return cls(0, hi - lo, device, _handle=h)

    def run(self, dev_scalars: int, count: int, scalars_mont: bool = True) -> bytes:
        out = _out(64)
        err = _Err()
        _check(self.lib.nzcb_msm_table_run(self.h, dev_scalars, count, int(scalars_mont), out, ctypes.byref(err)), err)
        return bytes(out)

    def close(self):
        if getattr(self, "h", None):
            self.lib.nzcb_msm_table_destroy(self.h)
            self.h = None

    __del__ = close


class WitnessProgram:

    def __init__(self, program: bytes, device: int = 0):
        self.lib = load()
        self.device = device
        err = _Err()
        self.h = self.lib.nzcb_wprog_create(program, len(program), device, ctypes.byref(err))
        if not self.h:
            raise NzcbError(err.code, err.msg.decode(errors="replace"))
        info = (c_uint32 * 5)()
        self.lib.nzcb_wprog_info(self.h, info)
        self.n_wires, self.n_out, self.n_pub_in, self.n_prv_in, self.n_levels = list(info)
        self.n_inputs = self.n_pub_in + self.n_prv_in

    def close(self):
        if getattr(self, "h", None):
            self.lib.nzcb_wprog_destroy(self.h)
            self.h = None

    __del__ = close

    def run(self, inputs: bytes, count: int):
        out = _out(max(1, count * self.n_wires * 32))
        st = (ctypes.c_int32 * max(count, 1))()
        err = _Err()
        _check(self.lib.nzcb_wprog_run(self.h, inputs, count, out, st, ctypes.byref(err)), err)
        return bytes(out)[:count * self.n_wires * 32], [st[i] for i in range(count)]

    def run_dev(self, dev_inputs: int, count: int, dev_witness: int, stride: int) -> list:
        st = (ctypes.c_int32 * max(count, 1))()
        err = _Err()
# ... 879 lines not shown
```

Before: 48.55 proofs/s.

## Commit A, B, C wire polynomials over a precomputed per-signal basis

At setup, circom additions and the A/B/C gate maps are expanded into per-signal linear combinations of Lagrange-basis points. A device Groth16-style row reduction folds these into one G1 base per witness signal and set. At prove time, the round-1 A, B, C commitments gather witness values into a compact scalar array and run a fixed-base MSM over roughly nWit points per set instead of n gate points. This trades a heavy host-side expansion and an extra base table at setup for smaller per-proof MSMs, and it falls back to the Lagrange basis when expansion exceeds a cap. The bucket-walk loop in msm.hip also switches to a binary key search after a few linear steps.

```diff
diff --git a/include/nzcb_internal.h b/include/nzcb_internal.h
--- a/include/nzcb_internal.h
+++ b/include/nzcb_internal.h
@@ -16,6 +16,13 @@
 #define NZCB_DEBUG_GENERIC_K 2
 #define NZCB_FAULT_LANE_ALLOC 3
 int nzcb_debug_inject_fault(nzcb_ctx* ctx, int kind);
+
+int nzcb_debug_signal_basis_cap(int per_constraint);
+int nzcb_debug_signal_basis_info(const nzcb_ctx* ctx, uint64_t out[7]);
+int nzcb_debug_commit_abc(nzcb_ctx* ctx, const uint8_t* witness, size_t n_witness, const uint8_t* blinding,
+                          int signal_basis, uint8_t* out, nzcb_err* err);
+int nzcb_debug_signal_rows(nzcb_ctx* ctx, int set, uint8_t* rows_out, uint32_t* signals_out, size_t cap,
+                           nzcb_err* err);
 
 int nzcb_debug_f29(int device, int op, const uint32_t* in, size_t count, uint32_t* out, nzcb_err* err);
 
diff --git a/nzcb-circom_amd/csrc/capi_prover.cpp b/nzcb-circom_amd/csrc/capi_prover.cpp
--- a/nzcb-circom_amd/csrc/capi_prover.cpp
+++ b/nzcb-circom_amd/csrc/capi_prover.cpp
@@ -10,6 +10,7 @@
 
 #include "../../include/nzcb_internal.h"
 #include "prover.h"
+#include "sigbasis.h"
 
 namespace nzcb {
 
@@ -439,6 +440,38 @@
   return 0;
 }
 
+int nzcb_debug_signal_basis_cap(int per_constraint) { return (int)sig_basis_cap(per_constraint < 0 ? -1 : per_constraint); }
+
+int nzcb_debug_signal_basis_info(const nzcb_ctx* ctx, uint64_t out[7]) {
+  if (!ctx || !out) return NZCB_ERR_ARG;
+  const Prover& p = *ctx->p;
+  out[0] = p.sigcommit ? 1 : 0;
+  for (int k = 0; k < 3; k++) out[1 + k] = p.sig_cnt[k];
+  out[4] = p.sig_stride;
+  out[5] = p.sig_terms;
+  out[6] = p.stab.q.n * sizeof(G1Affine);
+  return 0;
+}
+
+int nzcb_debug_commit_abc(nzcb_ctx* ctx, const uint8_t* witness, size_t n_witness, const uint8_t* blinding,
+                          int signal_basis, uint8_t* out, nzcb_err* err) {
+  if (!ctx) return fail(err, NZCB_ERR_ARG, "null argument");
+  return guarded(err, [&] {
+    std::unique_lock<std::shared_mutex> lk(ctx->cfg);
+    ctx->p->debug_commit_abc(witness, n_witness, blinding, signal_basis != 0, out);
+  });
+}
+
+int nzcb_debug_signal_rows(nzcb_ctx* ctx, int set, uint8_t* rows_out, uint32_t* signals_out, size_t cap,
+                           nzcb_err* err) {
+  if (!ctx) return fail(err, NZCB_ERR_ARG, "null argument");
+  return guarded(err, [&] {
+    std::unique_lock<std::shared_mutex> lk(ctx->cfg);
+    if (set < 0 || set > 2 || cap < ctx->p->sig_cnt[set]) throw Error(NZCB_ERR_ARG, "signal rows: set 0..2, cap >= its rows");
+    ctx->p->debug_signal_rows(set, rows_out, signals_out);
+  });
+}
+
 int nzcb_proof_to_json(const uint8_t* proof, char* out, size_t cap) {
   if (!proof) return -1;
   static const char* pts[7] = {"A", "B", "C", "Z", "T1", "T2", "T3"};
diff --git a/nzcb-circom_amd/csrc/groth16.h b/nzcb-circom_amd/csrc/groth16.h
--- a/nzcb-circom_amd/csrc/groth16.h
+++ b/nzcb-circom_amd/csrc/groth16.h
@@ -180,6 +180,8 @@
   for (uint64_t row = 0; row < r.n_rows; row++) p.final_slot[row] = cnt[row] ? off[row] : kG16NoSlot;
   return p;
 }
+
+void g16_rows_g1_device(int device, const G1Pt* d_pts, const G16Rows& r, const G16Plan& plan, uint8_t* out);
 
 struct G16Schedule {
   uint32_t chunk = kG16DefaultChunk, fan_in = kG16DefaultFanIn;
diff --git a/nzcb-circom_amd/csrc/groth16.hip b/nzcb-circom_amd/csrc/groth16.hip
--- a/nzcb-circom_amd/csrc/groth16.hip
+++ b/nzcb-circom_amd/csrc/groth16.hip
@@ -215,6 +215,11 @@
 
 }
 
+void g16_rows_g1_device(int device, const G1Pt* d_pts, const G16Rows& r, const G16Plan& plan, uint8_t* out) {
+  G16DeviceBackend be(device);
+  be.rows_on<Fq>(d_pts, r, plan, out);
+}
+
 }
 
 using namespace nzcb;
diff --git a/nzcb-circom_amd/csrc/msm.h b/nzcb-circom_amd/csrc/msm.h
--- a/nzcb-circom_amd/csrc/msm.h
+++ b/nzcb-circom_amd/csrc/msm.h
@@ -74,7 +74,7 @@
                  hipStream_t st, const MsmBaseTable* table = nullptr);
 G1xyzz msm_finish(MsmScratch& sc, hipStream_t st);
 void msm_enqueue_sets(MsmScratch& sc, const Fr* const* scalars, int sets, size_t n, bool scalars_mont,
-                      hipStream_t st, const MsmBaseTable* table);
+                      hipStream_t st, const MsmBaseTable* table, const uint32_t* set_base = nullptr);
 void msm_finish_sets(MsmScratch& sc, hipStream_t st, G1xyzz* out);
 
 inline G1xyzz msm(MsmScratch& sc, const G1Affine* bases, const Fr* scalars, size_t n, bool mont, hipStream_t st,
diff --git a/nzcb-circom_amd/csrc/msm.hip b/nzcb-circom_amd/csrc/msm.hip
--- a/nzcb-circom_amd/csrc/msm.hip
+++ b/nzcb-circom_amd/csrc/msm.hip
@@ -203,7 +203,7 @@
 
 template <int C, int NW>
 __device__ __forceinline__ uint32_t bin_entries(const Fr* __restrict__ scalars, size_t i, int mont, size_t stride,
-                                                uint32_t (&kk)[NW], uint32_t (&vv)[NW]) {
+                                                uint32_t base, uint32_t (&kk)[NW], uint32_t (&vv)[NW]) {
   Fr s = scalars[i];
   if (mont & kDigMont) s = from_mont_fr29(s);
   const uint32_t flip = (mont & kDigMinForm) ? scalar_min_form(s) : 0u;
@@ -215,7 +215,7 @@
   }
   for_each_digit<C>(s, [&](int w, uint32_t b, uint32_t sign) {
     kk[w] = b;
-    vv[w] = (uint32_t)((size_t)w * stride + i) | ((sign ^ flip) << 31);
+    vv[w] = (uint32_t)((size_t)w * stride + base + i) | ((sign ^ flip) << 31);
     live |= 1u << w;
   });
   return live;
@@ -230,6 +230,7 @@
 static constexpr int kMaxSets = 3;
 struct BinSets {
   const Fr* p[kMaxSets];
+  uint32_t base[kMaxSets];
   uint32_t tps;
   uint32_t nb;
 };
@@ -250,7 +251,7 @@
     const size_t i = (size_t)lt * kTileScalars + (size_t)j * kBinThreads + threadIdx.x;
     if (i < n) {
       uint32_t kk[NW], vv[NW];
-      const uint32_t live = bin_entries<C, NW>(scalars, i, mont, 0, kk, vv);
+      const uint32_t live = bin_entries<C, NW>(scalars, i, mont, 0, 0u, kk, vv);
 #pragma unroll
       for (int w = 0; w < NW; w++)
         if ((live >> w) & 1u) atomicAdd(&h[(kk[w] + kbase) >> LO], 1u);
@@ -325,7 +326,7 @@
     const size_t i = (size_t)lt * kTileScalars + (size_t)j * kBinThreads + threadIdx.x;
     live[j] = 0;
     if (i < n) {
-      live[j] = bin_entries<C, NW>(scalars, i, mont, stride, kk[j], vv[j]);
+      live[j] = bin_entries<C, NW>(scalars, i, mont, stride, sets.base[set], kk[j], vv[j]);
 #pragma unroll
       for (int w = 0; w < NW; w++) {
         kk[j][w] += kbase;
@@ -698,7 +699,13 @@
       else if (!starts) carry_cont[t] = out;
       else carry_own[t] = out;
       inf = true;
-      while (pos < e && kend <= pos) {
+      for (int step = 0; pos < e && kend <= pos; step++) {
+        if (step == 4) {
+          k = find_key(offsets, nkeys, pos);
+          kstart = offsets[k];
+          kend = offsets[k + 1];
+          break;
+        }
         k++;
         kstart = kend;
         kend = offsets[k + 1];
@@ -1598,7 +1605,7 @@
 }
 
 static void msm_enqueue_impl(MsmScratch& sc, const G1Affine* bases, const Fr* const* scalars, int msets, size_t n,
-                             bool mont, hipStream_t st, const MsmBaseTable* table) {
+                             bool mont, hipStream_t st, const MsmBaseTable* table, const uint32_t* set_base = nullptr) {
   const auto t_enq = std::chrono::steady_clock::now();
   struct EnqueueClock {
     MsmScratch& sc;
@@ -1616,6 +1623,8 @@
   if (!sc.done) NZ_HIP(hipEventCreateWithFlags(&sc.done, hipEventDisableTiming));
   if (n > sc.max_points) throw Error(NZCB_ERR_ARG, "msm larger than scratch");
   if (table && n > table->n) throw Error(NZCB_ERR_ARG, "msm larger than its base table");
+  for (int k = 0; table && set_base && k < msets; k++)
+    if ((size_t)set_base[k] + n > table->n) throw Error(NZCB_ERR_ARG, "msm sets: a set's points lie past the base table");
   if (table && table->mont_folded && !mont) throw Error(NZCB_ERR_ARG, "2^-256-folded table needs Montgomery scalars");
   if (table && (!sc.buckets29.p || !sc.bin_counts.p))
     throw Error(NZCB_ERR_ARG, "msm scratch was not sized for the fixed-base schedule");
@@ -1682,7 +1691,10 @@
   mark(0);
   if (table) {
     BinSets bs{};
-    for (int k = 0; k < msets; k++) bs.p[k] = scalars[k];
+    for (int k = 0; k < msets; k++) {
+      bs.p[k] = scalars[k];
+      bs.base[k] = set_base ? set_base[k] : 0u;
+    }
     fixed_bucketing(sc, p, bs, n, mdig | (table->mont_folded ? 0 : kDigMinForm), table, st, mark);
   } else {
     keys_dispatch(p.c, scalars[0], n, mdig, sc, st);
@@ -1854,9 +1866,9 @@
 }
 
 void msm_enqueue_sets(MsmScratch& sc, const Fr* const* scalars, int sets, size_t n, bool mont, hipStream_t st,
-                      const MsmBaseTable* table) {
+                      const MsmBaseTable* table, const uint32_t* set_base) {
   if (!table) throw Error(NZCB_ERR_ARG, "msm sets: a table schedule");
-  msm_enqueue_impl(sc, nullptr, scalars, sets, n, mont, st, table);
+  msm_enqueue_impl(sc, nullptr, scalars, sets, n, mont, st, table, set_base);
 }
 
 static G1xyzz fixed_window_result(const G1xyzz* s, int hb, int a) {
diff --git a/nzcb-circom_amd/csrc/prover.h b/nzcb-circom_amd/csrc/prover.h
--- a/nzcb-circom_amd/csrc/prover.h
+++ b/nzcb-circom_amd/csrc/prover.h
@@ -49,6 +49,13 @@
   DevBuf<G1Affine> ltau;
   MsmBaseTable ltab;
   bool lcommit = false;
+  MsmBaseTable stab;
+  DevBuf<uint32_t> sig_idx;
+  uint32_t sig_cnt[3] = {0, 0, 0};
+  size_t sig_stride = 0;
+  bool sigcommit = false;
+  std::string sig_note;
+  uint64_t sig_terms = 0;
   DevBuf<Fr> qm, ql, qr, qo, qc;
   DevBuf<Fr> sigma;
   DevBuf<Fr> sig_h;
@@ -72,6 +79,7 @@
   DevBuf<Fr> wit;
   DevBuf<Fr> wtns_in;
   DevBuf<Fr> A, B, C, Z;
+  DevBuf<Fr> sig_scal;
   DevBuf<Fr> pol_a, pol_b, pol_c, pol_z;
   DevBuf<Fr> A4, B4, C4, Z4, T, Tz, t;
   DevBuf<Fr> bx_lo;
@@ -116,8 +124,14 @@
                      nzcb_msm_gather_fn gather, void* user);
   void prove(const uint8_t* witness, size_t n_witness, const uint8_t* blinding, uint8_t* proof_out,
              uint8_t* pub_out, bool witness_on_device = false);
+  void debug_commit_abc(const uint8_t* witness, size_t n_witness, const uint8_t* blinding, bool signal_basis,
+                        uint8_t* out);
+  void debug_signal_rows(int set, uint8_t* rows_out, uint32_t* signals_out);
 
  private:
+  void load_witness(const uint8_t* witness, const uint8_t* blinding, bool witness_on_device);
+  void build_signal_basis(const Zkey& z);
+  bool sig_note_logged = false;
   hipStream_t st() const { return eng->stream; }
   void init_slots();
   void alloc_workspace();
@@ -130,7 +144,7 @@
   void commit_start(int slot, const Fr* scalars, size_t len, const MsmBaseTable* tab = nullptr,
                     const G1Affine* bases = nullptr, bool on_main = false);
   G1Affine commit_finish(int slot);
-  void commit_start_abc(size_t len);
+  void commit_start_abc(size_t len, bool signal_basis);
   void commit_finish_abc(G1Affine& a, G1Affine& b, G1Affine& c);
   void eval_many(int np, const Fr* const* polys, const size_t* lens, const Fr* xs, Fr* out,
                  const std::function<void()>& overlap = nullptr);
diff --git a/nzcb-circom_amd/csrc/prover.hip b/nzcb-circom_amd/csrc/prover.hip
--- a/nzcb-circom_amd/csrc/prover.hip
+++ b/nzcb-circom_amd/csrc/prover.hip
@@ -1,6 +1,7 @@
 #include <rocprofiler-sdk-roctx/roctx.h>
 #include "lagrange.h"
 #include "prover.h"
+#include "sigbasis.h"
 #include "transcript.h"
 
 #include <cstring>
@@ -96,6 +97,27 @@
   B[n + 1] = bl[3];
   C[n] = bl[6];
   C[n + 1] = bl[5];
+}
+
+__global__ void k_sig_stage(const uint32_t* __restrict__ idx, uint32_t stride, uint32_t c0, uint32_t c1, uint32_t c2,
+                            const Fr* __restrict__ wit, const Fr* __restrict__ bl, Fr* __restrict__ out) {
+  const size_t i = (size_t)blockIdx.x * blockDim.x + threadIdx.x;
+  if (i >= (size_t)3 * stride) return;
+  const uint32_t set = (uint32_t)(i / stride), j = (uint32_t)(i - (size_t)set * stride);
+  const uint32_t cnt = set == 0 ? c0 : set == 1 ? c1 : c2;
+  Fr v = Fr::zero();
+  if (j < cnt) v = from_mont(wit[idx[i]]);
+  else if (j == cnt) v = from_mont(bl[2 + 2 * set]);
+  else if (j == cnt + 1) v = from_mont(bl[1 + 2 * set]);
+  out[i] = v;
+}
+
+static bool signal_commit_enabled() {
+  static const bool v = [] {
+    const char* e = std::getenv("NZCB_SIGNAL_COMMIT");
+    return !e || std::atoi(e) != 0;
+  }();
+  return v;
 }
 
 static bool abc_sets_enabled() {
@@ -1030,6 +1052,7 @@
       NZ_HIP(hipMemcpyAsync(adds.p, sorted.data(), nAdditions * sizeof(AddRec), hipMemcpyHostToDevice, s));
     NZ_HIP(hipStreamSynchronize(s));
   }
+  if (lcommit && signal_commit_enabled() && abc_sets_enabled()) build_signal_basis(z);
   Fr w4 = fr_root_of_unity(power + 2);
   size_t nlo = 4096, nhi = (n4 + 4095) / 4096;
   const Fr one = Fr::one();
@@ -1155,6 +1178,34 @@
   NZ_HIP(hipStreamSynchronize(s));
 }
 
+void Prover::build_signal_basis(const Zkey& z) {
+  hipStream_t s = st();
+  if (z.additions.len < (uint64_t)nAdditions * 72 || z.amap.len < (uint64_t)nConstraints * 4 ||
+      z.bmap.len < (uint64_t)nConstraints * 4 || z.cmap.len < (uint64_t)nConstraints * 4) {
+    sig_note = "signal basis: the key's maps are shorter than its header says; A, B, C are committed from the "
+               "Lagrange basis";
+    return;
+  }
+  NZ_HIP(hipStreamSynchronize(s));
+  SigBasis sb = sig_basis_build(eng->device, ltau.p, n, nWit, nVars, nConstraints, z.additions.p, nAdditions,
+                                z.amap.p, z.bmap.p, z.cmap.p, (size_t)n + 2);
+  sig_terms = sb.terms;
+  if (!sb.ok) {
+    sig_note = sb.note;
+    return;
+  }
+  for (int k = 0; k < 3; k++) sig_cnt[k] = sb.cnt[k];
+  sig_stride = sb.stride;
+  DevBuf<G1Affine> bases(sb.bases.size());
+  NZ_HIP(hipMemcpyAsync(bases.p, sb.bases.data(), sb.bases.size() * sizeof(G1Affine), hipMemcpyHostToDevice, s));
+  sig_idx.alloc(sb.idx.size());
+  NZ_HIP(hipMemcpyAsync(sig_idx.p, sb.idx.data(), sb.idx.size() * sizeof(uint32_t), hipMemcpyHostToDevice, s));
+  stab.build(bases.p, bases.n, lagrange_window(), s);
+  stab.sparse = lagrange_sparse();
+  NZ_HIP(hipStreamSynchronize(s));
+  sigcommit = true;
+}
+
 void Prover::init_slots() {
   for (int i = 0; i < kSlots; i++) {
     msc[i].reset(new MsmScratch());
@@ -1180,6 +1231,7 @@
   wit.alloc(nVars ? nVars : 1);
   wtns_in.alloc(nWit ? nWit : 1);
   A.alloc(n + 2); B.alloc(n + 2); C.alloc(n + 2); Z.alloc(n);
+  if (sigcommit) sig_scal.alloc(3 * sig_stride);
   pol_a.alloc(n + 2); pol_b.alloc(n + 2); pol_c.alloc(n + 2); pol_z.alloc(n + 3);
   const size_t ne = quot3 ? (size_t)3 * n : n4;
   A4.alloc(ne); B4.alloc(ne); C4.alloc(ne); Z4.alloc(ne);
@@ -1223,6 +1275,15 @@
   ltab.q.alias(pk.ltab.q);
   ltab.n = pk.ltab.n; ltab.stride = pk.ltab.stride; ltab.c = pk.ltab.c; ltab.nw = pk.ltab.nw;
   ltab.sparse = pk.ltab.sparse;
+  sigcommit = pk.sigcommit;
+  sig_note = pk.sig_note;
+  sig_terms = pk.sig_terms;
+  sig_stride = pk.sig_stride;
+  for (int k = 0; k < 3; k++) sig_cnt[k] = pk.sig_cnt[k];
+  sig_idx.alias(pk.sig_idx);
+  stab.q.alias(pk.stab.q);
+  stab.n = pk.stab.n; stab.stride = pk.stab.stride; stab.c = pk.stab.c; stab.nw = pk.stab.nw;
+  stab.sparse = pk.stab.sparse;
   qm.alias(pk.qm); ql.alias(pk.ql); qr.alias(pk.qr); qo.alias(pk.qo); qc.alias(pk.qc);
   sigma.alias(pk.sigma); sig_h.alias(pk.sig_h); q_h.alias(pk.q_h); w_h.alias(pk.w_h); lagrange.alias(pk.lagrange);
   amap.alias(pk.amap); bmap.alias(pk.bmap); cmap.alias(pk.cmap); adds.alias(pk.adds);
@@ -1473,11 +1534,21 @@
   return xyzz_to_affine(r);
 }
 
-void Prover::commit_start_abc(size_t len) {
+void Prover::commit_start_abc(size_t len, bool signal_basis) {
   roctxMarkA("mark: commit enqueue A, B, C");
   const Fr* sc[3] = {A.p, B.p, C.p};
   const size_t sp = prof_gpu ? span_begin(0, st()) : 0;
-  msm_enqueue_sets(*msc[0], sc, 3, len, true, st(), &ltab);
+  if (signal_basis && sigcommit) {
+    const uint32_t stride = (uint32_t)sig_stride;
+    hipLaunchKernelGGL(k_sig_stage, dim3(grid_for((size_t)3 * stride, kT, 1u << 30)), dim3(kT), 0, st(), sig_idx.p,
+                       stride, sig_cnt[0], sig_cnt[1], sig_cnt[2], wit.p, blind.p, sig_scal.p);
+    NZ_HIP(hipGetLastError());
+    const Fr* ss[3] = {sig_scal.p, sig_scal.p + stride, sig_scal.p + 2 * (size_t)stride};
+    const uint32_t base[3] = {0, stride, 2 * stride};
+    msm_enqueue_sets(*msc[0], ss, 3, stride, false, st(), &stab, base);
+  } else {
+    msm_enqueue_sets(*msc[0], sc, 3, len, true, st(), &ltab);
+  }
   if (prof_gpu) span_end(sp, st());
   roctxMarkA("mark: commit enqueued A, B, C");
 }
@@ -1491,6 +1562,42 @@
   b = xyzz_to_affine(r[1]);
   c = xyzz_to_affine(r[2]);
   msm_ms += ms_since(t0);
+}
+
+void Prover::debug_commit_abc(const uint8_t* witness, size_t n_witness, const uint8_t* blinding, bool signal_basis,
+                              uint8_t* out) {
+  if (!witness || !blinding || !out || n_witness != nWit) throw Error(NZCB_ERR_ARG, "commit A, B, C: bad argument");
+  if (!lcommit || !shards.empty() || split_send || msc[0]->max_lsets < 3)
+    throw Error(NZCB_ERR_ARG, "commit A, B, C: the context does not commit them in one schedule");
+  if (signal_basis && !sigcommit) throw Error(NZCB_ERR_ARG, "commit A, B, C: the context has no signal basis");
+  NZ_HIP(hipSetDevice(eng->device));
+  if (side_done) NZ_HIP(hipEventSynchronize(side_done));
+  load_witness(witness, blinding, false);
+  hipLaunchKernelGGL(k_abc_tail, dim3(1), dim3(64), 0, st(), A.p, B.p, C.p, (size_t)n, blind.p);
+  NZ_HIP(hipGetLastError());
+  commit_start_abc(n + 2, signal_basis);
+  G1Affine p[3];
+  commit_finish_abc(p[0], p[1], p[2]);
+  std::memcpy(out, p, sizeof p);
+}
+
+void Prover::debug_signal_rows(int set, uint8_t* rows_out, uint32_t* signals_out) {
+  if (set < 0 || set > 2 || !sigcommit) throw Error(NZCB_ERR_ARG, "signal rows: no such set or no signal basis");
+  NZ_HIP(hipSetDevice(eng->device));
+  const uint32_t cnt = sig_cnt[set];
+  if (!cnt) return;
+  if (!rows_out || !signals_out) throw Error(NZCB_ERR_ARG, "null argument");
+  std::vector<G1Affine> q(cnt);
+  NZ_HIP(hipMemcpy(q.data(), stab.q.p + (size_t)set * sig_stride, cnt * sizeof(G1Affine), hipMemcpyDeviceToHost));
+  NZ_HIP(hipMemcpy(signals_out, sig_idx.p + (size_t)set * sig_stride, cnt * sizeof(uint32_t), hipMemcpyDeviceToHost));
+  Fq thirty_two = Fq::zero();
+  thirty_two.v[0] = 32;
+  const Fq k = inverse(to_mont(thirty_two));
+  for (uint32_t i = 0; i < cnt; i++) {
+    q[i].x = q[i].x * k;
+    q[i].y = q[i].y * k;
+  }
+  std::memcpy(rows_out, q.data(), cnt * sizeof(G1Affine));
 }
 
 void Prover::set_msm_split(int world, size_t own_points, size_t own_lagrange, nzcb_msm_send_fn send,
@@ -1632,6 +1739,39 @@
 }
 }
 
+void Prover::load_witness(const uint8_t* witness, const uint8_t* blinding, bool witness_on_device) {
+  hipStream_t s = st();
+  Fr bl[13];
+  bl[0] = Fr::zero();
+  bl[12] = Fr::zero();
+  for (int i = 1; i <= 11; i++) bl[i] = blinding ? fr_from_le_normal(blinding + 32 * (i - 1)) : random_fr();
+  NZ_HIP(hipMemcpyAsync(blind.p, bl, sizeof(bl), hipMemcpyHostToDevice, s));
+  const Fr* wsrc = (const Fr*)witness;
+  if (!witness_on_device) {
+    NZ_HIP(hipMemcpyAsync(wtns_in.p, witness, (size_t)nWit * 32, hipMemcpyHostToDevice, s));
+    wsrc = wtns_in.p;
+  } else {
+    hipPointerAttribute_t at;
+    if (hipPointerGetAttributes(&at, witness) == hipSuccess && at.device != eng->device) {
+      NZ_HIP(hipMemcpyPeerAsync(wtns_in.p, eng->device, witness, at.device, (size_t)nWit * 32, s));
+      wsrc = wtns_in.p;
+    }
+  }
+  hipLaunchKernelGGL(k_wit_to_mont, dim3(grid_for(nWit, kT, 1u << 30)), dim3(kT), 0, s, wsrc, wit.p,
+                     (size_t)nWit);
+  for (size_t l = 0; l + 1 < add_level_start.size(); l++) {
+    uint32_t a0 = add_level_start[l], a1 = add_level_start[l + 1];
+    if (a1 > a0)
+      hipLaunchKernelGGL(k_additions, dim3(grid_for(a1 - a0, kT, 1u << 30)), dim3(kT), 0, s, adds.p + a0, a1 - a0,
+                         wit.p);
+  }
+  hipLaunchKernelGGL(k_build_abc, dim3(grid_for(std::max<size_t>(n, nPublic), kT, 1u << 30)), dim3(kT), 0, s,
+                     amap.p, bmap.p, cmap.p, nConstraints, n, wit.p, nVars, A.p, B.p, C.p, nPublic,
+                     top_host + mb_apub, top_host + mb_pubw);
+  NZ_HIP(hipGetLastError());
+  NZ_HIP(hipStreamSynchronize(s));
+}
+
 void Prover::prove(const uint8_t* witness, size_t n_witness, const uint8_t* blinding, uint8_t* proof_out,
                    uint8_t* pub_out, bool witness_on_device) {
   if (n_witness != nWit) {
@@ -1652,37 +1792,12 @@
   ranges.next("witness: calculateAdditions + buildABC");
   auto T0 = std::chrono::steady_clock::now();
   auto lg = [&](const std::string& m) { if (log) log(m); };
-  Fr bl[13];
-  bl[0] = Fr::zero();
-  bl[12] = Fr::zero();
-  for (int i = 1; i <= 11; i++) bl[i] = blinding ? fr_from_le_normal(blinding + 32 * (i - 1)) : random_fr();
-  NZ_HIP(hipMemcpyAsync(blind.p, bl, sizeof(bl), hipMemcpyHostToDevice, s));
-
+  if (!sig_note.empty() && !sig_note_logged && log) {
+    lg(sig_note);
+    sig_note_logged = true;
+  }
   lg("Reading Wtns");
-  const Fr* wsrc = (const Fr*)witness;
-  if (!witness_on_device) {
-    NZ_HIP(hipMemcpyAsync(wtns_in.p, witness, (size_t)nWit * 32, hipMemcpyHostToDevice, s));
-    wsrc = wtns_in.p;
-  } else {
-    hipPointerAttribute_t at;
-    if (hipPointerGetAttributes(&at, witness) == hipSuccess && at.device != eng->device) {
-      NZ_HIP(hipMemcpyPeerAsync(wtns_in.p, eng->device, witness, at.device, (size_t)nWit * 32, s));
-      wsrc = wtns_in.p;
-    }
-  }
-  hipLaunchKernelGGL(k_wit_to_mont, dim3(grid_for(nWit, kT, 1u << 30)), dim3(kT), 0, s, wsrc, wit.p,
-                     (size_t)nWit);
-  for (size_t l = 0; l + 1 < add_level_start.size(); l++) {
-    uint32_t a0 = add_level_start[l], a1 = add_level_start[l + 1];
-    if (a1 > a0)
-      hipLaunchKernelGGL(k_additions, dim3(grid_for(a1 - a0, kT, 1u << 30)), dim3(kT), 0, s, adds.p + a0, a1 - a0,
-                         wit.p);
-  }
-  hipLaunchKernelGGL(k_build_abc, dim3(grid_for(std::max<size_t>(n, nPublic), kT, 1u << 30)), dim3(kT), 0, s,
-                     amap.p, bmap.p, cmap.p, nConstraints, n, wit.p, nVars, A.p, B.p, C.p, nPublic,
-                     top_host + mb_apub, top_host + mb_pubw);
-  NZ_HIP(hipGetLastError());
-  NZ_HIP(hipStreamSynchronize(s));
+  load_witness(witness, blinding, witness_on_device);
   tm[1] = ms_since(T0);
 
   ranges.next("round1: to4T + commit A, B, C");
@@ -1699,7 +1814,7 @@
         lg("multiexp A");
         lg("multiexp B");
         lg("multiexp C");
-        commit_start_abc(n + 2);
+        commit_start_abc(n + 2, true);
       } else {
       lg("multiexp A");
       commit_start(0, A.p, n + 2, &ltab, ltau.p);
diff --git a/nzcb-circom_amd/csrc/sigbasis.h b/nzcb-circom_amd/csrc/sigbasis.h
--- /dev/null
+++ b/nzcb-circom_amd/csrc/sigbasis.h
@@ -0,0 +1,28 @@
+#pragma once
+#include <string>
+#include <vector>
+
+#include "ec.h"
+
+namespace nzcb {
+
+struct SigBasis {
+  bool ok = false;
+  std::string note;
+  uint32_t cnt[3] = {0, 0, 0};
+  size_t stride = 0;
+  std::vector<uint32_t> idx;
+  std::vector<G1Affine> bases;
+  uint64_t terms = 0;
+  uint64_t expanded = 0;
+};
+constexpr uint32_t kSigNone = 0xffffffffu;
+constexpr uint64_t kSigCapDefault = 64;
+
+uint64_t sig_basis_cap(int64_t per_constraint = -2);
+
+SigBasis sig_basis_build(int device, const G1Affine* d_ltau, uint32_t n, uint32_t nWit, uint32_t nVars,
+                         uint32_t nConstraints, const uint8_t* additions, uint32_t nAdditions,
+                         const uint8_t* amap, const uint8_t* bmap, const uint8_t* cmap, size_t max_stride);
+
+}
diff --git a/nzcb-circom_amd/csrc/sigbasis.hip b/nzcb-circom_amd/csrc/sigbasis.hip
--- /dev/null
+++ b/nzcb-circom_amd/csrc/sigbasis.hip
@@ -0,0 +1,141 @@
+#include "sigbasis.h"
+
+#include <atomic>
+#include <cstring>
+
+#include "groth16.h"
+
+namespace nzcb {
+
+static std::atomic<uint64_t> g_sig_cap{kSigCapDefault};
+
+uint64_t sig_basis_cap(int64_t per_constraint) {
+  if (per_constraint == -2) return g_sig_cap.load();
+  return g_sig_cap.exchange(per_constraint < 0 ? kSigCapDefault : (uint64_t)per_constraint);
+}
+
+namespace {
+
+struct SigTerm {
+  uint32_t s;
+  Fr c;
+};
+
+}
+
+SigBasis sig_basis_build(int device, const G1Affine* d_ltau, uint32_t n, uint32_t nWit, uint32_t nVars,
+                         uint32_t nConstraints, const uint8_t* additions, uint32_t nAdditions,
+                         const uint8_t* amap, const uint8_t* bmap, const uint8_t* cmap, size_t max_stride) {
+  SigBasis sb;
+  const uint64_t cap = sig_basis_cap() * 3 * (uint64_t)nConstraints;
+  auto give_up = [&](const std::string& why) {
+    sb.ok = false;
+    sb.note = "signal basis: " + why + "; A, B, C are committed from the Lagrange basis";
+    return sb;
+  };
+  std::vector<uint64_t> off((size_t)nAdditions + 1, 0);
+  std::vector<SigTerm> ex;
+  std::vector<SigTerm> ta, tb;
+  for (uint32_t k = 0; k < nAdditions; k++) {
+    const uint8_t* p = additions + (size_t)k * 72;
+    uint32_t ai, bi;
+    Fr ac, bc;
+    std::memcpy(&ai, p, 4);
+    std::memcpy(&bi, p + 4, 4);
+    std::memcpy(ac.v, p + 8, 32);
+    std::memcpy(bc.v, p + 40, 32);
+    auto operand = [&](uint32_t v, const Fr& coef, std::vector<SigTerm>& out) {
+      out.clear();
+      if (v == 0 || v >= nVars) return;
+      if (v < nWit) {
+        out.push_back({v, coef});
+        return;
+      }
+      const uint32_t kk = v - nWit;
+      if (kk >= k) return;
+      for (uint64_t t = off[kk]; t < off[kk + 1]; t++) out.push_back({ex[t].s, coef * ex[t].c});
+    };
+    operand(ai, ac, ta);
+    operand(bi, bc, tb);
+    size_t i = 0, j = 0;
+    auto put = [&](uint32_t s, const Fr& c) {
+      if (!reduce_once(c).is_zero()) ex.push_back({s, c});
+    };
+    while (i < ta.size() || j < tb.size()) {
+      if (j == tb.size() || (i < ta.size() && ta[i].s < tb[j].s)) {
+        put(ta[i].s, ta[i].c);
+        i++;
+      } else if (i == ta.size() || tb[j].s < ta[i].s) {
+        put(tb[j].s, tb[j].c);
+        j++;
+      } else {
+        put(ta[i].s, ta[i].c + tb[j].c);
+        i++;
+        j++;
+      }
+    }
+    off[k + 1] = ex.size();
+    if (ex.size() > cap) return give_up("the additions expand past " + std::to_string(cap) + " terms");
+  }
+  sb.expanded = ex.size();
+
+  const uint32_t gates = nConstraints < n ? nConstraints : n;
+  G16RowsBuilder b((uint64_t)3 * nWit, n);
+  const uint8_t* maps[3] = {amap, bmap, cmap};
+  for (int set = 0; set < 3; set++) {
+    for (uint32_t g = 0; g < gates; g++) {
+      uint32_t v;
+      std::memcpy(&v, maps[set] + (size_t)g * 4, 4);
+      if (v == 0 || v >= nVars) continue;
+      if (v < nWit) {
+        b.add((uint64_t)set * nWit + v, g, Fr::one());
+        sb.terms++;
+      } else {
+        const uint32_t kk = v - nWit;
+        for (uint64_t t = off[kk]; t < off[kk + 1]; t++) b.add((uint64_t)set * nWit + ex[t].s, g, ex[t].c);
+        sb.terms += off[kk + 1] - off[kk];
+      }
+      if (sb.terms > cap) return give_up("the gates expand past " + std::to_string(cap) + " terms");
+    }
+  }
+  ex.clear();
+  ex.shrink_to_fit();
+  G16Rows rows = b.finish();
+  const G16Schedule sch = g16_schedule();
+  const G16Plan plan = g16_plan(rows, sch.chunk, sch.fan_in);
+  std::vector<G1Affine> out((size_t)3 * nWit);
+  g16_rows_g1_device(device, reinterpret_cast<const G1Pt*>(d_ltau), rows, plan, reinterpret_cast<uint8_t*>(out.data()));
+
+  auto present = [&](size_t r) { return rows.row_off[r + 1] > rows.row_off[r] && !out[r].is_inf(); };
+  uint32_t most = 0;
+  for (int set = 0; set < 3; set++) {
+    for (uint32_t s = 0; s < nWit; s++) sb.cnt[set] += present((size_t)set * nWit + s) ? 1u : 0u;
+    most = sb.cnt[set] > most ? sb.cnt[set] : most;
+  }
+  sb.stride = (size_t)most + 2;
+  if (sb.stride > max_stride)
+    return give_up("a set has " + std::to_string(most) + " signals, more than the " + std::to_string(n) + " gate slots");
+  G1Affine tail[2];
+  if (hipMemcpy(tail, d_ltau + n, sizeof tail, hipMemcpyDeviceToHost) != hipSuccess)
+    throw Error(NZCB_ERR_HIP, "signal basis: reading the blinding points failed");
+  G1Affine inf;
+  inf.x = Fq::zero();
+  inf.y = Fq::zero();
+  sb.idx.assign(3 * sb.stride, kSigNone);
+  sb.bases.assign(3 * sb.stride, inf);
+  for (int set = 0; set < 3; set++) {
+    size_t at = (size_t)set * sb.stride;
+    for (uint32_t s = 0; s < nWit; s++) {
+      const size_t r = (size_t)set * nWit + s;
+      if (!present(r)) continue;
+      sb.idx[at] = s;
+      sb.bases[at++] = out[r];
+    }
+    sb.bases[at] = tail[0];
+    sb.bases[at + 1] = tail[1];
+  }
+  sb.ok = true;
+  return sb;
+}
+
+}
diff --git a/nzcb-circom_amd/nzcb/__init__.py b/nzcb-circom_amd/nzcb/__init__.py
--- a/nzcb-circom_amd/nzcb/__init__.py
+++ b/nzcb-circom_amd/nzcb/__init__.py
@@ -50,6 +50,7 @@
     "nzcb_groth16_setup", "nzcb_groth16_setup_file", "nzcb_groth16_contribute", "nzcb_groth16_contribute_file",
     "nzcb_groth16_vk_to_json", "nzcb_groth16_vk_to_json_file", "nzcb_engine_groth16_rows",
     "nzcb_debug_groth16_schedule", "nzcb_debug_groth16_timings",
+    "nzcb_debug_signal_basis_cap", "nzcb_debug_signal_basis_info", "nzcb_debug_commit_abc", "nzcb_debug_signal_rows",
 ]
 
 NZCB_FAULT_QUOTIENT = 1
@@ -82,6 +83,10 @@
         return True
     m = re.match(r"\s*[+-]?\d+", e)
     return bool(m) and int(m.group()) != 0
+
+
+def signal_basis_cap(per_constraint: int = -1) -> int:
+    return load().nzcb_debug_signal_basis_cap(per_constraint)
 
 
 def guard_check(device: int = -1) -> int:
@@ -329,6 +334,10 @@
                                              ctypes.c_uint64, POINTER(c_uint32), u8p, u8p, POINTER(_Err)]),
         "nzcb_debug_groth16_schedule": (c_int, [c_int, c_int, POINTER(c_int), POINTER(c_int)]),
         "nzcb_debug_groth16_timings": (c_int, [POINTER(c_double), c_int]),
+        "nzcb_debug_signal_basis_cap": (c_int, [c_int]),
+        "nzcb_debug_signal_basis_info": (c_int, [c_void_p, POINTER(c_uint64)]),
+        "nzcb_debug_commit_abc": (c_int, [c_void_p, u8p, c_size_t, u8p, c_int, u8p, POINTER(_Err)]),
+        "nzcb_debug_signal_rows": (c_int, [c_void_p, c_int, u8p, POINTER(c_uint32), c_size_t, POINTER(_Err)]),
     }
     lib.missing_symbols = []
     for name, (res, args) in sigs.items():
@@ -896,6 +905,31 @@
     def inject_fault(self, kind: int = NZCB_FAULT_QUOTIENT) -> None:
         if self.lib.nzcb_debug_inject_fault(self.h, kind) != 0:
             raise ValueError(f"bad fault kind {kind}")
+
+    def signal_basis_info(self) -> dict:
+        out = (c_uint64 * 7)()
+        self.lib.nzcb_debug_signal_basis_info(self.h, out)
+        return {"on": bool(out[0]), "rows": [int(out[1]), int(out[2]), int(out[3])], "stride": int(out[4]),
+                "terms": int(out[5]), "table_bytes": int(out[6])}
+
+    def commit_abc(self, witness_le: bytes, blinding: bytes, signal_basis: bool):
+        if len(blinding) != BLINDING_BYTES:
+            raise ValueError("blinding must be 11 x 32 bytes")
+        out = _out(192)
+        err = _Err()
+        _check(self.lib.nzcb_debug_commit_abc(self.h, _buf(witness_le), len(witness_le) // 32, _buf(blinding),
+                                              int(signal_basis), out, ctypes.byref(err)), err)
+        b = bytes(out)
+        return b[:64], b[64:128], b[128:]
+
+    def signal_rows(self, k: int) -> dict:
+        cnt = self.signal_basis_info()["rows"][k]
+        rows = _out(64 * cnt)
+        sig = (c_uint32 * max(cnt, 1))()
+        err = _Err()
+        _check(self.lib.nzcb_debug_signal_rows(self.h, k, rows, sig, cnt, ctypes.byref(err)), err)
+        b = bytes(rows)
+        return {int(sig[i]): b[64 * i:64 * i + 64] for i in range(cnt)}
 
     def kernel_stats(self, enable: int = -1):
         out = (c_double * 4)()
```

Result: faster. 49.75 proofs/s (median of 6 runs) (+2.5%).
